# zhibaishouheilab/HealthiVert-GAN

Hardware: AMD Instinct MI355X
Metric: sagittal slices/sec (train step, G+D) at 256x256 bs=16 (higher is better)
Workload: dtype f16; 1 GPU; two-stage coarse+refine generator + 3x PatchGAN D train step, 256x256, per-GPU bs=16, norm=batch, vanilla GAN; global_batch=16, parallelism=dp1, launch=hipGraph replay (1 graphs/step), 4 streams

## Files before the change

healthivert-gan_amd/csrc/conv_igemm.hip:

```cpp
#include <string.h>

#include "hv_common.h"
#include <stdlib.h>

#define HV_MAX_TAPS 25
#define HV_BK 32

thread_local int hv_path_note = 0;
thread_local int hv_wtable_used = 0;
extern "C" int hv_last_weight_tables(void) { return hv_wtable_used; }
thread_local char hv_kname[192] = "";
extern "C" const char* hv_last_kernel_name(void) { return hv_kname; }
extern "C" int hv_last_kernel_path(void) { return hv_path_note; }
thread_local hipEvent_t hv_ev_start = nullptr, hv_ev_stop = nullptr;
extern "C" int hv_set_kernel_timing(void* ev_start, void* ev_stop) {
    hv_ev_start = (hipEvent_t)ev_start; hv_ev_stop = (hipEvent_t)ev_stop;
    return HV_OK;
}

int hv_conv2d_halo(const hv_conv_desc* d, const void* w_f16, hipStream_t s);
int hv_conv2d_g4(const hv_conv_desc* d, hipStream_t s);
int hv_conv2d_thin_dgrad(const hv_conv_desc* d, hipStream_t s);
int hv_conv2d_logits_dgrad(const hv_conv_desc* d, hipStream_t s);
size_t hv_conv2d_g4_stats_floats(const hv_conv_desc* d, int* nparts);
size_t hv_conv2d_g4_bstats_parts(const hv_conv_desc* d);
size_t hv_conv2d_logits_bstats_parts(const hv_conv_desc* d);
size_t hv_wgrad_halo_workspace_bytes(const hv_wgrad_desc* d);
int hv_wgrad_halo(const hv_wgrad_desc* d, int* nslabs, hipStream_t s);
size_t hv_wgrad_tr_workspace_bytes(const hv_wgrad_desc* d);
int hv_wgrad_tr(const hv_wgrad_desc* d, int* nslabs, hipStream_t s);
int hv_wgrad_thin(const hv_wgrad_desc* d, int* nslabs, hipStream_t s);
size_t hv_wgrad_thin_workspace_bytes(const hv_wgrad_desc* d);
int hv_conv2d_narrow(const hv_conv_desc* d, hipStream_t s);
int hv_conv2d_thin_in(const hv_conv_desc* d, hipStream_t s);
int hv_conv2d_stem5(const hv_conv_desc* d, hipStream_t s);
int hv_conv2d_stem5_dgrad(const hv_conv_desc* d, hipStream_t s);
int hv_conv2d_head(const hv_conv_desc* d, hipStream_t s);
int hv_conv2d_px(const hv_conv_desc* d, hipStream_t s);
int hv_conv2d_s2t(const hv_conv_desc* d, hipStream_t s);

struct ConvCls {
    int ph, pw, Hc, Wc, ntaps, Ktot, m0, mcount;
    uint32_t taps[HV_MAX_TAPS];
};
struct ConvK {
    const void* x; const float* w; const float* bias; const float* scale; void* y;
    int x_half, y_half, mul_half;
    long long w_bs, scale_bs;
    int B, Hl, Wl, in_shift, Wp, img_stride, x_ld, x_coff, Cin;
    int Cout, w_row, y_ld, y_coff, Ho, Wo;
    int bstep, boff, ostep;
    float alpha; int act, accumulate, vec_store, ncls;
    int xcd_swizzle;
    const void* mul_src; int mul_ld, mul_coff, mul_act, mul_vec;
    ConvCls cls[4];
};

template <typename T> struct Stage;
template <> struct Stage<float> {
    static constexpr int LD = HV_BK + 4;
    static __device__ __forceinline__ void st4(float* dst, float4 v) { *reinterpret_cast<float4*>(dst) = v; }
};
template <> struct Stage<_Float16> {
    static constexpr int LD = HV_BK + 8;
    static __device__ __forceinline__ void st4(_Float16* dst, float4 v) {
        f16x4 h = {(_Float16)v.x, (_Float16)v.y, (_Float16)v.z, (_Float16)v.w};
        *reinterpret_cast<f16x4*>(dst) = h;
    }
};

template <typename T, int MT, int NT> struct Frags;
template <int MT, int NT> struct Frags<float, MT, NT> {
    float4 w[NT][2], x[MT][2];
    __device__ __forceinline__ void load(const float* Bs, const float* As, int wrow0, int xrow0, int lane) {
        const int off = (lane & 15) * Stage<float>::LD + (lane >> 4) * 8;
#pragma unroll
        for (int n = 0; n < NT; ++n) {
            const float* p = Bs + (wrow0 + n * 16) * Stage<float>::LD + off;
            w[n][0] = *reinterpret_cast<const float4*>(p);
            w[n][1] = *reinterpret_cast<const float4*>(p + 4);
        }
#pragma unroll
        for (int m = 0; m < MT; ++m) {
            const float* p = As + (xrow0 + m * 16) * Stage<float>::LD + off;
            x[m][0] = *reinterpret_cast<const float4*>(p);
            x[m][1] = *reinterpret_cast<const float4*>(p + 4);
        }
    }
    __device__ __forceinline__ void mma(f32x4 (&acc)[NT][MT]) {
#pragma unroll
        for (int n = 0; n < NT; ++n)
#pragma unroll
            for (int m = 0; m < MT; ++m) {
                f32x4 a = acc[n][m];
                a = __builtin_amdgcn_mfma_f32_16x16x4f32(w[n][0].x, x[m][0].x, a, 0, 0, 0);
                a = __builtin_amdgcn_mfma_f32_16x16x4f32(w[n][0].y, x[m][0].y, a, 0, 0, 0);
                a = __builtin_amdgcn_mfma_f32_16x16x4f32(w[n][0].z, x[m][0].z, a, 0, 0, 0);
                a = __builtin_amdgcn_mfma_f32_16x16x4f32(w[n][0].w, x[m][0].w, a, 0, 0, 0);
                a = __builtin_amdgcn_mfma_f32_16x16x4f32(w[n][1].x, x[m][1].x, a, 0, 0, 0);
                a = __builtin_amdgcn_mfma_f32_16x16x4f32(w[n][1].y, x[m][1].y, a, 0, 0, 0);
                a = __builtin_amdgcn_mfma_f32_16x16x4f32(w[n][1].z, x[m][1].z, a, 0, 0, 0);
                a = __builtin_amdgcn_mfma_f32_16x16x4f32(w[n][1].w, x[m][1].w, a, 0, 0, 0);
                acc[n][m] = a;
            }
    }
};
template <int MT, int NT> struct Frags<_Float16, MT, NT> {
    f16x8 w[NT], x[MT];
    __device__ __forceinline__ void load(const _Float16* Bs, const _Float16* As, int wrow0, int xrow0, int lane) {
        const int off = (lane & 15) * Stage<_Float16>::LD + (lane >> 4) * 8;
#pragma unroll
        for (int n = 0; n < NT; ++n) w[n] = *reinterpret_cast<const f16x8*>(Bs + (wrow0 + n * 16) * Stage<_Float16>::LD + off);
#pragma unroll
        for (int m = 0; m < MT; ++m) x[m] = *reinterpret_cast<const f16x8*>(As + (xrow0 + m * 16) * Stage<_Float16>::LD + off);
    }
    __device__ __forceinline__ void mma(f32x4 (&acc)[NT][MT]) {
#pragma unroll
        for (int n = 0; n < NT; ++n)
#pragma unroll
            for (int m = 0; m < MT; ++m) acc[n][m] = __builtin_amdgcn_mfma_f32_16x16x32_f16(w[n], x[m], acc[n][m], 0, 0, 0);
    }
};

template <typename T, int BM, int BN, int WM, int WN, bool ASC, bool XH>
__global__ __launch_bounds__(256) void conv_igemm_kernel(const ConvK p) {
    constexpr int LD = Stage<T>::LD;
    constexpr int APASS = BM / 32;
    constexpr int BPASS = (BN + 31) / 32;
    constexpr int TMW = BM / WM, TNW = BN / WN;
    constexpr int MT = TMW / 16, NT = TNW / 16;
    static_assert(WM * WN == 4 && MT >= 1 && NT >= 1, "bad tile");
    __shared__ __attribute__((aligned(16))) T As[BM * LD];
    __shared__ __attribute__((aligned(16))) T Bs[BN * LD];
    __shared__ uint32_t taps_s[32];

    const int tid = threadIdx.x, lane = tid & 63, wave = tid >> 6;
    int bx = blockIdx.x;
    if (p.xcd_swizzle) {
        const int q = gridDim.x >> 3, r = gridDim.x & 7, xcd = bx & 7, loc = bx >> 3;
        bx = xcd < r ? xcd * (q + 1) + loc : r * (q + 1) + (xcd - r) * q + loc;
    }
    int ci = 0;
#pragma unroll
    for (int i = 1; i < 4; ++i)
        if (i < p.ncls && bx >= p.cls[i].m0) ci = i;
    const ConvCls& C = p.cls[ci];
    const int ntaps = C.ntaps, Ktot = C.Ktot, Hc = C.Hc, Wc = C.Wc, Mc = C.mcount, ph = C.ph, pw = C.pw;
    if (tid < ntaps) taps_s[tid] = C.taps[tid];
    const int m_base = (bx - C.m0) * BM;
    const int n_base = blockIdx.y * BN;
    const int HWc = Hc * Wc;

    const int chunk = tid & 7, prow = tid >> 3;
    int a_nb[APASS], a_hw[APASS];
    const int sample0 = m_base / HWc;
#pragma unroll
    for (int i = 0; i < APASS; ++i) {
        const int m = m_base + prow + i * 32;
        int bh = -20000, bw = -20000, nb = 0;
        if (m < Mc) {
            const int n = m / HWc, rem = m - n * HWc;
            const int ii = rem / Wc, jj = rem - ii * Wc;
            bh = ii * p.bstep + p.boff;
            bw = jj * p.bstep + p.boff;
            nb = n * p.img_stride;
        }
        a_nb[i] = nb;
        a_hw[i] = (int)(((uint32_t)bh << 16) | ((uint32_t)bw & 0xffffu));
    }
    const float* wbase = p.w + (p.w_bs ? (long long)sample0 * p.w_bs : 0ll);
    const int nk = (Ktot + HV_BK - 1) / HV_BK;

    float4 ra[APASS], rb[BPASS];
    auto gload = [&](int kt) {
        const int kg = kt * HV_BK + chunk * 4;
        if (!ASC) {
            const bool kok = kg < Ktot;
            int tapi = 0, c = 0, dh = 0, dw = 0, widx = 0;
            if (kok) {
                tapi = kg / p.Cin;
                c = kg - tapi * p.Cin;
                const uint32_t e = taps_s[tapi];
                dh = (int)(int8_t)(e & 0xff);
// ... 524 lines not shown
#pragma unroll
            for (int it = 0; it < XPT; ++it) store(Xs, LDX, rx[it], x_cg[it], x_run[it]);
        }
        __syncthreads();
        if (pix0 + KT < pix_end) {
            if (has_g) load_g(pix0 + KT);
            if (has_x) load_x(pix0 + KT);
        }
        if constexpr (F16) {
            const _Float16* G16 = reinterpret_cast<const _Float16*>(Gs);
            const _Float16* X16 = reinterpret_cast<const _Float16*>(Xs);
#pragma unroll
            for (int ks = 0; ks < KT / 32; ++ks) {
                f16x8 a[NT], b[CT];
#pragma unroll
                for (int n = 0; n < NT; ++n) {
                    const int row = wn * TNW + n * 16 + (lane & 15);
                    a[n] = *reinterpret_cast<const f16x8*>(G16 + row * LDG + ((ks * 4 + (lane >> 4)) ^ ((row >> 2) & 7)) * 8);
                }
#pragma unroll
                for (int c = 0; c < CT; ++c) {
                    const int row = wc * TCW + c * 16 + (lane & 15);
                    b[c] = *reinterpret_cast<const f16x8*>(X16 + row * LDX + ((ks * 4 + (lane >> 4)) ^ ((row >> 2) & 7)) * 8);
                }
#pragma unroll
                for (int n = 0; n < NT; ++n)
#pragma unroll
                    for (int c = 0; c < CT; ++c) acc[n][c] = __builtin_amdgcn_mfma_f32_16x16x32_f16(a[n], b[c], acc[n][c], 0, 0, 0);
            }
        } else {
            const float* G32 = reinterpret_cast<const float*>(Gs);
            const float* X32 = reinterpret_cast<const float*>(Xs);
#pragma unroll
            for (int k4 = 0; k4 < KT / 4; ++k4) {
                const int pk = k4 * 4 + (lane >> 4);
                float a[NT], b[CT];
#pragma unroll
                for (int n = 0; n < NT; ++n) a[n] = G32[pk * LDG + wn * TNW + n * 16 + (lane & 15)];
#pragma unroll
                for (int c = 0; c < CT; ++c) b[c] = X32[pk * LDX + wc * TCW + c * 16 + (lane & 15)];
#pragma unroll
                for (int n = 0; n < NT; ++n)
#pragma unroll
                    for (int c = 0; c < CT; ++c) acc[n][c] = __builtin_amdgcn_mfma_f32_16x16x4f32(a[n], b[c], acc[n][c], 0, 0, 0);
            }
        }
    }
    if (do_bias) {
        __syncthreads();
        float* bsh = reinterpret_cast<float*>(Xs);
        if (has_g) { bsh[tid * 4 + 0] = bs0; bsh[tid * 4 + 1] = bs1; bsh[tid * 4 + 2] = bs2; bsh[tid * 4 + 3] = bs3; }
        __syncthreads();
        if (tid < BN && n_base + tid < p.Cout) {
            const int cg = tid >> 2, c = tid & 3;
            float t = 0.f;
            for (int run = 0; run < KT / 8; ++run) t += bsh[(run * (BN / 4) + cg) * 4 + c];
            p.bias_out[(long long)blockIdx.x * p.Cout + n_base + tid] = t;
        }
    }
    float* out = p.out + (long long)blockIdx.x * p.slab;
#pragma unroll
    for (int n = 0; n < NT; ++n)
#pragma unroll
        for (int c = 0; c < CT; ++c) {
            const int j = j_base + wc * TCW + c * 16 + (lane & 15);
            if (j >= p.J) continue;
#pragma unroll
            for (int r = 0; r < 4; ++r) {
                const int co = n_base + wn * TNW + n * 16 + (lane >> 4) * 4 + r;
                if (co < p.Cout) out[(long long)co * p.J + j] = acc[n][c][r];
            }
        }
}

template <int G>
__global__ __launch_bounds__(256) void wgrad_reduce_kernel(const float* __restrict__ slabs, float* __restrict__ dw, long long n, int splits, int accumulate,
                                                           const float* __restrict__ bslabs, float* __restrict__ dbias, int nb, int bias_accumulate) {
    constexpr int Q = 256 / G;
    __shared__ float4 sh[G][Q];
    const int e = threadIdx.x % Q, grp = threadIdx.x / Q;
    const long long wblocks = (n / 4 + Q - 1) / Q;
    auto add = [](float4& a, const float4 b) { a.x += b.x; a.y += b.y; a.z += b.z; a.w += b.w; };
    const bool bias_block = (long long)blockIdx.x >= wblocks;
    const long long i = bias_block ? ((long long)blockIdx.x - wblocks) * Q + e : ((long long)blockIdx.x * Q + e) * 4;
    const bool live = i < (bias_block ? (long long)nb : n);
    float4 acc[4];
#pragma unroll
    for (int u = 0; u < 4; ++u) acc[u] = make_float4(0.f, 0.f, 0.f, 0.f);
    if (live) {
        int k = grp;
        if (bias_block) {
            for (; k + 3 * G < splits; k += 4 * G)
#pragma unroll
                for (int u = 0; u < 4; ++u) acc[u].x += bslabs[(long long)(k + u * G) * nb + i];
            for (; k < splits; k += G) acc[0].x += bslabs[(long long)k * nb + i];
        } else {
            for (; k + 3 * G < splits; k += 4 * G)
#pragma unroll
                for (int u = 0; u < 4; ++u) add(acc[u], *reinterpret_cast<const float4*>(slabs + (long long)(k + u * G) * n + i));
            for (; k < splits; k += G) add(acc[0], *reinterpret_cast<const float4*>(slabs + (long long)k * n + i));
        }
    }
    add(acc[0], acc[1]); add(acc[2], acc[3]); add(acc[0], acc[2]);
    sh[grp][e] = acc[0];
    __syncthreads();
#pragma unroll
    for (int h = G / 2; h >= 1; h >>= 1) {
        if (grp < h) add(sh[grp][e], sh[grp + h][e]);
        __syncthreads();
    }
    if (grp == 0 && live) {
        float4 t = sh[0][e];
        if (bias_block) dbias[i] = bias_accumulate ? dbias[i] + t.x : t.x;
        else {
            if (accumulate) add(t, *reinterpret_cast<const float4*>(dw + i));
            *reinterpret_cast<float4*>(dw + i) = t;
        }
    }
}

thread_local HvFold hv_carry = {};
thread_local int hv_carry_taken = 0;
static int launch_wgrad_reduce(const float* slabs, float* dw, long long n, int splits, int accumulate, const float* bslabs, float* dbias, int nb,
                                int bias_accumulate, hipStream_t s);
static int wgrad_fold_or_defer(const hv_wgrad_desc* d, const float* slabs, long long n, int splits, const float* bslabs, hipStream_t s) {
    if (d->pending && !(n & 3) && !(((uintptr_t)slabs | (uintptr_t)d->dw) & 15)) {
        hv_wgrad_fold* f = d->pending;
        f->slabs = slabs; f->dw = d->dw; f->numel = n; f->nslabs = splits; f->accumulate = d->accumulate;
        f->bias_slabs = d->dbias ? bslabs : nullptr; f->dbias = d->dbias; f->Cout = d->Cout; f->dbias_accumulate = d->dbias_accumulate;
        return HV_OK;
    }
    if (d->pending) d->pending->nslabs = 0;
    return launch_wgrad_reduce(slabs, d->dw, n, splits, d->accumulate, bslabs, d->dbias, d->Cout, d->dbias_accumulate, s);
}
extern "C" int hv_wgrad_fold_now(const hv_wgrad_fold* f, void* stream) {
    if (!f) return HV_ERR_ARG;
    if (f->nslabs <= 0) return HV_OK;
    if (!f->slabs || !f->dw || f->numel <= 0 || (f->numel & 3)) return HV_ERR_ARG;
    return launch_wgrad_reduce(f->slabs, f->dw, f->numel, f->nslabs, f->accumulate, f->bias_slabs, f->dbias, f->Cout, f->dbias_accumulate, (hipStream_t)stream);
}
static int launch_wgrad_reduce(const float* slabs, float* dw, long long n, int splits, int accumulate, const float* bslabs, float* dbias, int nb,
                                int bias_accumulate, hipStream_t s) {
#define HV_RED(G_)                                                                                                                          \
    hipLaunchKernelGGL(wgrad_reduce_kernel<G_>, dim3(hv_cdiv(n / 4, 256 / G_) + (dbias ? hv_cdiv(nb, 256 / G_) : 0)), dim3(256), 0, s, slabs, dw, n, splits, \
                       accumulate, bslabs, dbias, nb, bias_accumulate)
    if (splits <= 16) HV_RED(4);
    else if (splits <= 64) HV_RED(16);
    else HV_RED(32);
#undef HV_RED
    HV_LAUNCH_CHECK();
    return HV_OK;
}

struct WgradPlan { int BN, BC, KT, splits, chunk; };
static int wgrad_plan(const hv_wgrad_desc* d, WgradPlan* pl) {
    const int J = d->KH * d->KW * d->Cin;
    const long long M = (long long)d->B * d->Ho * d->Wo;
    constexpr int kBc128MinJ = 4096;
    int BN, BC;
    if (d->Cout <= 16) { BN = 16; BC = 128; }
    else if (d->Cout <= 32) { BN = 32; BC = 128; }
    else if (d->Cout <= 64) { BN = 64; BC = J >= 512 ? 256 : 64; }
    else { BN = 128; BC = J >= kBc128MinJ ? 128 : 64; }
    const long long tiles = (long long)hv_cdiv(d->Cout, BN) * hv_cdiv(J, BC);
    constexpr int kWantWg = 512;
    long long want = (kWantWg + tiles - 1) / tiles;
    if (want > 256) want = 256;
    long long maxs = (M + 255) / 256;
    long long splits = want < 1 ? 1 : want;
    if (splits > maxs) splits = maxs;
    if (splits < 1) splits = 1;
    const int KT = d->precision == HV_F32 ? 32 : ((BN == 64 && BC == 64) ? 128 : 64);
    long long chunk = (M + splits - 1) / splits;
    chunk = (chunk + KT - 1) / KT * KT;
    splits = (M + chunk - 1) / chunk;
    pl->BN = BN; pl->BC = BC; pl->KT = KT; pl->splits = (int)splits; pl->chunk = (int)chunk;
    return HV_OK;
}

static int wgrad_validate(const hv_wgrad_desc* d) {
    if (!d || !d->x || !d->g || !d->dw) return HV_ERR_ARG;
    if (d->B <= 0 || d->H <= 0 || d->W <= 0 || d->Cin <= 0 || d->Cout <= 0 || d->KH <= 0 || d->KW <= 0 || d->stride <= 0 ||
        d->dil <= 0 || d->pad < 0 || d->Ho <= 0 || d->Wo <= 0)
        return HV_ERR_ARG;
    if ((d->Cin & 3) || (d->Cout & 3) || (d->x_ld & 3) || (d->x_coff & 3) || (d->g_ld & 3) || (d->g_coff & 3)) return HV_ERR_UNSUPPORTED;
    if (((uintptr_t)d->x & 15) || ((uintptr_t)d->g & 15)) return HV_ERR_UNSUPPORTED;
    if (d->in_shift < 0 || d->in_shift > 1) return HV_ERR_UNSUPPORTED;
    if (d->precision != HV_F32 && d->precision != HV_F16) return HV_ERR_ARG;
    if ((d->x_f16 != 0) != (d->g_f16 != 0) || (d->x_f16 != 0) != (d->precision == HV_F16)) return HV_ERR_UNSUPPORTED;
    const int Hp = d->H >> d->in_shift, Wp = d->W >> d->in_shift;
    if ((long long)d->B * Hp * Wp * d->x_ld >= (1ll << 29) || (long long)d->B * d->Ho * d->Wo * d->g_ld >= (1ll << 29)) return HV_ERR_UNSUPPORTED;
    return HV_OK;
}

extern "C" size_t hv_conv2d_wgrad_workspace_bytes(const hv_wgrad_desc* d) {
    if (wgrad_validate(d) != HV_OK) return 0;
    const size_t thin = hv_wgrad_thin_workspace_bytes(d);
    if (thin) return thin;
    const size_t halo = hv_wgrad_halo_workspace_bytes(d);
    if (halo) return halo;
    const size_t trb = hv_wgrad_tr_workspace_bytes(d);
    if (trb) return trb;
    WgradPlan pl;
    wgrad_plan(d, &pl);
    if (pl.splits <= 1 && !d->accumulate && !d->dbias) return 0;
    return (size_t)pl.splits * ((size_t)d->Cout * d->KH * d->KW * d->Cin + (d->dbias ? d->Cout : 0)) * sizeof(float);
}

template <typename T, bool FAST>
static int launch_wgrad(const WgradK& k, const WgradPlan& pl, hipStream_t s) {
    constexpr bool F16 = sizeof(T) == 2;
    constexpr int KT = F16 ? 64 : 32, KT64 = F16 ? 128 : 32;
    dim3 grid(pl.splits, hv_cdiv(k.Cout, pl.BN), hv_cdiv(k.J, pl.BC));
    if (pl.KT != ((pl.BN == 64 && pl.BC == 64) ? KT64 : KT)) return HV_ERR_ARG;
    {
        const int bn = pl.BN, bc = pl.BN == 16 || pl.BN == 32 ? 128 : pl.BC, wn = (pl.BN <= 32 || (pl.BN == 64 && pl.BC == 256)) ? 1 : 2;
        HV_KNAME("wgrad_kernel<%s, %d, %d, %d, %d, %d, %s>", F16 ? "_Float16" : "float", bn, bc, wn, 4 / wn, pl.KT, FAST ? "true" : "false");
    }
    constexpr bool SH = F16;
    if (pl.BN == 16) hipLaunchKernelGGL((wgrad_kernel<T, 16, 128, 1, 4, KT, FAST, SH>), grid, dim3(256), 0, s, k);
    else if (pl.BN == 32) hipLaunchKernelGGL((wgrad_kernel<T, 32, 128, 1, 4, KT, FAST, SH>), grid, dim3(256), 0, s, k);
    else if (pl.BN == 64 && pl.BC == 256) hipLaunchKernelGGL((wgrad_kernel<T, 64, 256, 1, 4, KT, FAST, SH>), grid, dim3(256), 0, s, k);
    else if (pl.BN == 64) hipLaunchKernelGGL((wgrad_kernel<T, 64, 64, 2, 2, KT64, FAST, SH>), grid, dim3(256), 0, s, k);
    else if (pl.BC == 128) hipLaunchKernelGGL((wgrad_kernel<T, 128, 128, 2, 2, KT, FAST, SH>), grid, dim3(256), 0, s, k);
    else hipLaunchKernelGGL((wgrad_kernel<T, 128, 64, 2, 2, KT, FAST, SH>), grid, dim3(256), 0, s, k);
    HV_LAUNCH_CHECK();
    return HV_OK;
}

static int wgrad_dispatch(const hv_wgrad_desc* d, void* stream);
extern "C" int hv_conv2d_wgrad(const hv_wgrad_desc* d, void* stream) {
    int rc = wgrad_validate(d);
    if (rc != HV_OK) return rc;
    hv_carry.splits = 0;
    hv_carry_taken = 0;
    const hv_wgrad_fold* c = d->carry;
    if (c && c->nslabs > 0) {
        if (!c->slabs || !c->dw || c->numel <= 0 || (c->numel & 3)) return HV_ERR_ARG;
        const bool overlap = (c->slabs == d->workspace);
        if (!overlap && c->dw != d->dw) {
            hv_carry = HvFold{c->slabs, c->dw, c->numel, c->nslabs, c->accumulate, c->dbias ? c->bias_slabs : nullptr, c->dbias, c->Cout, c->dbias_accumulate};
        } else {
            rc = hv_wgrad_fold_now(c, stream);
            if (rc != HV_OK) return rc;
            c = nullptr;
        }
    } else c = nullptr;
    rc = wgrad_dispatch(d, stream);
    const bool taken = hv_carry_taken != 0;
    hv_carry.splits = 0;
    hv_carry_taken = 0;
    if (rc != HV_OK) return rc;
    if (c && !taken) return hv_wgrad_fold_now(c, stream);
    return HV_OK;
}
static int wgrad_dispatch(const hv_wgrad_desc* d, void* stream) {
    int rc;
    const long long nW = (long long)d->Cout * d->KH * d->KW * d->Cin;
    {
        int nslabs = 0;
        rc = hv_wgrad_thin(d, &nslabs, (hipStream_t)stream);
        if (rc == HV_ERR_UNSUPPORTED) rc = hv_wgrad_halo(d, &nslabs, (hipStream_t)stream);
        if (rc == HV_ERR_UNSUPPORTED) rc = hv_wgrad_tr(d, &nslabs, (hipStream_t)stream);
        if (rc == HV_OK) {
            const float* bsl = d->dbias ? d->workspace + (long long)nslabs * nW : nullptr;
            return wgrad_fold_or_defer(d, d->workspace, nW, nslabs, bsl, (hipStream_t)stream);
        }
        if (rc != HV_ERR_UNSUPPORTED) return rc;
    }
    WgradPlan pl;
    wgrad_plan(d, &pl);
    const bool direct = pl.splits <= 1 && !d->accumulate && !d->dbias;
    if (!direct) {
        if (!d->workspace || d->workspace_bytes < (size_t)pl.splits * (nW + (d->dbias ? d->Cout : 0)) * sizeof(float)) return HV_ERR_WORKSPACE;
    }
    hv_path_note = 10;
    WgradK k;
    k.x = d->x; k.g = d->g; k.out = direct ? d->dw : d->workspace;
    k.B = d->B; k.Hl = d->H; k.Wl = d->W; k.in_shift = d->in_shift; k.Wp = d->W >> d->in_shift;
    k.img_stride = (d->H >> d->in_shift) * k.Wp * d->x_ld; k.x_ld = d->x_ld; k.x_coff = d->x_coff; k.Cin = d->Cin;
    k.Ho = d->Ho; k.Wo = d->Wo; k.g_ld = d->g_ld; k.g_coff = d->g_coff; k.Cout = d->Cout;
    k.KW = d->KW; k.stride = d->stride; k.pad = d->pad; k.dil = d->dil; k.J = d->KH * d->KW * d->Cin;
    k.M = d->B * d->Ho * d->Wo; k.chunk = pl.chunk; k.slab = nW;
    k.bias_out = d->dbias ? d->workspace + (long long)pl.splits * nW : nullptr;
    k.half = d->x_f16 ? 1 : 0;
    const size_t es = k.half ? 2 : 4;
    k.x_bytes = (unsigned)((size_t)d->B * (d->H >> d->in_shift) * k.Wp * d->x_ld * es);
    k.g_bytes = (unsigned)((size_t)k.M * d->g_ld * es);
    auto pow2 = [](int v) { return v > 0 && (v & (v - 1)) == 0; };
    const bool fast = pow2(d->Wo) && pow2(d->Ho) && d->Wo >= 8;
    k.lw = k.lhw = 0;
    k.kt_q = pl.KT / d->Wo; k.kt_r = pl.KT % d->Wo;
    if (fast) { k.lw = __builtin_ctz(d->Wo); k.lhw = k.lw + __builtin_ctz(d->Ho); }
    hipStream_t s = (hipStream_t)stream;
    HV_TIMING_BEGIN(s);
    if (d->precision == HV_F32) rc = fast ? launch_wgrad<float, true>(k, pl, s) : launch_wgrad<float, false>(k, pl, s);
    else rc = fast ? launch_wgrad<_Float16, true>(k, pl, s) : launch_wgrad<_Float16, false>(k, pl, s);
    HV_TIMING_END(s);
    if (rc != HV_OK) return rc;
    if (!direct) return wgrad_fold_or_defer(d, d->workspace, nW, pl.splits, k.bias_out, s);
    if (d->pending) d->pending->nslabs = 0;
    return HV_OK;
}
```

healthivert-gan_amd/csrc/prep.hip:

```cpp
#include <stdlib.h>

#include "hv_common.h"

#define SN_EPS 1e-12f
#define PREP_THREADS 512
#define PREP_MAXK 4608
#define PREP_MAXCO 1024

__device__ __forceinline__ long long wsrc_index(const hv_wprep_layer& L, int co, int ci, int tap) {
    return L.transposed_src ? ((long long)ci * L.Cout + co) * L.taps + tap : ((long long)co * L.Cin + ci) * L.taps + tap;
}

__global__ __launch_bounds__(PREP_THREADS) void weight_prep_kernel(const hv_wprep_layer* __restrict__ layers) {
    const hv_wprep_layer L = layers[blockIdx.x];
    __shared__ float v_s[PREP_MAXK];
    __shared__ float u_s[PREP_MAXCO];
    __shared__ float red[20];
    const int tid = threadIdx.x, lane = tid & 63, wave = tid >> 6, nwave = PREP_THREADS / 64;
    const int K = L.Cin * L.taps;
    float sigma = 1.f;
    if (L.sn) {
        const float* W = L.w_orig;
        for (int i = tid; i < L.Cout; i += PREP_THREADS) u_s[i] = L.u[i];
        for (int i = tid; i < K; i += PREP_THREADS) v_s[i] = L.v[i];
// ... 551 lines not shown
    return HV_OK;
}

__global__ void adam_tick_kernel(float* step) { step[0] += 1.f; }

__global__ __launch_bounds__(256) void adam_kernel(const hv_adam_tensor* __restrict__ ts, const float* __restrict__ lr_p, float beta1,
                                                   float beta2, float eps, const float* __restrict__ step_p) {
    const hv_adam_tensor t = ts[blockIdx.y];
    const long long base = (long long)blockIdx.x * 1024;
    if (base >= t.n) return;
    const float step = step_p[0], lr = lr_p[0];
    const float bc1 = 1.f - powf(beta1, step), bc2 = 1.f - powf(beta2, step);
    const float step_size = lr / bc1, bc2_sqrt = sqrtf(bc2);
#pragma unroll
    for (int k = 0; k < 4; ++k) {
        const long long i = base + k * 256 + threadIdx.x;
        if (i < t.n) {
            const float g = t.g[i];
            const float m = t.m[i] + (g - t.m[i]) * (1.f - beta1);
            const float v = t.v[i] * beta2 + (1.f - beta2) * g * g;
            t.m[i] = m;
            t.v[i] = v;
            const float denom = sqrtf(v) / bc2_sqrt + eps;
            t.p[i] = t.p[i] - step_size * (m / denom);
        }
    }
}

__global__ __launch_bounds__(256) void grad_unscale_check_kernel(float* __restrict__ g, long long n, float mul, float* __restrict__ state) {
    bool bad = false;
    const bool scale = mul != 1.f;
    for (long long i = ((long long)blockIdx.x * 256 + threadIdx.x) * 4; i < n; i += (long long)gridDim.x * 1024) {
        if (i + 3 < n) {
            float4 v = *reinterpret_cast<const float4*>(g + i);
            bad |= !(fabsf(v.x) <= 3.0e38f) | !(fabsf(v.y) <= 3.0e38f) | !(fabsf(v.z) <= 3.0e38f) | !(fabsf(v.w) <= 3.0e38f);
            if (scale) { v.x *= mul; v.y *= mul; v.z *= mul; v.w *= mul; *reinterpret_cast<float4*>(g + i) = v; }
        } else {
            for (long long j = i; j < n; ++j) { bad |= !(fabsf(g[j]) <= 3.0e38f); if (scale) g[j] *= mul; }
        }
    }
    if (__any(bad) && (threadIdx.x & 63) == 0) { hv_publish(state + 1, 1.f); hv_stores_done(); }
    __syncthreads();
    if (threadIdx.x == 0) {
        unsigned* ticket = reinterpret_cast<unsigned*>(state + 4);
        if (hv_take_ticket_is_last(ticket, gridDim.x)) {
            const bool any_bad = hv_collect(state + 1) != 0.f;
            if (any_bad) state[2] += 1.f; else state[0] += 1.f;
            state[3] = any_bad ? 1.f : 0.f;
            hv_publish(state + 1, 0.f);
            hv_ticket_reset(ticket);
        }
    }
}
__global__ __launch_bounds__(256) void adam_guarded_kernel(const hv_adam_tensor* __restrict__ ts, const float* __restrict__ lr_p, float beta1,
                                                           float beta2, float eps, const float* __restrict__ state) {
    if (state[3] != 0.f) return;
    const hv_adam_tensor t = ts[blockIdx.y];
    const long long base = (long long)blockIdx.x * 1024;
    if (base >= t.n) return;
    const float step = state[0], lr = lr_p[0];
    const float bc1 = 1.f - powf(beta1, step), bc2 = 1.f - powf(beta2, step);
    const float step_size = lr / bc1, bc2_sqrt = sqrtf(bc2);
#pragma unroll
    for (int k = 0; k < 4; ++k) {
        const long long i = base + k * 256 + threadIdx.x;
        if (i < t.n) {
            const float g = t.g[i];
            const float m = t.m[i] + (g - t.m[i]) * (1.f - beta1);
            const float v = t.v[i] * beta2 + (1.f - beta2) * g * g;
            t.m[i] = m;
            t.v[i] = v;
            const float denom = sqrtf(v) / bc2_sqrt + eps;
            t.p[i] = t.p[i] - step_size * (m / denom);
        }
    }
}
extern "C" int hv_adam_step_guarded(const hv_adam_tensor* d_tensors, int n_tensors, long long max_numel, const float* d_lr, float beta1,
                                    float beta2, float eps, float* d_state, float* flat_grad, long long n_grad, float grad_mul, void* stream) {
    if (!d_tensors || n_tensors <= 0 || max_numel <= 0 || !d_lr || !d_state || !flat_grad || n_grad <= 0 || ((uintptr_t)flat_grad & 15) || !(grad_mul > 0.f))
        return HV_ERR_ARG;
    const int blocks = (int)(n_grad / 4096 + 1 < 256 ? n_grad / 4096 + 1 : 256);
    hipLaunchKernelGGL(grad_unscale_check_kernel, dim3(blocks), dim3(256), 0, (hipStream_t)stream, flat_grad, n_grad, grad_mul, d_state);
    HV_LAUNCH_CHECK();
    dim3 grid(hv_cdiv(max_numel, 1024), n_tensors);
    hipLaunchKernelGGL(adam_guarded_kernel, grid, dim3(256), 0, (hipStream_t)stream, d_tensors, d_lr, beta1, beta2, eps, d_state);
    HV_LAUNCH_CHECK();
    return HV_OK;
}

extern "C" int hv_adam_step(const hv_adam_tensor* d_tensors, int n_tensors, long long max_numel, const float* d_lr, float beta1,
                            float beta2, float eps, float* d_step, void* stream) {
    if (!d_tensors || n_tensors <= 0 || max_numel <= 0 || !d_lr || !d_step) return HV_ERR_ARG;
    hipLaunchKernelGGL(adam_tick_kernel, dim3(1), dim3(1), 0, (hipStream_t)stream, d_step);
    HV_LAUNCH_CHECK();
    dim3 grid(hv_cdiv(max_numel, 1024), n_tensors);
    hipLaunchKernelGGL(adam_kernel, grid, dim3(256), 0, (hipStream_t)stream, d_tensors, d_lr, beta1, beta2, eps, d_step);
    HV_LAUNCH_CHECK();
    return HV_OK;
}

__global__ void fill_kernel(float* p, long long n, float v) {
    long long i = (long long)blockIdx.x * blockDim.x + threadIdx.x;
    const long long st = (long long)gridDim.x * blockDim.x;
    for (; i < n; i += st) p[i] = v;
}
__global__ void axpy_kernel(float* y, const float* x, long long n, float a, int assign) {
    long long i = (long long)blockIdx.x * blockDim.x + threadIdx.x;
    const long long st = (long long)gridDim.x * blockDim.x;
    for (; i < n; i += st) y[i] = assign ? a * x[i] : y[i] + a * x[i];
}
static int ew_grid(long long n) { long long b = (n + 255) / 256; return (int)(b > 4096 ? 4096 : (b < 1 ? 1 : b)); }
extern "C" int hv_fill(float* p, long long n, float value, void* stream) {
    if (!p || n <= 0) return HV_ERR_ARG;
    hipLaunchKernelGGL(fill_kernel, dim3(ew_grid(n)), dim3(256), 0, (hipStream_t)stream, p, n, value);
    HV_LAUNCH_CHECK();
    return HV_OK;
}
extern "C" int hv_axpy(float* y, const float* x, long long n, float a, void* stream) {
    if (!y || !x || n <= 0) return HV_ERR_ARG;
    hipLaunchKernelGGL(axpy_kernel, dim3(ew_grid(n)), dim3(256), 0, (hipStream_t)stream, y, x, n, a, 0);
    HV_LAUNCH_CHECK();
    return HV_OK;
}
__global__ void affine_kernel(float* y, const float* x, long long n, float a, float b) {
    long long i = (long long)blockIdx.x * blockDim.x + threadIdx.x;
    const long long st = (long long)gridDim.x * blockDim.x;
    for (; i < n; i += st) y[i] = a * x[i] + b;
}
extern "C" int hv_affine(float* y, const float* x, long long n, float a, float b, void* stream) {
    if (!y || !x || n <= 0) return HV_ERR_ARG;
    hipLaunchKernelGGL(affine_kernel, dim3(ew_grid(n)), dim3(256), 0, (hipStream_t)stream, y, x, n, a, b);
    HV_LAUNCH_CHECK();
    return HV_OK;
}

__global__ void mul_kernel(float* y, const float* x, const float* z, long long n) {
    long long i = (long long)blockIdx.x * blockDim.x + threadIdx.x;
    const long long st = (long long)gridDim.x * blockDim.x;
    for (; i < n; i += st) y[i] = z ? (y[i] * x[i]) * z[i] : y[i] * x[i];
}
extern "C" int hv_mul(float* y, const float* x, long long n, void* stream) {
    if (!y || !x || n <= 0) return HV_ERR_ARG;
    hipLaunchKernelGGL(mul_kernel, dim3(ew_grid(n)), dim3(256), 0, (hipStream_t)stream, y, x, (const float*)nullptr, n);
    HV_LAUNCH_CHECK();
    return HV_OK;
}
extern "C" int hv_mul3(float* y, const float* x, const float* z, long long n, void* stream) {
    if (!y || !x || !z || n <= 0) return HV_ERR_ARG;
    hipLaunchKernelGGL(mul_kernel, dim3(ew_grid(n)), dim3(256), 0, (hipStream_t)stream, y, x, z, n);
    HV_LAUNCH_CHECK();
    return HV_OK;
}

extern "C" int hv_version(void) { return 106; }
extern "C" const char* hv_arch(void) { return "gfx950"; }
```

healthivert-gan_amd/csrc/wgrad_tr.hip:

```cpp
#include <stdlib.h>

#include <type_traits>

#include "hv_common.h"

typedef __fp16 hv_fp16x4 __attribute__((__vector_size__(4 * sizeof(__fp16))));
typedef unsigned int u32x4 __attribute__((ext_vector_type(4)));
typedef unsigned int u32x2 __attribute__((ext_vector_type(2)));

struct WTrK {
    const _Float16* x; const _Float16* g; float* slabs;
    int Hl, Wl, in_shift, Wp, img_stride, x_ld, x_coff, Cin;
    int Ho, Wo, g_ld, g_coff, Cout, pad;
    int tiles_x, tiles_per_img, ntiles;
    int dil, tiles_per_sub;
    int Hf, Wf;
    long long slab;
    unsigned x_bytes, g_bytes;
    float* bias_out;
    int dbg;
    int gx;
    HvFold fold;
};

__device__ __forceinline__ f16x4 tr_read(const _Float16* lds_addr) {
    typedef hv_fp16x4 __attribute__((address_space(3)))* lp;
    return __builtin_bit_cast(f16x4, __builtin_amdgcn_ds_read_tr16_b64_v4f16((lp)(lds_addr)));
}

__host__ __device__ constexpr int wtr_stride(int ch, int st) {
    const int row = ch * 2;
    if (st == 1) return (row / 32) % 2 ? row : row + 32;
    return row + 16;
}

template <int KS, int ST, int BN, int BC>
__global__ __launch_bounds__(256, 2) void wgrad_tr_kernel(const WTrK p) {
    constexpr int TH = 8, TW = 16, TAPS = KS * KS, SLOTS = (TAPS + 3) / 4;
    constexpr int PH = (TH - 1) * ST + KS, PW = (TW - 1) * ST + KS;
    constexpr int NT = BN / 16, CT = BC / 16;
    constexpr int SG = wtr_stride(BN, 1), SX = wtr_stride(BC, ST);
    constexpr int GI = TH * TW * (BN / 8), XI = PH * PW * (BC / 8);
    constexpr int GPT = (GI + 255) / 256, XPT = (XI + 255) / 256;
    static_assert(NT * CT * SLOTS <= 32, "accumulator budget");
    extern __shared__ __attribute__((aligned(16))) char smem[];
    char* Gs = smem;
    char* Xs = smem + TH * TW * SG;

    if ((int)blockIdx.x >= p.gx) {
        const int fx = (int)gridDim.x - p.gx;
        hv_fold_blocks(p.fold, ((int)blockIdx.x - p.gx) + fx * ((int)blockIdx.y + (int)gridDim.y * (int)blockIdx.z), fx * (int)gridDim.y * (int)gridDim.z, smem);
        return;
    }
    const int tid = threadIdx.x, lane = tid & 63, wave = __builtin_amdgcn_readfirstlane(tid >> 6);
    const int co0 = blockIdx.y * BN, ci0 = blockIdx.z * BC;
    const int grp = lane >> 4, sub = lane & 15, qr = sub >> 2, pc = sub & 3;

    f32x4 acc[SLOTS][NT][CT];
#pragma unroll
    for (int s = 0; s < SLOTS; ++s)
#pragma unroll
        for (int n = 0; n < NT; ++n)
#pragma unroll
            for (int c = 0; c < CT; ++c) acc[s][n][c] = (f32x4){0.f, 0.f, 0.f, 0.f};
    const bool do_bias = p.bias_out != nullptr && blockIdx.z == 0 && wave == 0;
    f32x4 bacc[NT];
#pragma unroll
    for (int n = 0; n < NT; ++n) bacc[n] = (f32x4){0.f, 0.f, 0.f, 0.f};

    const _Float16* ga = reinterpret_cast<const _Float16*>(Gs + (4 * grp + qr) * SG + pc * 8);
    const _Float16* xa[SLOTS];
#pragma unroll
    for (int s = 0; s < SLOTS; ++s) {
        const int t = wave + 4 * s, r = t / KS, q = t - r * KS;
        xa[s] = reinterpret_cast<const _Float16*>(Xs + ((4 * grp + qr) * ST + (t < TAPS ? r * PW + q : 0)) * SX + pc * 8);
    }

    const __amdgpu_buffer_rsrc_t xsrc = __builtin_amdgcn_make_buffer_rsrc(const_cast<_Float16*>(p.x), 0, p.x_bytes, 0x00020000);
    const __amdgpu_buffer_rsrc_t gsrc = __builtin_amdgcn_make_buffer_rsrc(const_cast<_Float16*>(p.g), 0, p.g_bytes, 0x00020000);
    u32x4 rg[GPT], rx[XPT];
    auto prefetch = [&](int tile) __attribute__((always_inline)) {
        const int n_img = tile / p.tiles_per_img;
        int tr = tile - n_img * p.tiles_per_img;
        const int d = p.dil, sub = tr / p.tiles_per_sub;
        tr -= sub * p.tiles_per_sub;
        const int ry = sub / d, rxo = sub - ry * d;
        const int oy0 = (tr / p.tiles_x) * TH, ox0 = (tr % p.tiles_x) * TW;
#pragma unroll
        for (int i = 0; i < GPT; ++i) {
            const int e = tid + i * 256;
            const int c8 = e % (BN / 8), pix = e / (BN / 8), ty = pix / TW, tx = pix - ty * TW;
            const int oy = oy0 + ty, ox = ox0 + tx, co = co0 + c8 * 8;
            const bool ok = e < GI && oy < p.Ho && ox < p.Wo && co < p.Cout;
            rg[i] = __builtin_amdgcn_raw_buffer_load_b128(gsrc, ok ? (unsigned)(((n_img * p.Hf + ry + d * oy) * p.Wf + rxo + d * ox) * p.g_ld + p.g_coff + co) * 2u : 0x80000000u, 0, 0);
        }
#pragma unroll
        for (int i = 0; i < XPT; ++i) {
            const int e = tid + i * 256;
            const int c8 = e % (BC / 8), pix = e / (BC / 8), py = pix / PW, px = pix - py * PW;
            const int hi = oy0 * ST - p.pad + py, wi = ox0 * ST - p.pad + px, ci = ci0 + c8 * 8;
            const bool ok = e < XI && (unsigned)hi < (unsigned)p.Hl && (unsigned)wi < (unsigned)p.Wl && ci < p.Cin;
            rx[i] = __builtin_amdgcn_raw_buffer_load_b128(
                xsrc, ok ? (unsigned)(n_img * p.img_stride + (((ry + d * hi) >> p.in_shift) * p.Wp + ((rxo + d * wi) >> p.in_shift)) * p.x_ld + p.x_coff + ci) * 2u : 0x80000000u, 0, 0);
        }
    };
    auto flush = [&]() __attribute__((always_inline)) {
#pragma unroll
        for (int i = 0; i < GPT; ++i) {
            const int e = tid + i * 256;
            if (e < GI) *reinterpret_cast<u32x4*>(Gs + (e / (BN / 8)) * SG + (e % (BN / 8)) * 16) = rg[i];
        }
#pragma unroll
        for (int i = 0; i < XPT; ++i) {
            const int e = tid + i * 256;
            if (e < XI) *reinterpret_cast<u32x4*>(Xs + (e / (BC / 8)) * SX + (e % (BC / 8)) * 16) = rx[i];
        }
    };
    const f16x8 ones = {1, 1, 1, 1, 1, 1, 1, 1};

    if ((int)blockIdx.x < p.ntiles) prefetch(blockIdx.x);
    for (int tile = blockIdx.x; tile < p.ntiles; tile += p.gx) {
        __syncthreads();
        flush();
        __syncthreads();
        if (tile + p.gx < p.ntiles) prefetch(tile + p.gx);
        auto lda = [&](int ks, f16x8 (&a)[NT]) __attribute__((always_inline)) {
#pragma unroll
            for (int n = 0; n < NT; ++n) {
                const f16x4 lo = tr_read(ga + ((2 * ks) * TW * SG + n * 32) / 2), hi = tr_read(ga + ((2 * ks + 1) * TW * SG + n * 32) / 2);
                a[n] = (f16x8){lo[0], lo[1], lo[2], lo[3], hi[0], hi[1], hi[2], hi[3]};
            }
        };
        auto ldb = [&](int ks, int sl, f16x8 (&bb)[CT]) __attribute__((always_inline)) {
#pragma unroll
            for (int c = 0; c < CT; ++c) {
                const f16x4 lo = tr_read(xa[sl] + ((2 * ks) * ST * PW * SX + c * 32) / 2), hi = tr_read(xa[sl] + ((2 * ks + 1) * ST * PW * SX + c * 32) / 2);
                bb[c] = (f16x8){lo[0], lo[1], lo[2], lo[3], hi[0], hi[1], hi[2], hi[3]};
            }
        };
        f16x8 aq[2][NT], bq[2][CT];
        lda(0, aq[0]);
        ldb(0, 0, bq[0]);
#pragma unroll
        for (int ks = 0; ks < TH / 2; ++ks) {
            if (do_bias) {
#pragma unroll
                for (int n = 0; n < NT; ++n) bacc[n] = __builtin_amdgcn_mfma_f32_16x16x32_f16(aq[ks & 1][n], ones, bacc[n], 0, 0, 0);
            }
#pragma unroll
            for (int sl = 0; sl < SLOTS; ++sl) {
                const int idx = ks * SLOTS + sl;
                __builtin_amdgcn_sched_barrier(0);
                if (sl + 1 < SLOTS) ldb(ks, sl + 1, bq[(idx + 1) & 1]);
                else if (ks + 1 < TH / 2) { lda(ks + 1, aq[(ks + 1) & 1]); ldb(ks + 1, 0, bq[(idx + 1) & 1]); }
                __builtin_amdgcn_sched_barrier(0);
                if (wave + 4 * sl < TAPS) {
#pragma unroll
                    for (int n = 0; n < NT; ++n)
#pragma unroll
                        for (int c = 0; c < CT; ++c) acc[sl][n][c] = __builtin_amdgcn_mfma_f32_16x16x32_f16(aq[ks & 1][n], bq[idx & 1][c], acc[sl][n][c], 0, 0, 0);
                }
            }
        }
    }
    float* out = p.slabs + (long long)blockIdx.x * p.slab;
#pragma unroll
    for (int s = 0; s < SLOTS; ++s) {
        const int t = wave + 4 * s;
        if (t >= TAPS) continue;
#pragma unroll
        for (int n = 0; n < NT; ++n)
#pragma unroll
            for (int c = 0; c < CT; ++c) {
                const int ci = ci0 + c * 16 + (lane & 15);
#pragma unroll
                for (int r = 0; r < 4; ++r) {
                    const int co = co0 + n * 16 + (lane >> 4) * 4 + r;
                    if (co < p.Cout && ci < p.Cin) out[((long long)co * TAPS + t) * p.Cin + ci] = acc[s][n][c][r];
                }
            }
    }
    if (do_bias && (lane & 15) == 0) {
#pragma unroll
        for (int n = 0; n < NT; ++n)
#pragma unroll
            for (int r = 0; r < 4; ++r) {
                const int co = co0 + n * 16 + (lane >> 4) * 4 + r;
                if (co < p.Cout) p.bias_out[(long long)blockIdx.x * p.Cout + co] = bacc[n][r];
            }
    }
}

typedef int i32x4 __attribute__((ext_vector_type(4)));
__device__ __forceinline__ void wtr_dma16(i32x4 rsrc, unsigned lds_byte, unsigned voff) {
    asm volatile("s_mov_b32 m0, %0\n\tbuffer_load_dwordx4 %1, %2, 0 offen lds" : : "s"(__builtin_amdgcn_readfirstlane(lds_byte)), "v"(voff), "s"(rsrc) : "memory", "m0");
}
__device__ __forceinline__ i32x4 wtr_rsrc(const void* base, unsigned bytes) {
    const unsigned long long a = (unsigned long long)base;
    return (i32x4){(int)__builtin_amdgcn_readfirstlane((unsigned)a), (int)__builtin_amdgcn_readfirstlane((unsigned)(a >> 32) & 0xffffu),
                   (int)__builtin_amdgcn_readfirstlane(bytes), 0x00020000};
}

template <int KS, int ST>
struct WTrdCfg {
    static constexpr int BN = 64, BC = 32, TH = 8, TW = 16, TAPS = KS * KS, SLOTS = (TAPS + 3) / 4;
    static constexpr int PH = (TH - 1) * ST + KS, PW = (TW - 1) * ST + KS, PWP = ST == 1 ? 24 : 48;
    static constexpr int NT = BN / 16, CT = BC / 16, XPR = BC / 8, XROW = BC * 2;
    static constexpr int XI = PH * PWP * XPR, XINS = (XI + 63) / 64, XPT = (XINS + 3) / 4;
    static constexpr int GBUF = TH * TW * 128, XBUF = XINS * 1024, BUFSZ = GBUF + XBUF;
    static constexpr int SPS = CT == 2 ? 2 : 4;
};

template <int KS, int ST>
__global__ __launch_bounds__(512, 1) void wgrad_trd_kernel(const WTrK p) {
    using C = WTrdCfg<KS, ST>;
    constexpr int BN = C::BN, BC = C::BC, TH = C::TH, TW = C::TW, TAPS = C::TAPS, SLOTS = C::SLOTS, PW = C::PW, PWP = C::PWP;
    constexpr int NT = C::NT, CT = C::CT, XPR = C::XPR, XROW = C::XROW, XI = C::XI, XINS = C::XINS, XPT = C::XPT, GBUF = C::GBUF, BUFSZ = C::BUFSZ;
    constexpr int SPS = SLOTS < C::SPS ? SLOTS : C::SPS, NSTG = (SLOTS + SPS - 1) / SPS;
    extern __shared__ __attribute__((aligned(16))) char smem[];
    const int tid = threadIdx.x, lane = tid & 63, wave8 = __builtin_amdgcn_readfirstlane(tid >> 6);
    const bool loader = wave8 >= 4;
    const int wave = wave8 & 3;
    const int co0 = blockIdx.y * BN, ci0 = blockIdx.z * BC;
    const int grp = lane >> 4, sub = lane & 15, qr = sub >> 2, pc = sub & 3, tx_l = 4 * grp + qr;

    f32x4 acc[SLOTS][NT][CT];
#pragma unroll
    for (int s = 0; s < SLOTS; ++s)
#pragma unroll
        for (int n = 0; n < NT; ++n)
#pragma unroll
            for (int c = 0; c < CT; ++c) acc[s][n][c] = (f32x4){0.f, 0.f, 0.f, 0.f};
    const bool do_bias = p.bias_out != nullptr && blockIdx.z == 0 && wave8 == 4;
    f32x4 bacc[NT];
#pragma unroll
    for (int n = 0; n < NT; ++n) bacc[n] = (f32x4){0.f, 0.f, 0.f, 0.f};

    const int ga0 = tx_l * 128 + (((tx_l >> 1) & 3) << 5) + pc * 8;
    int xa0[SLOTS];
#pragma unroll
    for (int s = 0; s < SLOTS; ++s) {
        const int t = wave + 4 * s, tt = t < TAPS ? t : 0, r = tt / KS, q = tt - r * KS;
        const int u = ST == 1 ? tx_l + q : tx_l + (q >> 1), half = ST == 1 ? 0 : (q & 1) * 24;
        xa0[s] = GBUF + (r * PWP + half + u) * XROW + (((u >> 2) & 1) << 5) + pc * 8;
    }

    constexpr int NOPE = -(1 << 30);
    int grel[4], xrel[XPT], xpp[XPT];
#pragma unroll
    for (int i = 0; i < 4; ++i) {
        const int e = (wave * 4 + i) * 64 + lane, pix = e >> 3, j = e & 7, ty = pix >> 4, tx = pix & 15;
        const int co = co0 + ((j ^ (((tx >> 1) & 3) << 1)) << 3);
        grel[i] = co < p.Cout ? (ty * p.Wo + tx) * p.g_ld + p.g_coff + co : NOPE;
    }
#pragma unroll
    for (int i = 0; i < XPT; ++i) {
        const int e = (wave + 4 * i) * 64 + lane, row = e / XPR, j = e % XPR;
        const int py = row / PWP, rem = row - py * PWP;
        const int u = ST == 1 ? rem : rem % 24, px = ST == 1 ? rem : 2 * u + rem / 24;
        const int ci = ci0 + ((j ^ (((u >> 2) & 1) << 1)) << 3);
        const bool ok = e < XI && px < PW && ci < p.Cin;
        xrel[i] = ok ? (py * p.Wl + px) * p.x_ld + p.x_coff + ci : NOPE;
        xpp[i] = (py << 8) | px;
    }
    const i32x4 xsrc = wtr_rsrc(p.x, p.x_bytes), gsrc = wtr_rsrc(p.g, p.g_bytes);
    const unsigned lds0 = (unsigned)(size_t)(__attribute__((address_space(3))) char*)smem;

    struct TileAt { int hmax, wmax, gbase, y0, x0, xbase; };
    auto tile_at = [&](int tile) __attribute__((always_inline)) {
        TileAt t;
        const int n_img = tile / p.tiles_per_img, tr = tile - n_img * p.tiles_per_img;
        const int ty0 = tr / p.tiles_x, oy0 = ty0 * TH, ox0 = (tr - ty0 * p.tiles_x) * TW;
        t.hmax = p.Ho - oy0; t.wmax = p.Wo - ox0;
        t.gbase = ((n_img * p.Ho + oy0) * p.Wo + ox0) * p.g_ld;
        t.y0 = oy0 * ST - p.pad; t.x0 = ox0 * ST - p.pad;
        t.xbase = n_img * p.img_stride + (t.y0 * p.Wl + t.x0) * p.x_ld;
        return t;
    };
    constexpr int NPART = 4 + XPT;
    auto issue_part = [&](const TileAt& t, int buf, int part) __attribute__((always_inline)) {
        const unsigned dstb = lds0 + buf * BUFSZ;
        if (part < 4) {
            const int i = part, k = wave * 4 + i, pix = k * 8 + (lane >> 3), ty = pix >> 4, tx = pix & 15;
            const bool ok = grel[i] >= 0 && ty < t.hmax && tx < t.wmax;
            wtr_dma16(gsrc, dstb + k * 1024, ok ? (unsigned)(t.gbase + grel[i]) * 2u : 0x80000000u);
        } else {
            const int i = part - 4, k = wave + 4 * i;
            if (k < XINS) {
                const int hi = t.y0 + (xpp[i] >> 8), wi = t.x0 + (xpp[i] & 255);
                const bool ok = xrel[i] > NOPE / 2 && (unsigned)hi < (unsigned)p.Hl && (unsigned)wi < (unsigned)p.Wl;
                wtr_dma16(xsrc, dstb + GBUF + k * 1024, ok ? (unsigned)(t.xbase + xrel[i]) * 2u : 0x80000000u);
            }
        }
    };

    const f16x8 ones = {1, 1, 1, 1, 1, 1, 1, 1};
    f16x8 aq[2][NT], bq[2][SPS][CT];
    auto lda = [&](int BUFC, int ks, int n, f16x8 (&a)[NT]) __attribute__((always_inline)) {
        const _Float16* base = reinterpret_cast<const _Float16*>(smem + ((ga0 + BUFC) ^ (n << 5)));
        const f16x4 lo = tr_read(base + ((2 * ks) * TW * 128) / 2), hi = tr_read(base + ((2 * ks + 1) * TW * 128) / 2);
        a[n] = (f16x8){lo[0], lo[1], lo[2], lo[3], hi[0], hi[1], hi[2], hi[3]};
    };
    auto ldb = [&](int BUFC, int ks, int sl, f16x8 (&bb)[CT]) __attribute__((always_inline)) {
#pragma unroll
        for (int c = 0; c < CT; ++c) {
            const _Float16* base = reinterpret_cast<const _Float16*>(smem + ((xa0[sl] + BUFC) ^ (c << 5)));
            const f16x4 lo = tr_read(base + ((2 * ks) * ST * PWP * XROW) / 2), hi = tr_read(base + ((2 * ks + 1) * ST * PWP * XROW) / 2);
            bb[c] = (f16x8){lo[0], lo[1], lo[2], lo[3], hi[0], hi[1], hi[2], hi[3]};
        }
    };
    auto load_stage = [&](int BUFC, int g) __attribute__((always_inline)) {
        const int ks = g / NSTG, j = g - ks * NSTG;
#pragma unroll
        for (int u = 0; u < SPS; ++u)
            if (j * SPS + u < SLOTS) ldb(BUFC, ks, j * SPS + u, bq[g & 1][u]);
    };
    auto load_a_part = [&](int BUFC, int ks, int j) __attribute__((always_inline)) {
        constexpr int PER = (NT + NSTG - 1) / NSTG;
#pragma unroll
        for (int n = j * PER; n < (j + 1) * PER && n < NT; ++n) lda(BUFC, ks, n, aq[ks & 1]);
    };
#define WTD_MIX()                                                                                                                       \
    do {                                                                                                                                \
        __builtin_amdgcn_sched_group_barrier(0x008, 1, 0); __builtin_amdgcn_sched_group_barrier(0x100, 1, 0);                             \
        __builtin_amdgcn_sched_group_barrier(0x008, 1, 0); __builtin_amdgcn_sched_group_barrier(0x100, 1, 0);                             \
        __builtin_amdgcn_sched_group_barrier(0x008, 1, 0); __builtin_amdgcn_sched_group_barrier(0x100, 1, 0);                             \
        __builtin_amdgcn_sched_group_barrier(0x008, 1, 0); __builtin_amdgcn_sched_group_barrier(0x100, 1, 0);                             \
    } while (0)
    auto tile_body = [&](int BUFC) __attribute__((always_inline)) {
        constexpr int NG = (TH / 2) * NSTG;
#pragma unroll
        for (int j = 0; j < NSTG; ++j) load_a_part(BUFC, 0, j);
        load_stage(BUFC, 0);
#pragma unroll
        for (int g = 0; g < NG; ++g) {
            const int ks = g / NSTG, j = g - ks * NSTG;
            __builtin_amdgcn_sched_barrier(0);
#ifdef WT_STAMPS
            if (!(p.dbg & 4))
#endif
            if (g + 1 < NG) {
                load_stage(BUFC, g + 1);
                if (ks + 1 < TH / 2) load_a_part(BUFC, ks + 1, j);
            }
#pragma unroll
            for (int u = 0; u < SPS; ++u) {
                const int sl = j * SPS + u;
#ifdef WT_STAMPS
                if (p.dbg & 2) continue;
#endif
                if (sl < SLOTS && wave + 4 * sl < TAPS) {
#pragma unroll
                    for (int n = 0; n < NT; ++n)
#pragma unroll
                        for (int c = 0; c < CT; ++c) acc[sl][n][c] = __builtin_amdgcn_mfma_f32_16x16x32_f16(aq[ks & 1][n], bq[g & 1][u][c], acc[sl][n][c], 0, 0, 0);
                }
            }
            WTD_MIX(); WTD_MIX(); WTD_MIX(); WTD_MIX();
        }
    };
    auto bias_tile = [&](int BUFC) __attribute__((always_inline)) {
#pragma unroll
        for (int ks = 0; ks < TH / 2; ++ks) {
            f16x8 a[NT];
#pragma unroll
            for (int n = 0; n < NT; ++n) lda(BUFC, ks, n, a);
#pragma unroll
            for (int n = 0; n < NT; ++n) bacc[n] = __builtin_amdgcn_mfma_f32_16x16x32_f16(a[n], ones, bacc[n], 0, 0, 0);
        }
    };

#ifdef WT_STAMPS
    unsigned long long wt_t[4], wt_sum[3] = {0, 0, 0}, wt_begin = __builtin_amdgcn_s_memrealtime();
#define WTD_STAMP(i) wt_t[i] = __builtin_amdgcn_s_memrealtime()
#define WTD_ACC() do { __builtin_amdgcn_sched_barrier(0); WTD_STAMP(3); for (int i_ = 0; i_ < 3; ++i_) wt_sum[i_] += wt_t[i_ + 1] - wt_t[i_]; } while (0)
#else
#define WTD_STAMP(i)
#define WTD_ACC()
#endif
    const int step = gridDim.x;
    auto issue_tile = [&](int t, int buf) __attribute__((always_inline)) {
        const TileAt at = tile_at(t);
#pragma unroll
        for (int q = 0; q < NPART; ++q) issue_part(at, buf, q);
    };
    if (loader) {
        int tile = blockIdx.x, buf = 0;
        if (tile < p.ntiles) issue_tile(tile, 0);
        for (; tile < p.ntiles; tile += step, buf ^= 1) {
            __builtin_amdgcn_s_waitcnt(0x0F70);
            __builtin_amdgcn_s_barrier();
#ifdef WT_STAMPS
            if (p.dbg & 1) continue;
#endif
            if (tile + step < p.ntiles) issue_tile(tile + step, buf ^ 1);
            if (do_bias) bias_tile(buf * BUFSZ);
        }
    } else {
        int bufoff = 0;
        for (int tile = blockIdx.x; tile < p.ntiles; tile += step, bufoff ^= BUFSZ) {
            WTD_STAMP(0);
            __syncthreads();
            WTD_STAMP(1);
            WTD_STAMP(2);
            tile_body(bufoff);
            WTD_ACC();
        }
    }
#ifdef WT_STAMPS
    const unsigned long long wt_loop_end = __builtin_amdgcn_s_memrealtime();
#endif
    float* out = p.slabs + (long long)blockIdx.x * p.slab;
#pragma unroll
    for (int s = 0; s < SLOTS; ++s) {
        const int t = wave + 4 * s;
        if (t >= TAPS || loader) continue;
#pragma unroll
        for (int n = 0; n < NT; ++n)
#pragma unroll
            for (int c = 0; c < CT; ++c) {
                const int ci = ci0 + c * 16 + (lane & 15);
#pragma unroll
                for (int r = 0; r < 4; ++r) {
                    const int co = co0 + n * 16 + (lane >> 4) * 4 + r;
                    if (co < p.Cout && ci < p.Cin) out[((long long)co * TAPS + t) * p.Cin + ci] = acc[s][n][c][r];
                }
            }
    }
    if (do_bias && (lane & 15) == 0) {
#pragma unroll
        for (int n = 0; n < NT; ++n)
#pragma unroll
            for (int r = 0; r < 4; ++r) {
                const int co = co0 + n * 16 + (lane >> 4) * 4 + r;
                if (co < p.Cout) p.bias_out[(long long)blockIdx.x * p.Cout + co] = bacc[n][r];
            }
    }
#ifdef WT_STAMPS
    __builtin_amdgcn_s_waitcnt(0);
    if (tid == 0 && blockIdx.x == gridDim.x / 2 && blockIdx.y == gridDim.y / 2 && blockIdx.z == 0)
        printf("wtrd<%d,%d> grid %d x %d x %d: barrier %.2f  tile scalars %.2f  mfma section (+dma issue) %.2f  | loop %.2f  slab write %.2f us\n", KS, ST,
               (int)gridDim.x, (int)gridDim.y, (int)gridDim.z, wt_sum[0] / 100.0, wt_sum[1] / 100.0, wt_sum[2] / 100.0,
               (wt_loop_end - wt_begin) / 100.0, (__builtin_amdgcn_s_memrealtime() - wt_loop_end) / 100.0);
#endif
}

struct WTrPlan { int BN, BC, gx, dil; size_t lds; bool dma; };

static bool wgrad_tr_plan(const hv_wgrad_desc* d, WTrPlan* pl) {
    if (d->precision != HV_F16 || !d->x_f16 || !d->g_f16 || d->KH != d->KW) return false;
    if (!((d->KH == 3 || d->KH == 4) && (d->stride == 1 || d->stride == 2))) return false;
    pl->dil = 1;
    if (d->dil != 1) {
        if ((d->dil != 2 && d->dil != 4 && d->dil != 8) || d->KH != 3 || d->stride != 1 || d->pad != d->dil || d->in_shift) return false;
        if (d->H % d->dil || d->W % d->dil || d->Ho != d->H || d->Wo != d->W) return false;
        pl->dil = d->dil;
    } else if (d->Ho != (d->H + 2 * d->pad - d->KH) / d->stride + 1 || d->Wo != (d->W + 2 * d->pad - d->KW) / d->stride + 1) return false;
    if ((d->Cin & 7) || (d->Cout & 7) || (d->x_ld & 7) || (d->x_coff & 7) || (d->g_ld & 7) || (d->g_coff & 7)) return false;
    if (d->Cout < (d->stride == 2 ? 16 : 32) || d->Cin < 16) return false;
    pl->BN = d->Cout >= 64 ? 64 : 32;
    pl->BC = d->Cin >= 32 ? 32 : 16;
    {
        if (d->stride == 1 && d->Cout == 64 && d->Cin <= 64 && d->Cin >= 32) pl->BN = 32;
    }
    const bool s2_dma = d->stride == 2 && pl->BN == 64 && !(d->Cin & 31) && d->in_shift == 0;
    if (d->stride == 2 && pl->BN == 64 && !s2_dma) pl->BC = 16;
    const int PH = 7 * d->stride + d->KH, PW = 15 * d->stride + d->KW;
    pl->lds = (size_t)128 * wtr_stride(pl->BN, 1) + (size_t)PH * PW * wtr_stride(pl->BC, d->stride);
    pl->dma = pl->BN == 64 && pl->BC == 32 && d->in_shift == 0 && pl->dil == 1;
    const bool dma_candidate = pl->dma;
    if (pl->dma) {
        const int PWP = d->stride == 1 ? 24 : 48, XI = PH * PWP * (pl->BC / 8);
        pl->lds = (size_t)2 * (8 * 16 * 128 + (XI + 63) / 64 * 1024);
    }
    const long long ntiles = (long long)d->B * pl->dil * pl->dil * hv_cdiv(d->Ho / pl->dil, 8) * hv_cdiv(d->Wo / pl->dil, 16);
    constexpr int kWantBig = 256, kWantSmall = 512;
    auto chunks = [&]() {
        const long long pairs = (long long)hv_cdiv(d->Cout, pl->BN) * hv_cdiv(d->Cin, pl->BC);
        const int want = (pairs <= 4 && (long long)d->Cout * d->KH * d->KW * d->Cin * 4 <= 256 * 1024) ? kWantSmall : kWantBig;
        long long gx = (want + pairs - 1) / pairs;
        if (gx > ntiles) gx = ntiles;
        if (gx < 1) gx = 1;
        pl->gx = (int)gx;
    };
    chunks();
    if (dma_candidate && ntiles < 4 * pl->gx) {
        pl->dma = false;
        if (d->stride == 2) { pl->BC = 16; chunks(); }
        pl->lds = (size_t)128 * wtr_stride(pl->BN, 1) + (size_t)PH * PW * wtr_stride(pl->BC, d->stride);
    }
    return true;
}

size_t hv_wgrad_tr_workspace_bytes(const hv_wgrad_desc* d) {
    WTrPlan pl;
    if (!wgrad_tr_plan(d, &pl)) return 0;
    return (size_t)pl.gx * ((size_t)d->Cout * d->KH * d->KW * d->Cin + (d->dbias ? d->Cout : 0)) * sizeof(float);
}

template <int KS, int ST, int BN, int BC>
static int launch_wtr(const WTrK& k, const WTrPlan& pl, const hv_wgrad_desc* d, hipStream_t s) {
    auto kern = wgrad_tr_kernel<KS, ST, BN, BC>;
    static int lds_limit = 48 * 1024;
    if ((int)pl.lds > lds_limit) {
        hipError_t e = hipFuncSetAttribute(reinterpret_cast<const void*>(kern), hipFuncAttributeMaxDynamicSharedMemorySize, 150 * 1024);
        if (e != hipSuccess) return -1000 - (int)e;
        lds_limit = 150 * 1024;
    }
    dim3 grid(pl.gx, hv_cdiv(d->Cout, BN), hv_cdiv(d->Cin, BC));
    WTrK kk = k;
    kk.fold.splits = 0;
    const int fx = hv_carry_blocks((int)(grid.y * grid.z));
    if (fx > 0) { kk.fold = hv_carry; hv_carry_taken = 1; grid.x += fx; }
    hv_path_note = 12;
    HV_KNAME("wgrad_tr_kernel<%d, %d, %d, %d>", KS, ST, BN, BC);
    HV_TIMING_BEGIN(s);
    hipLaunchKernelGGL(kern, grid, dim3(256), pl.lds, s, kk);
    HV_TIMING_END(s);
    HV_LAUNCH_CHECK();
    return HV_OK;
}

template <int KS, int ST>
static int launch_wtrd(const WTrK& k, const WTrPlan& pl, const hv_wgrad_desc* d, hipStream_t s) {
    auto kern = wgrad_trd_kernel<KS, ST>;
    static bool raised = false;
    if (!raised) {
        hipError_t e = hipFuncSetAttribute(reinterpret_cast<const void*>(kern), hipFuncAttributeMaxDynamicSharedMemorySize, 150 * 1024);
        if (e != hipSuccess) return -1000 - (int)e;
        raised = true;
    }
    dim3 grid(pl.gx, hv_cdiv(d->Cout, 64), hv_cdiv(d->Cin, WTrdCfg<KS, ST>::BC));
    hv_path_note = 13;
    HV_KNAME("wgrad_trd_kernel<%d, %d>", KS, ST);
    HV_TIMING_BEGIN(s);
    hipLaunchKernelGGL(kern, grid, dim3(512), pl.lds, s, k);
    HV_TIMING_END(s);
    HV_LAUNCH_CHECK();
    return HV_OK;
}

template <int KS, int ST, int BN>
__global__ __launch_bounds__(256, 2) void wgrad_thinx_kernel(const WTrK p) {
    constexpr int TH = 8, TW = 16, TAPS = KS * KS, NTN = (TAPS + 3) / 4, NT = BN / 16;
    constexpr int PH = (TH - 1) * ST + KS, PW = (TW - 1) * ST + KS;
    constexpr int SG = wtr_stride(BN, 1);
    constexpr int GI = TH * TW * (BN / 8), XI = PH * PW;
    constexpr int GPT = (GI + 255) / 256, XPT = (XI + 255) / 256;
    constexpr int XBYTES = (XI * 8 + 15) / 16 * 16;
    static_assert(NT * NTN <= 16, "accumulator budget");
    extern __shared__ __attribute__((aligned(16))) char smem[];
    char* Gs = smem;
    char* Xs = smem + TH * TW * SG;
    float* red = reinterpret_cast<float*>(smem);

    if ((int)blockIdx.x >= p.gx) {
        const int fx = (int)gridDim.x - p.gx;
        hv_fold_blocks(p.fold, ((int)blockIdx.x - p.gx) + fx * ((int)blockIdx.y + (int)gridDim.y * (int)blockIdx.z), fx * (int)gridDim.y * (int)gridDim.z, smem);
        return;
    }
    const int tid = threadIdx.x, lane = tid & 63, wave = __builtin_amdgcn_readfirstlane(tid >> 6);
    const int co0 = blockIdx.y * BN;
    const int grp = lane >> 4, sub = lane & 15, qr = sub >> 2, pc = sub & 3;
    f32x4 acc[NT][NTN];
#pragma unroll
    for (int n = 0; n < NT; ++n)
#pragma unroll
        for (int j = 0; j < NTN; ++j) acc[n][j] = (f32x4){0.f, 0.f, 0.f, 0.f};
    const bool do_bias = p.bias_out != nullptr;
    f32x4 bacc[NT];
#pragma unroll
    for (int n = 0; n < NT; ++n) bacc[n] = (f32x4){0.f, 0.f, 0.f, 0.f};
    const _Float16* ga = reinterpret_cast<const _Float16*>(Gs + ((2 * wave) * TW + 4 * grp + qr) * SG + pc * 8);
    const _Float16* xb[NTN];
#pragma unroll
    for (int j = 0; j < NTN; ++j) {
        const int t = 4 * j + pc, tt = t < TAPS ? t : 0, r = tt / KS, q = tt - r * KS;
        xb[j] = reinterpret_cast<const _Float16*>(Xs + ((((2 * wave) * ST + r) * PW) + (4 * grp + qr) * ST + q) * 8);
    }
    const __amdgpu_buffer_rsrc_t xsrc = __builtin_amdgcn_make_buffer_rsrc(const_cast<_Float16*>(p.x), 0, p.x_bytes, 0x00020000);
    const __amdgpu_buffer_rsrc_t gsrc = __builtin_amdgcn_make_buffer_rsrc(const_cast<_Float16*>(p.g), 0, p.g_bytes, 0x00020000);
    constexpr int DEPTH = BN > 16 ? 2 : 3;
    u32x4 rgs[DEPTH][GPT];
    u32x2 rxs[DEPTH][XPT];
    auto prefetch = [&](int tile, auto SI) __attribute__((always_inline)) {
        u32x4 (&rg)[GPT] = rgs[decltype(SI)::value];
        u32x2 (&rx)[XPT] = rxs[decltype(SI)::value];
        const int n_img = tile / p.tiles_per_img, tr = tile - n_img * p.tiles_per_img;
        const int oy0 = (tr / p.tiles_x) * TH, ox0 = (tr % p.tiles_x) * TW;
#pragma unroll
        for (int i = 0; i < GPT; ++i) {
            const int e = tid + i * 256;
            const int c8 = e % (BN / 8), pix = e / (BN / 8), ty = pix / TW, tx = pix - ty * TW;
            const int oy = oy0 + ty, ox = ox0 + tx, co = co0 + c8 * 8;
            const bool ok = e < GI && oy < p.Ho && ox < p.Wo && co < p.Cout;
            rg[i] = __builtin_amdgcn_raw_buffer_load_b128(gsrc, ok ? (unsigned)(((n_img * p.Ho + oy) * p.Wo + ox) * p.g_ld + p.g_coff + co) * 2u : 0x80000000u, 0, 0);
        }
#pragma unroll
        for (int i = 0; i < XPT; ++i) {
            const int e = tid + i * 256;
            const int py = e / PW, px = e - py * PW;
            const int hi = oy0 * ST - p.pad + py, wi = ox0 * ST - p.pad + px;
            const bool ok = e < XI && (unsigned)hi < (unsigned)p.Hl && (unsigned)wi < (unsigned)p.Wl;
            rx[i] = __builtin_bit_cast(u32x2, __builtin_amdgcn_raw_buffer_load_b64(xsrc, ok ? (unsigned)(n_img * p.img_stride + (hi * p.Wp + wi) * p.x_ld + p.x_coff) * 2u : 0x80000000u, 0, 0));
        }
    };
    auto flush = [&](auto SI) __attribute__((always_inline)) {
        u32x4 (&rg)[GPT] = rgs[decltype(SI)::value];
        u32x2 (&rx)[XPT] = rxs[decltype(SI)::value];
#pragma unroll
        for (int i = 0; i < GPT; ++i) {
            const int e = tid + i * 256;
            if (e < GI) *reinterpret_cast<u32x4*>(Gs + (e / (BN / 8)) * SG + (e % (BN / 8)) * 16) = rg[i];
        }
#pragma unroll
        for (int i = 0; i < XPT; ++i) {
            const int e = tid + i * 256;
            if (e < XI) *reinterpret_cast<u32x2*>(Xs + e * 8) = rx[i];
        }
    };
    const f16x8 ones = {1, 1, 1, 1, 1, 1, 1, 1};
    auto mfma_tile = [&]() __attribute__((always_inline)) {
        f16x8 a[NT], b[NTN];
#pragma unroll
        for (int n = 0; n < NT; ++n) {
            const f16x4 lo = tr_read(ga + (n * 32) / 2), hi = tr_read(ga + (TW * SG + n * 32) / 2);
            a[n] = (f16x8){lo[0], lo[1], lo[2], lo[3], hi[0], hi[1], hi[2], hi[3]};
        }
#pragma unroll
        for (int j = 0; j < NTN; ++j) {
            const f16x4 lo = tr_read(xb[j]), hi = tr_read(xb[j] + (ST * PW * 8) / 2);
            b[j] = (f16x8){lo[0], lo[1], lo[2], lo[3], hi[0], hi[1], hi[2], hi[3]};
        }
// ... 150 lines not shown
        f16x8 a[NT], b[NTN];
#pragma unroll
        for (int n = 0; n < NT; ++n) {
            const f16x4 lo = tr_read(xa + (n * 32) / 2), hi = tr_read(xa + (TW * SX + n * 32) / 2);
            a[n] = (f16x8){lo[0], lo[1], lo[2], lo[3], hi[0], hi[1], hi[2], hi[3]};
        }
#pragma unroll
        for (int j = 0; j < NTN; ++j) {
            const f16x4 lo = tr_read(tb[j]), hi = tr_read(tb[j] + (PW * 8) / 2);
            b[j] = (f16x8){lo[0], lo[1], lo[2], lo[3], hi[0], hi[1], hi[2], hi[3]};
        }
#pragma unroll
        for (int n = 0; n < NT; ++n)
#pragma unroll
            for (int j = 0; j < NTN; ++j) acc[n][j] = __builtin_amdgcn_mfma_f32_16x16x32_f16(a[n], b[j], acc[n][j], 0, 0, 0);
    };
    typedef std::integral_constant<int, 0> S0;
    typedef std::integral_constant<int, 1> S1;
    typedef std::integral_constant<int, (DEPTH > 2 ? 2 : 0)> S2;
    int tile = blockIdx.x;
    if (tile < p.ntiles) prefetch(tile, S0());
    if (DEPTH > 2 && tile + p.gx < p.ntiles) prefetch(tile + p.gx, S1());
    auto one = [&](auto SA, auto SC) __attribute__((always_inline)) {
        __syncthreads();
        flush(SA);
        __syncthreads();
        if (tile + (DEPTH - 1) * p.gx < p.ntiles) prefetch(tile + (DEPTH - 1) * p.gx, SC);
        mfma_tile();
        tile += p.gx;
    };
    while (tile < p.ntiles) {
        if constexpr (DEPTH > 2) {
            one(S0(), S2());
            if (tile >= p.ntiles) break;
            one(S1(), S0());
            if (tile >= p.ntiles) break;
            one(S2(), S1());
        } else {
            one(S0(), S1());
            if (tile >= p.ntiles) break;
            one(S1(), S0());
        }
    }
    __syncthreads();
    for (int wv = 0; wv < 4; ++wv) {
        if (wave == wv) {
#pragma unroll
            for (int n = 0; n < NT; ++n)
#pragma unroll
                for (int j = 0; j < NTN; ++j)
#pragma unroll
                    for (int r = 0; r < 4; ++r) {
                        float* d = red + ((n * NTN + j) * 16 + 4 * (lane >> 4) + r) * 16 + (lane & 15);
                        *d = wv == 0 ? acc[n][j][r] : *d + acc[n][j][r];
                    }
        }
        __syncthreads();
    }
    float* out = p.slabs + (long long)blockIdx.x * p.slab;
    for (int e = tid; e < NT * NTN * 256; e += 256) {
        const int row = e & 15, n = (e >> 4) % NT, cj = e / (16 * NT), col = cj & 15, j = cj >> 4;
        const int t = 4 * j + (col >> 2), co = col & 3, ci = ci0 + n * 16 + row;
        if (t < TAPS && co < p.Cout && ci < p.Cin) out[((long long)co * TAPS + t) * p.Cin + ci] = red[((n * NTN + j) * 16 + row) * 16 + col];
    }
}

struct WThinPlan { int kind, gx; size_t lds; };
static bool wgrad_thin_plan(const hv_wgrad_desc* d, WThinPlan* pl) {
    if (d->precision != HV_F16 || !d->x_f16 || !d->g_f16 || d->KH != d->KW || d->dil != 1 || d->in_shift != 0) return false;
    if (d->Ho != (d->H + 2 * d->pad - d->KH) / d->stride + 1 || d->Wo != (d->W + 2 * d->pad - d->KW) / d->stride + 1) return false;
    pl->kind = 0;
    const bool thin_x = d->Cin <= 4 && !(d->x_ld & 3) && !(d->x_coff & 3) && !(d->Cout & 7) && !(d->g_ld & 7) && !(d->g_coff & 7);
    const bool thin_g = d->Cout <= 4 && !(d->g_ld & 3) && !(d->g_coff & 3) && d->stride == 1 && !d->dbias && !(d->x_ld & 3) && !(d->x_coff & 3);
    if (thin_x && d->KH == 5 && d->stride == 1 && d->Cout <= 16) pl->kind = 1;
    else if (thin_g && d->KH == 4 && !(d->Cin & 63) && !(d->x_ld & 7) && !(d->x_coff & 7)) pl->kind = 2;
    else if (thin_g && d->KH == 3 && d->Cin <= 16 && d->Cin > 4) pl->kind = 3;
    if (!pl->kind) return false;
    const int BN = pl->kind == 2 ? 64 : 16, TAPS = d->KH * d->KW, NTN = (TAPS + 3) / 4;
    const int PH = 7 * d->stride + d->KH, PW = 15 * d->stride + d->KW;
    const size_t stage = (size_t)128 * wtr_stride(BN, 1) + (size_t)(PH * PW * 8 + 15) / 16 * 16, red = (size_t)(BN / 16) * (NTN * 256 + 16) * 4;
    pl->lds = stage > red ? stage : red;
    if (pl->lds < 4096) pl->lds = 4096;
    const long long ntiles = pl->kind == 1 ? (long long)d->B * hv_cdiv(d->Ho, 8) * hv_cdiv(d->Wo, 16) : (long long)d->B * hv_cdiv(d->H, 8) * hv_cdiv(d->W, 16);
    constexpr int kWant = 512;
    const long long blocks = pl->kind == 2 ? d->Cin / 64 : 1;
    long long gx = kWant / blocks;
    if (gx < 32) gx = 32;
    pl->gx = (int)(gx < ntiles ? gx : ntiles);
    return true;
}
size_t hv_wgrad_thin_workspace_bytes(const hv_wgrad_desc* d) {
    WThinPlan pl;
    if (!wgrad_thin_plan(d, &pl)) return 0;
    return (size_t)pl.gx * ((size_t)d->Cout * d->KH * d->KW * d->Cin + (d->dbias ? d->Cout : 0)) * sizeof(float);
}
template <int KS, int ST, int BN>
static int launch_wthinx(const WTrK& k, const WThinPlan& pl, const hv_wgrad_desc* d, hipStream_t s) {
    auto kern = wgrad_thinx_kernel<KS, ST, BN>;
    dim3 grid(pl.gx, hv_cdiv(d->Cout, BN), 1);
    WTrK kk = k;
    kk.fold.splits = 0;
    const int fx = hv_carry_blocks((int)grid.y);
    if (fx > 0) { kk.fold = hv_carry; hv_carry_taken = 1; grid.x += fx; }
    hv_path_note = 12;
    HV_KNAME("wgrad_thinx_kernel<%d, %d, %d>", KS, ST, BN);
    HV_TIMING_BEGIN(s);
    hipLaunchKernelGGL(kern, grid, dim3(256), pl.lds, s, kk);
    HV_TIMING_END(s);
    HV_LAUNCH_CHECK();
    return HV_OK;
}
template <int KS, int BN, int IB>
static int launch_wthing(const WTrK& k, const WThinPlan& pl, const hv_wgrad_desc* d, hipStream_t s) {
    auto kern = wgrad_thing_kernel<KS, BN, IB>;
    dim3 grid(pl.gx, hv_cdiv(d->Cin, BN), 1);
    WTrK kk = k;
    kk.fold.splits = 0;
    const int fx = hv_carry_blocks((int)grid.y);
    if (fx > 0) { kk.fold = hv_carry; hv_carry_taken = 1; grid.x += fx; }
    hv_path_note = 12;
    HV_KNAME("wgrad_thing_kernel<%d, %d, %d>", KS, BN, IB);
    HV_TIMING_BEGIN(s);
    hipLaunchKernelGGL(kern, grid, dim3(256), pl.lds, s, kk);
    HV_TIMING_END(s);
    HV_LAUNCH_CHECK();
    return HV_OK;
}
int hv_wgrad_thin(const hv_wgrad_desc* d, int* nslabs, hipStream_t s) {
    WThinPlan pl;
    if (!wgrad_thin_plan(d, &pl)) return HV_ERR_UNSUPPORTED;
    if (!d->workspace || d->workspace_bytes < hv_wgrad_thin_workspace_bytes(d)) return HV_ERR_WORKSPACE;
    WTrK k;
    k.x = reinterpret_cast<const _Float16*>(d->x); k.g = reinterpret_cast<const _Float16*>(d->g); k.slabs = d->workspace;
    k.Hl = d->H; k.Wl = d->W; k.in_shift = 0; k.Wp = d->W;
    k.img_stride = d->H * d->W * d->x_ld; k.x_ld = d->x_ld; k.x_coff = d->x_coff; k.Cin = d->Cin;
    k.Ho = d->Ho; k.Wo = d->Wo; k.Hf = d->Ho; k.Wf = d->Wo; k.g_ld = d->g_ld; k.g_coff = d->g_coff; k.Cout = d->Cout; k.pad = d->pad;
    k.dil = 1;
    if (pl.kind == 1) { k.tiles_x = hv_cdiv(k.Wo, 16); k.tiles_per_sub = k.tiles_x * hv_cdiv(k.Ho, 8); }
    else { k.tiles_x = hv_cdiv(k.Wl, 16); k.tiles_per_sub = k.tiles_x * hv_cdiv(k.Hl, 8); }
    k.tiles_per_img = k.tiles_per_sub; k.ntiles = k.tiles_per_img * d->B;
    k.slab = (long long)d->Cout * d->KH * d->KW * d->Cin;
    k.bias_out = d->dbias ? d->workspace + (long long)pl.gx * k.slab : nullptr;
    k.dbg = 0;
    k.gx = pl.gx;
    k.fold.splits = 0;
    k.x_bytes = (unsigned)((size_t)d->B * k.img_stride * sizeof(_Float16));
    k.g_bytes = (unsigned)((size_t)d->B * d->Ho * d->Wo * d->g_ld * sizeof(_Float16));
    *nslabs = pl.gx;
    if (pl.kind == 1) return launch_wthinx<5, 1, 16>(k, pl, d, s);
    if (pl.kind == 2) return launch_wthing<4, 64, 16>(k, pl, d, s);
    return launch_wthing<3, 16, 8>(k, pl, d, s);
}

int hv_wgrad_tr(const hv_wgrad_desc* d, int* nslabs, hipStream_t s) {
    WTrPlan pl;
    if (!wgrad_tr_plan(d, &pl)) return HV_ERR_UNSUPPORTED;
    const size_t need = hv_wgrad_tr_workspace_bytes(d);
    if (!d->workspace || d->workspace_bytes < need) return HV_ERR_WORKSPACE;
    WTrK k;
    k.x = reinterpret_cast<const _Float16*>(d->x); k.g = reinterpret_cast<const _Float16*>(d->g); k.slabs = d->workspace;
    const int dl = pl.dil;
    k.Hl = d->H / dl; k.Wl = d->W / dl; k.in_shift = d->in_shift; k.Wp = d->W >> d->in_shift;
    k.img_stride = (d->H >> d->in_shift) * k.Wp * d->x_ld; k.x_ld = d->x_ld; k.x_coff = d->x_coff; k.Cin = d->Cin;
    k.Ho = d->Ho / dl; k.Wo = d->Wo / dl; k.Hf = d->Ho; k.Wf = d->Wo; k.g_ld = d->g_ld; k.g_coff = d->g_coff; k.Cout = d->Cout; k.pad = dl > 1 ? 1 : d->pad;
    k.dil = dl;
    k.tiles_x = hv_cdiv(k.Wo, 16); k.tiles_per_sub = k.tiles_x * hv_cdiv(k.Ho, 8); k.tiles_per_img = k.tiles_per_sub * dl * dl; k.ntiles = k.tiles_per_img * d->B;
    k.slab = (long long)d->Cout * d->KH * d->KW * d->Cin;
    k.bias_out = d->dbias ? d->workspace + (long long)pl.gx * k.slab : nullptr;
    k.dbg = 0;
    k.gx = pl.gx;
    k.fold.splits = 0;
#ifdef WT_STAMPS
    if (getenv("HV_WTR_DBG")) k.dbg = atoi(getenv("HV_WTR_DBG"));
#endif
    k.x_bytes = (unsigned)((size_t)d->B * k.img_stride * sizeof(_Float16));
    k.g_bytes = (unsigned)((size_t)d->B * d->Ho * d->Wo * d->g_ld * sizeof(_Float16));
    *nslabs = pl.gx;
#define WTR(KS_, ST_)                                                                                     \
    do {                                                                                                  \
        if (pl.dma) return launch_wtrd<KS_, ST_>(k, pl, d, s);                                            \
        if (pl.BN == 64 && pl.BC == 32) return launch_wtr<KS_, ST_, 64, 32>(k, pl, d, s);                 \
        if (pl.BN == 64 && pl.BC == 16) return launch_wtr<KS_, ST_, 64, 16>(k, pl, d, s);                 \
        if (pl.BN == 32 && pl.BC == 32) return launch_wtr<KS_, ST_, 32, 32>(k, pl, d, s);                 \
        return launch_wtr<KS_, ST_, 32, 16>(k, pl, d, s);                                                 \
    } while (0)
    if (d->KH == 3 && d->stride == 1) WTR(3, 1);
    if (d->KH == 3) WTR(3, 2);
    if (d->stride == 1) WTR(4, 1);
    WTR(4, 2);
#undef WTR
}
```

healthivert-gan_amd/engine.py:

```python
import contextlib
import ctypes
import os
import types

import torch

from . import lib as _lib
from . import ops
from .lib import ptr, stream
from .ops import Act, rup


def precision_note(precision):
    if precision in ('fp16', 'f16'):
        return 'fp16 MFMA operands / fp32 accumulate; activations and gradients stored as fp16 (image tensors, attention scores, weights, statistics fp32)'
    return 'fp32 MFMA (v_mfma_f32_16x16x4_f32), fp32 storage'


SN_MAX_K, SN_MAX_COUT = 4608, 1024


class ConvParams:

    def __init__(self, name, weight, bias, cin, cout, k, cin_fwd=None, cin_wg=None, u=None, v=None, transposed_src=False):
# ... 123 lines not shown
            mf = mb = 7
            if lean and not c.transposed_src:
                mf = (c.use_fwd or 7) | (1 if c.sn else 0)
                mb = c.use_bwd or 7
            rows.append(dict(w_orig=c.weight.data, u=c.u if c.sn else None, v=c.v if c.sn else None, sigma=c.sigma,
                             w_fwd=c.w_fwd if mf & 1 else None, w_bwd=c.w_bwd if mb & 1 else None, w_fwd_h=c.w_fwd_h if mf & 2 else None,
                             w_bwd_h=c.w_bwd_h if mb & 2 else None, w_fwd_t=c.w_fwd_t if mf & 4 else None, w_bwd_t=c.w_bwd_t if mb & 4 else None,
                             Cout=c.cout, Cin=c.cin, taps=c.taps, CinP=c.cin_fwd, CoutF=c.cout, CoutP=c.coutP, CinB=c.cin_fwd, sn=int(c.sn),
                             power_iter=int(pi and c.sn), transposed_src=int(c.transposed_src), w_fwd_t2=c.w_fwd_t2, K2=int(c.split_k or 0)))
        return rows

    def weights_changed(self):
        self.version += 1

    def prep(self, device, power_iter, only_if_stale=False):
        self._ensure(device)
        pi = bool(power_iter)
        table = self.t_prep[pi]
        tset = 'full'
        if LEAN and ops.precision_id(None) == ops.F16:
            tset = tuple((c.use_fwd, c.use_bwd) for c in self.convs)
        if only_if_stale and not pi and PREP_SKIP and self.prepared is not None and self.prepared[0] == self.version and self.prepared[1] in ('full', tset):
            return
        self.prepared = (self.version, tset)
        if LEAN and ops.precision_id(None) == ops.F16:
            key = (self._key, pi, tuple((c.use_fwd, c.use_bwd) for c in self.convs))
            table = self.t_lean.get(key)
            if table is None:
                table = self.t_lean[key] = ops.LayerTable('hv_wprep_layer')
                table.update(self._prep_rows(pi, True), key, device)
        ops.weight_prep(table, max(c.sizes()[0] + c.sizes()[1] for c in self.convs), any_sn=any(c.sn for c in self.convs),
                        any_legacy=any(c.transposed_src for c in self.convs))

    def fold_chain(self):
        h = torch.cuda.current_stream().cuda_stream
        c = self.fold_chains.get(h)
        if c is None:
            c = self.fold_chains[h] = ops.FoldChain(h)
        return c

    def flush_folds(self):
        h = torch.cuda.current_stream().cuda_stream
        for k, c in self.fold_chains.items():
            if k == h:
                c.flush()
            else:
                assert c.pending is None, 'a weight-gradient fold chain of another stream was not flushed before finish_backward()'

    def finish_backward(self, accumulate=False):
        self.flush_folds()
        ops.weight_prep_backward(self.t_bwd[bool(accumulate)], max(c.cout * c.cin * c.taps for c in self.convs), any(c.sn for c in self.convs))


class ConvNode:
    __slots__ = ('p', 'x', 'y', 'k', 's', 'pad', 'd', 'act', 'shift', 'need_dx', 'transposed', 'use_bias', 'dx_c', 'pool_to', 'split', 'full')

    def __init__(self, p, x, y, s=1, pad=0, d=1, act='none', shift=0, need_dx=True, transposed=False, use_bias=True, dx_c=None):
        self.p, self.x, self.y, self.k, self.s, self.pad, self.d = p, x, y, p.k, s, pad, d
        self.act, self.shift, self.need_dx, self.transposed, self.use_bias = act, shift, need_dx, transposed, use_bias
        self.dx_c = dx_c
        self.pool_to = None
        self.split = None
        self.full = None

    def forward_call(self, prec, xn=None, x_raw=None):
        p = self.p
        kw = dict(bias=p.bias if self.use_bias else None, act=self.act, w_h=p.w_fwd_h, precision=prec, cout=p.cout, wuse=(p, 'use_fwd'))
        if self.split is not None and p.w_fwd_t2 is not None and ops.precision_id(prec) == ops.F16:
            low, x1 = self.split
            if low.f16 and self.y.f16 and low.C == p.split_k:
                call = ops.ConvCall(low, p.w_fwd, self.y, self.k, self.s, self.pad, self.d, w_t=p.w_fwd_t2, in_shift=1, cin=p.split_k,
                                    x1=(x1, p.w_fwd, p.split_k, p.taps * p.cin_fwd, p.cin_fwd), **kw)
                if call.supported():
                    return call
        src = self.x if x_raw is None else x_raw
        return ops.ConvCall(Act(src.t, p.cin_fwd, src.coff), p.w_fwd, self.y, self.k, self.s, self.pad, self.d, w_t=p.w_fwd_t, in_shift=self.shift,
                            transposed=self.transposed, xn=xn, **kw)

    def split_forward(self, prec):
        return bool(self.forward_call(prec).d.x1)

    def forward(self, prec, stats=None, xn=None, x_raw=None):
        self.forward_call(prec, xn, x_raw).launch(stats)

    def stats_parts(self, prec):
        return self.forward_call(prec).stats_parts()

    def dx_view(self, book, form):
        a = self.pool_to[0] if form == 'pool_to' else self.x
        g = book.twin(a)
        C = a.C if form == 'pool_to' else self.p.cin_fwd
        return Act(g.t, C if form == 'src' else self.dx_c or C, g.coff)

    def dx_call(self, book, prec, form, dst, accumulate, mul_x=None, bn=None):
        p = self.p
        gy = book.twin(self.y)
        mul = None
        if form == 'pool_to' and self.pool_to[1] != 'none':
            mul = (Act(self.pool_to[0].t, dst.C, self.pool_to[0].coff), self.pool_to[1])
        elif form in ('pool', 'plain') and mul_x:
            mul = (Act(self.x.t, p.cin_fwd, self.x.coff), mul_x)
        return ops.ConvCall(Act(gy.t, p.coutP, gy.coff), p.w_bwd, dst, self.k, self.s, self.pad, self.d, transposed=form != 'src', pool2=form in ('pool', 'pool_to'),
                            accumulate=int(accumulate), precision=prec, w_h=p.w_bwd_h, w_t=p.w_bwd_t, mul=mul, bn=bn, wuse=(p, 'use_bwd'))

    def full_scratch(self):
        if self.full is None:
            x = self.x
            self.full = Act(torch.zeros(x.B, x.H * 2, x.W * 2, x.ld, dtype=x.t.dtype, device=x.t.device), self.p.cin_fwd, 0)
        return self.full

    def pooled(self, book, prec, form='pool', mul_x=None):
        dst = self.dx_view(book, form)
        return self.dx_call(book, prec, form, dst, book.accumulates(dst), mul_x=mul_x).supported()


NO_FORK_STREAMS = set()
_named_streams = {}


def named_stream(name, device, priority=0):
    dev = torch.device(device)
    key = (name, dev.index if dev.index is not None else torch.cuda.current_device(), priority)
    st = _named_streams.get(key)
    if st is None:
        st = _named_streams[key] = torch.cuda.Stream(device=dev, priority=priority)
    return st


PREP_SKIP = os.environ.get('HV_PREP_SKIP', '1') != '0'
LEAN = False


@contextlib.contextmanager
def lean_tables(on=True):
    global LEAN
    prev, LEAN = LEAN, bool(on)
    try:
        yield
    finally:
        LEAN = prev


SERIAL = False


class GradBook:

    def __init__(self):
        self.twins = {}
        self.written = set()
        self.side = None
        self._side_of = None
        self.wgrad_block = WgradBlock()

    def fork(self):
        cur = torch.cuda.current_stream()
        if self.side is None or self._side_of != cur.cuda_stream:
            self.side, self._side_of = named_stream('wgrad-side-of-%x' % cur.cuda_stream, cur.device), cur.cuda_stream
        self.side.wait_stream(cur)
        return self.side

    def join(self):
        if self.side is not None:
            torch.cuda.current_stream().wait_stream(self.side)

    def twin(self, a):
        t = self.twins.get(id(a.t))
        if t is None:
            t = torch.zeros_like(a.t)
            self.twins[id(a.t)] = t
        return Act(t, a.C, a.coff)

    def reset(self):
        self.written.clear()

    def accumulates(self, a):
        return (id(a.t), a.coff, a.C) in self.written

    def mark(self, a):
        acc = self.accumulates(a)
        self.written.add((id(a.t), a.coff, a.C))
        return acc


class WgradBlock:
    __slots__ = ('side', 'collecting', 'queue', 'later', 'pset')

    def __init__(self):
        self.side, self.collecting, self.queue, self.later, self.pset = None, False, [], [], None

    def open(self, pset, device):
        fork = not SERIAL and torch.cuda.current_stream().cuda_stream not in NO_FORK_STREAMS
        self.side = named_stream('generator-wgrad-block', device) if fork else None
        self.collecting, self.queue, self.later, self.pset = fork, [], [], pset

    def add(self, run):
        self.queue.append(run)

    def before_next_block(self, run):
        if self.collecting:
            self.later.append(run)
        else:
            run()

    def launch(self, keep_collecting=False):
        if self.side is None:
            return
        self.side.wait_stream(torch.cuda.current_stream())
        with torch.cuda.stream(self.side):
            for run in self.queue:
                run()
            self.pset.fold_chain().flush()
        self.queue, self.later, self.collecting = self.later, [], keep_collecting

    def join(self):
        assert not self.queue and not self.later, 'WgradBlock.join(): queued weight gradients were never launched'
        if self.side is not None:
            torch.cuda.current_stream().wait_stream(self.side)
        self.side, self.collecting = None, False


def _wgrad(node, p, xin, gfull, accumulate, prec, dbias=None, dbias_accumulate=False):
    chain = p.owner.fold_chain() if p.owner is not None else None
    if node.transposed:
        ops.conv2d_wgrad(gfull, xin, p.dw, node.k, node.s, node.pad, node.d, accumulate=accumulate, precision=prec, chain=chain)
    else:
        ops.conv2d_wgrad(xin, gfull, p.dw, node.k, node.s, node.pad, node.d, in_shift=node.shift, accumulate=accumulate, precision=prec,
                         dbias=dbias, dbias_accumulate=dbias_accumulate, chain=chain)


def conv_backward(node, book, prec, dbias_accumulate=False, wgrad_accumulate=False, wgrad=True, x_wg=None, premultiplied=False,
                  mul_x=None, dbias_done=False, bn=None):
    p = node.p
    assert bn is None or (node.need_dx and not node.transposed and node.pool_to is None and not node.shift), 'conv_backward: bn= needs the plain data-gradient branch'
    gy = book.twin(node.y)
    want_dbias = p.bias is not None and node.use_bias and wgrad and not dbias_done
    fuse_dbias = want_dbias and not node.transposed and p.coutP == p.cout
    if (node.act != 'none' and not premultiplied) or (want_dbias and not fuse_dbias):
        ops.act_backward(gy, node.y, 'none' if premultiplied else node.act, dbias=p.bias.grad if (want_dbias and not fuse_dbias) else None, dbias_accumulate=dbias_accumulate)
    gfull = Act(gy.t, p.coutP, gy.coff)
    if wgrad:
        xs = node.x if x_wg is None else x_wg
        xin = Act(xs.t, p.cin_wg, xs.coff)
        if book.wgrad_block.collecting:
            book.wgrad_block.add(lambda node=node, p=p, xin=xin, gfull=gfull, acc=wgrad_accumulate, db=p.bias.grad if fuse_dbias else None, dba=dbias_accumulate:
                                 _wgrad(node, p, xin, gfull, acc, prec, dbias=db, dbias_accumulate=dba))
        else:
            _wgrad(node, p, xin, gfull, wgrad_accumulate, prec, dbias=p.bias.grad if fuse_dbias else None, dbias_accumulate=dbias_accumulate)
    if not node.need_dx:
        return
    if node.transposed:
        form = 'src'
    elif node.pool_to is not None and node.pooled(book, prec, 'pool_to'):
        form = 'pool_to'
    elif node.shift:
        form = 'pool' if node.pooled(book, prec, 'pool', mul_x) else 'full'
    else:
        form = 'plain'
    if form == 'full':
        assert not mul_x
        full = node.full_scratch()
        node.dx_call(book, prec, 'full', full, False).launch()
        gx = node.dx_view(book, 'plain')
        ops.copy_channels(full, gx, mode=3, accumulate=book.mark(gx))
    else:
        dst = node.dx_view(book, form)
        node.dx_call(book, prec, form, dst, book.mark(dst), mul_x=mul_x, bn=bn).launch()


_branch_streams = {}


def branch_stream():
    if SERIAL:
        return None
    cur = torch.cuda.current_stream()
    if cur.cuda_stream in NO_FORK_STREAMS:
        return None
    key = cur.device.index
    st = _branch_streams.get(key)
    if st is None:
        st = _branch_streams[key] = named_stream('generator-branch', cur.device)
        NO_FORK_STREAMS.add(st.cuda_stream)
    return st


def chain_link(n, nxt, book, prec):
    if not (nxt is not None and n.need_dx and not n.transposed and nxt.act != 'none'
            and n.x.t is nxt.y.t and n.x.coff == nxt.y.coff and n.p.cin_fwd <= nxt.y.t.shape[-1] - nxt.y.coff):
        return False
    return not n.shift or n.pooled(book, prec, 'pool', nxt.act)


def conv_backward_chain(nodes, book, prec, premultiplied_first=False, stop_before=None):
    pre = premultiplied_first
    for i, n in enumerate(nodes):
        nxt = nodes[i + 1] if i + 1 < len(nodes) else stop_before
        link = chain_link(n, nxt, book, prec)
        conv_backward(n, book, prec, premultiplied=pre, mul_x=nxt.act if link else None)
        pre = link


CA_GRAM = True
CA_GEMM = True


def _bgemm(A, B, C, M, N, K, batch, alpha=1.0, colscale=None, b_split=0):
    _lib.get().call('hv_bgemm_nt_h' if C.dtype == torch.float16 else 'hv_bgemm_nt', ptr(A), int(A.dtype == torch.float16), K, ctypes.c_longlong(M * K), ptr(B), int(B.dtype == torch.float16), K,
                    ctypes.c_longlong(N * K), ptr(C), N, ctypes.c_longlong(M * N), M, N, K, batch, ctypes.c_float(alpha), ptr(colscale),
                    ctypes.c_longlong(N if colscale is not None else 0), int(b_split), stream())


def attention_route(prec, f, C, h, w):
    if not (CA_GEMM and ops.precision_id(prec) == ops.F16 and (9 * C) % 32 == 0 and (h * w) % 32 == 0 and C % 4 == 0):
        return 'conv'
    return 'gram' if CA_GRAM and f.f16 and C == 64 and w in (32, 64) and f.ld % 8 == 0 and f.coff == 0 else 'gemm'


CA_TABLES = dict(conv=dict(forward='fd wp wpT raw rawT A f32 out32', backward='AT dOrawT dwp dout32 df32'),
                 gemm=dict(forward='fd wp wp_h raw_h rawT_h A_h O', backward='wpT_h dwp dOraw_h dOrawT_h AT_h df32'),
                 gram=dict(forward='fd_h fdT_h q raw_h rawT_h A_h O', backward='dOraw_h dOrawT_h AT_h df32'),
                 shared=dict(forward='S0 S1 norm rnorm mm argmax', per_sample='mm_b', backward='dA dS1 dS0 Gs coef'))


class AttentionPlan:

    def __init__(self, B, H, W, C, device, img_hw, scale=10.0, fuse=True):
        self.B, self.H, self.W, self.C, self.dims, self.device = B, H, W, C, (B, H, W, C), device
        self.h, self.w, self.L = h, w, L = H // 2, W // 2, (H // 2) * (W // 2)
        assert h == w and H % 2 == 0, "contextual attention expects a square, even-sized feature map"
        self.img_hw, self.scale, self.fuse = img_hw, scale, fuse
        self.fused_adjoint = fuse and h == 32 and w == 32
        self.unused = set() if fuse and not self.fused_adjoint else {'dS0'} if fuse else {'S1', 'dS0'}
        f32, f16 = torch.float32, torch.float16
        LL, fmap, vec, tab, tabT = (f32, (B, h, w, L)), (f32, (B, H, W, C)), (f32, (B, L)), (f16, (B, L, 16 * C)), (f16, (B, 16 * C, L))
        self.spec = dict(S0=LL, S1=LL, dS0=LL, A=LL, AT=LL, dA=LL, dS1=LL, Gs=LL, f32=fmap, out32=fmap, dout32=fmap, df32=fmap, norm=vec, rnorm=vec, q=vec, mm_b=vec, mm=(f32, (L,)),
                         argmax=(torch.int32, (B * L,)), coef=(f32, (33 * B, L)), fd=(f32, (B, h, w, C)), dwp=(f32, (B, h, w, 9 * C)), wp=(f32, (B, L, 9 * C)), wpT=(f32, (B, 9 * C, L)),
                         raw=(f32, (B, L, 16 * C)), rawT=(f32, (B, C, 16 * L)), dOrawT=(f32, (B, C, 16 * L)), wp_h=(f16, (B, L, 9 * C)), wpT_h=(f16, (B, 9 * C, L)), raw_h=tab, rawT_h=tabT,
                         O=tab, dOraw_h=tab, dOrawT_h=tabT, A_h=(f16, (B, L, L)), AT_h=(f16, (B, L, L)), fd_h=(f16, (B, L, C)), fdT_h=(f16, (B, C, L)))
        self.owned, self.sets, self.route, self.last = {}, {}, None, None
        self.buffers('shared', 'forward')

    gemm = property(lambda self: self.route in ('gemm', 'gram'))
    gram = property(lambda self: self.route == 'gram')
    nbytes = lambda self: sum(t.numel() * t.element_size() for t in self.owned.values())

    def buffers(self, route, stage, skip=()):
        r = self if route == 'shared' else self.sets.setdefault(route, types.SimpleNamespace())
        for n in CA_TABLES[route][stage].split():
            if (route, n) in self.owned or n in self.unused or n in skip:
                continue
            if torch.cuda.is_current_stream_capturing():
                raise RuntimeError('AttentionPlan%s: %s route, %s would allocate %s inside a stream capture -- run it eagerly once first' % (self.dims, route, stage, n))
            t = self.owned[route, n] = torch.zeros(*self.spec[n][1], dtype=self.spec[n][0], device=self.device)
            setattr(r, n, Act(t) if t.dim() == 4 else t)
        return r

    def forward(self, f, mask_img, out, prec, want_argmax=False, per_sample_mask=False):
        route, self.route, self.last = attention_route(prec, f, self.C, self.h, self.w), None, None
        L_, B, L, (patches, scores, paste) = _lib.get(), self.B, self.L, self.steps[route][:3]
        r = self.buffers(route, 'forward', skip=[n for n, a in (('f32', f), ('out32', out)) if not a.f16])
        mm, mm_stride = (self.buffers('shared', 'per_sample').mm_b, L) if per_sample_mask else (self.mm, 0)
        patches(self, r, f)
        mask = ('hv_ca_mask_batched', ptr(mask_img), B, ctypes.c_longlong(self.img_hw[0] * self.img_hw[1])) if per_sample_mask else ('hv_ca_mask', ptr(mask_img))
        L_.call(*mask, *self.img_hw, self.h, self.w, ptr(mm), stream())
        scores(self, r, prec)
        if self.fuse:
            L_.call('hv_ca_fuse', ptr(self.S0.t), ptr(self.S1.t), B, self.h, self.w, 0, stream())
        s = self.S1 if self.fuse else self.S0
        if route != 'conv':
            L_.call('hv_ca_softmax_f16', ptr(s.t), ptr(mm), ctypes.c_longlong(mm_stride), ptr(r.A_h), B, L, ctypes.c_float(self.scale), ptr(self.argmax) if want_argmax else None, stream())
        elif per_sample_mask:
            L_.call('hv_ca_softmax_batched', ptr(s.t), ptr(mm), ctypes.c_longlong(mm_stride), ptr(r.A.t), B, L, ctypes.c_float(self.scale), ptr(self.argmax) if want_argmax else None, stream())
        else:
            L_.call('hv_ca_softmax', ptr(s.t), ptr(mm), ptr(r.A.t), B, L, ctypes.c_float(self.scale), ptr(self.argmax) if want_argmax else None, stream())
        paste(self, r, out, prec)
        self.route, self.last = route, (ops.precision_id(prec), per_sample_mask)

    def backward(self, dout, df, accumulate, prec):
        if self.route is None or self.last != (ops.precision_id(prec), False):
            raise RuntimeError('AttentionPlan%s: backward(prec=%s) does not follow the last forward: route %s, (precision, per-sample mask) %s' % (self.dims, prec, self.route, self.last))
        L_, B, L, (paste_grad, score_grad) = _lib.get(), self.B, self.L, self.steps[self.route][3:]
        r = self.buffers(self.route, 'backward', skip=[n for n, a in (('dout32', dout), ('df32', df)) if not a.f16])
        self.buffers('shared', 'backward')
        df_user, df = df, r.df32 if df.f16 else df
        paste_grad(self, r, dout, df, accumulate and df is df_user, prec)
        name, A = ('hv_ca_softmax_backward', r.A.t) if self.route == 'conv' else ('hv_ca_softmax_backward_f16', r.A_h)
        L_.call(name, ptr(self.dA.t), ptr(A), ptr(self.mm), ptr(self.dS1.t), B, L, ctypes.c_float(self.scale), stream())
        if self.fused_adjoint:
            L_.call('hv_ca_fuse_backward_prep', ptr(self.dS1.t), ptr(self.S0.t), ptr(self.norm), ptr(self.rnorm), ptr(self.Gs.t), ptr(self.coef), B, self.h, self.w, stream())
        else:
            if self.fuse:
                L_.call('hv_ca_fuse', ptr(self.dS1.t), ptr(self.dS0.t), B, self.h, self.w, 1, stream())
            L_.call('hv_ca_score_backward_prep', ptr((self.dS0 if self.fuse else self.dS1).t), ptr(self.S0.t), ptr(self.norm), ptr(self.rnorm), ptr(self.Gs.t), ptr(self.coef), B, L, stream())
        score_grad(self, r, df, prec)
        if df is not df_user:
            ops.copy_channels(df, df_user, mode=0, accumulate=bool(accumulate))

    def _conv_patches(self, r, f):
        if f.f16:
            ops.copy_channels(f, r.f32, mode=0)
# ... 61 lines not shown
```

healthivert-gan_amd/models/inpaint_networks.py:

```python
import contextlib
import os

import torch
import torch.nn as nn
from torch.nn.utils import spectral_norm as _sn_register

from ._backend import engine as E
from ._backend import lib as _lib
from ._backend import ops
ptr, stream = _lib.ptr, _lib.stream
Act = ops.Act

_ACTS = ('relu', 'elu', 'lrelu', 'prelu', 'selu', 'tanh', 'sigmoid', 'none')


class Conv2dBlock(nn.Module):

    def __init__(self, input_dim, output_dim, kernel_size, stride, padding=0, conv_padding=0, dilation=1, weight_norm='sn',
                 norm='none', activation='relu', pad_type='zero', transpose=False):
        super().__init__()
        assert pad_type in ('reflect', 'replicate', 'zero', 'none'), "Unsupported padding type: {}".format(pad_type)
        assert norm in ('bn', 'in', 'none'), "Unsupported normalization: {}".format(norm)
        assert weight_norm in ('sn', 'wn', 'none'), "Unsupported normalization: {}".format(weight_norm)
        assert activation in _ACTS, "Unsupported activation: {}".format(activation)
# ... 257 lines not shown
        c = gen.cnum
        self.B, self.H, self.W, self.dev = B, H, W, device
        dt = ops.storage_dtype(gen.precision)
        self.book = E.GradBook()
        levels, views = _buffers(c)
        a = self.a = {n: Act(torch.zeros(B, H >> lv, W >> lv, ops.cpad(C), dtype=dt, device=device), C, 0) for lv, bufs in enumerate(levels) for n, C in bufs.items()}
        a.update({n: a[src].slice(coff, C) for n, (src, coff, C) in views.items()})
        for n in _IMAGES:
            setattr(self, n, torch.zeros(B, 1, H, W, dtype=torch.float32, device=device))
            a[n] = Act(getattr(self, n).view(B, H, W, 1))
        self.node, self.chain = {}, {}
        for gname, chains in _layers(c).items():
            for chain, rows in chains.items():
                for layer, src, dst, s, pad, d, act, *flags in rows:
                    self.node['%s.%s' % (gname, layer)] = E.ConvNode(gen._pset_convs['%s.%s' % (gname, layer)], a[src], a[dst], s, pad, d, act, **(flags[0] if flags else {}))
                self.chain[gname, chain] = tuple(self.node['%s.%s' % (gname, row[0])] for row in rows)
        self.up = {n: _UpConcat(self.node[n], self.node[producer], cam_mode) for n, (_, producer, cam_mode) in _UP_CONCAT.items()}
        self.head = {n: _Head(node, self.book) for n, node in self.node.items() if node.p.cout == 1}
        self.c_pool, self.f_pool = torch.zeros(B, 4 * c, device=device), torch.zeros(B, 4 * c, device=device)
        self.pred1, self.pred2 = torch.zeros(B, 1, device=device), torch.zeros(B, 1, device=device)
        self.attn = gen.fine_generator.contextul_attention.plan(B, H // 4, W // 4, 4 * c, device, (H, W))
        self.d_xs1_total, self.d_cs_total = torch.zeros_like(self.x_stage1), torch.zeros_like(self.coarse_seg)
        self.mask_img = None
        self.generation = 0

    def forward(self, prec, gname, *chains):
        for chain in chains:
            for n in self.chain[gname, chain]:
                n.forward(prec)


class Generator(nn.Module):
    def __init__(self, config, use_cuda):
        super().__init__()
        self.input_dim = config['input_dim']
        self.cnum = config['ngf']
        self.use_cuda = use_cuda
        if self.input_dim != 1:
            raise NotImplementedError("Generator HIP path: input_dim == 1 (single-channel CT slices)")
        self.coarse_generator = CoarseGenerator(self.input_dim, self.cnum, self.use_cuda)
        self.fine_generator = FineGenerator(self.input_dim, self.cnum, self.use_cuda)
        self.precision = None
        self._plans = {}
        self._pset = None
        self._eval_graphs = {}
        self.use_graph = os.environ.get('HV_GRAPH', '1') != '0'
        self._pset_convs = None
        self.time_fine = None
        self._fine_graph_keep = None

    def paramset(self):
        if self._pset is None:
            convs = {}
            for gname in ('coarse_generator', 'fine_generator'):
                g = getattr(self, gname)
                for n, m in g.named_children():
                    if isinstance(m, Conv2dBlock):
                        convs['%s.%s' % (gname, n)] = m.params('%s.%s' % (gname, n), cin_fwd=ops.cpad(m.cin))
            chains = _layers(self.cnum)['coarse_generator']
            for n, (chain, _, _) in _UP_CONCAT.items():
                k2 = chains[chain][0][-1]['dx_c']
                if k2 % 32 == 0 and convs[n].cin == k2 + 1:
                    convs[n].split_k = k2
            self._pset_convs = convs
            cg, fg = self.coarse_generator, self.fine_generator
            self._pset = E.ParamSet(convs.values(), [cg.fc_height.weight, cg.fc_height.bias, fg.fc_height.weight, fg.fc_height.bias])
        return self._pset

    def _plan(self, B, H, W, device):
        key = (B, H, W, str(device), ops.precision_id(self.precision))
        if key not in self._plans:
            if H % 8 or W % 8 or H != W:
                raise NotImplementedError("Generator HIP path expects square inputs with a side divisible by 8")
            self.paramset()
            self._plans[key] = _GenPlan(self, B, H, W, device)
        return self._plans[key]

    def run_forward(self, x, mask, CAM, slice_ratio, training=None, per_sample_mask=False):
        _lib.require_gpu(x, mask, CAM)
        training = self.training if training is None else training
        prec = ops.precision_id(self.precision)
        B, _, H, W = x.shape
        dev = x.device
        P = self._plan(B, H, W, dev)
        self.paramset().prep(dev, power_iter=training)
        x = x.contiguous().float(); mask = mask.contiguous().float(); CAM = CAM.contiguous().float()
        ratio = slice_ratio.to(device=dev, dtype=torch.float64).contiguous()
        P.mask_img = mask
        cg, cgn, a = self.coarse_generator, 'coarse_generator', P.a
        cam = Act(CAM.view(B, H, W, 1))
        ops.gen_input(x, None, mask, ratio, a['c_in'], 0)
        P.forward(prec, cgn, 'enc')
        ops.gap_fc_sigmoid(a['c10'], cg.fc_height.weight, cg.fc_height.bias, P.c_pool, P.pred1)
        P.forward(prec, cgn, 'mid')
        P.up['coarse_generator.conv20'].forward(cam, prec)
        P.forward(prec, cgn, 'dec20')
        P.up['coarse_generator.conv19'].forward(cam, prec)
        P.forward(prec, cgn, 'dec19', 'heads')
        tf = self.time_fine
        if tf is not None and not torch.cuda.is_current_stream_capturing():
            tf.append((torch.cuda.Event(enable_timing=True), torch.cuda.Event(enable_timing=True)))
            tf[-1][0].record()
        else:
            tf = None
        self._fine_forward(P, x, mask, ratio, prec, per_sample_mask)
        if tf is not None:
            tf[-1][1].record()
        return P

    def _fine_forward(self, P, x, mask, ratio, prec, per_sample_mask=False):
        fg, fgn, a = self.fine_generator, 'fine_generator', P.a
        ops.gen_input(x, P.coarse_seg, mask, ratio, a['f_in'], 1)
        side = E.branch_stream()
        main = torch.cuda.current_stream()
        if side is not None:
            side.wait_stream(main)
        with (torch.cuda.stream(side) if side is not None else contextlib.nullcontext()):
            P.forward(prec, fgn, 'pm_in', 'pm')
            P.attn.forward(a['p6'], mask, a['ca'], prec, want_argmax=True, per_sample_mask=per_sample_mask)
            P.forward(prec, fgn, 'pm_out')
        P.forward(prec, fgn, 'dilated')
        if side is not None:
            main.wait_stream(side)
        P.forward(prec, fgn, 'merge')
        ops.gap_fc_sigmoid(a['a11'], fg.fc_height.weight, fg.fc_height.bias, P.f_pool, P.pred2)
        P.forward(prec, fgn, 'trunk')
        ops.copy_channels(a['x_stage1'], a['cat17'].slice(a['a16'].C, 1), mode=0)
        P.forward(prec, fgn, 'heads')

    def fine_forward_graph(self, P, x, mask, slice_ratio):
        prec = ops.precision_id(self.precision)
        ratio = slice_ratio.to(device=x.device, dtype=torch.float64).contiguous()
        x = x.contiguous().float(); mask = mask.contiguous().float()
        g = torch.cuda.CUDAGraph()
        with torch.cuda.graph(g, stream=E.named_stream('capture', x.device), capture_error_mode='thread_local'):
            self._fine_forward(P, x, mask, ratio, prec)
        self._fine_graph_keep = (x, mask, ratio)
        return g

    def run_backward(self, P, d_coarse_seg, d_fine_seg, d_x_stage1, d_x_stage2, d_pred1, d_pred2):
        prec = ops.precision_id(self.precision)
        B, H, W = P.B, P.H, P.W
        book, a, N, head = P.book, P.a, P.node, P.head
        book.reset()
        cg, fg = self.coarse_generator, self.fine_generator
        coarse, fine = (lambda chain: reversed(P.chain['coarse_generator', chain])), (lambda chain: reversed(P.chain['fine_generator', chain]))
        up19, up20 = P.up['coarse_generator.conv19'], P.up['coarse_generator.conv20']
        zero = lambda t, ref: torch.zeros_like(ref) if t is None else t.contiguous().float()
        d_fine_seg, d_x_stage2 = zero(d_fine_seg, P.fine_seg), zero(d_x_stage2, P.x_stage2)
        d_coarse_seg, d_x_stage1 = zero(d_coarse_seg, P.coarse_seg), zero(d_x_stage1, P.x_stage1)
        d_pred1, d_pred2 = zero(d_pred1, P.pred1), zero(d_pred2, P.pred2)
        wg = book.wgrad_block
        wg.open(self.paramset(), d_x_stage2.device)
        wg.before_next_block(lambda: up19.materialise(prec))
        wg.before_next_block(lambda: up20.materialise(prec))
        head['fine_generator.allconv17'].backward(d_x_stage2, book, prec)
        head['fine_generator.allconv18'].backward(d_fine_seg, book, prec)
        ops.add_channels(Act(d_x_stage1.view(B, H, W, 1)), book.twin(a['cat17']).slice(a['a16'].C, 1), Act(P.d_xs1_total.view(B, H, W, 1)))
        allconv11, allconv12 = N['fine_generator.allconv11'], N['fine_generator.allconv12']
        E.conv_backward_chain(list(fine('trunk')), book, prec, stop_before=allconv11)
        pre11 = E.chain_link(allconv12, allconv11, book, prec)
        ops.gap_fc_sigmoid_backward(d_pred2, P.pred2, P.f_pool, fg.fc_height.weight, book.twin(a['a11']),
                                    fg.fc_height.weight.grad, fg.fc_height.bias.grad, mul=(a['a11'], allconv11.act) if pre11 else None)
        E.conv_backward(allconv11, book, prec, premultiplied=pre11, mul_x='elu')
        side = E.branch_stream()
        main = torch.cuda.current_stream()
        pmconv1, pmconv2 = N['fine_generator.pmconv1'], N['fine_generator.pmconv2_downsample']
        if side is not None:
            side.wait_stream(main)
        with (torch.cuda.stream(side) if side is not None else contextlib.nullcontext()):
            E.conv_backward_chain(list(fine('pm_out')), book, prec, premultiplied_first=True)
            gp6 = book.twin(a['p6'])
            P.attn.backward(book.twin(a['ca']), gp6, book.mark(gp6), prec)
            E.conv_backward_chain([*fine('pm'), *(fine('pm_in') if side is None else ())], book, prec, stop_before=None if side is None else pmconv1)
            if side is not None:
                self.paramset().fold_chain().flush()
        E.conv_backward_chain(list(fine('dilated')), book, prec, premultiplied_first=True)
        if side is not None:
            main.wait_stream(side)
            E.conv_backward(pmconv1, book, prec, premultiplied=E.chain_link(pmconv2, pmconv1, book, prec))
        ops.add_channels(Act(d_coarse_seg.view(B, H, W, 1)), book.twin(a['f_in']).slice(1, 1), Act(P.d_cs_total.view(B, H, W, 1)))
        wg.launch(keep_collecting=True)
        head['coarse_generator.conv17'].backward(P.d_xs1_total, book, prec, mul_x='elu')
        head['coarse_generator.conv18'].backward(P.d_cs_total, book, prec, mul_x='elu')
        p19 = up19.backward(coarse('dec19'), book, prec, True)
        p20 = up20.backward(coarse('dec20'), book, prec, p19)
        wg.launch()
        conv10, conv11 = N['coarse_generator.conv10_atrous'], N['coarse_generator.conv11']
        E.conv_backward_chain(list(coarse('mid')), book, prec, premultiplied_first=p20, stop_before=conv10)
        pre10 = E.chain_link(conv11, conv10, book, prec)
        ops.gap_fc_sigmoid_backward(d_pred1, P.pred1, P.c_pool, cg.fc_height.weight, book.twin(a['c10']),
                                    cg.fc_height.weight.grad, cg.fc_height.bias.grad, mul=(a['c10'], conv10.act) if pre10 else None)
        E.conv_backward_chain(list(coarse('enc')), book, prec, premultiplied_first=pre10)
        wg.join()
        self.paramset().finish_backward(accumulate=False)
        self.paramset().attach_grads()

    def forward(self, x, mask, CAM, slice_ratio):
        if not torch.is_tensor(slice_ratio):
            slice_ratio = torch.as_tensor(slice_ratio, dtype=torch.float64).reshape(-1)
        if self.use_graph and not self.training and not torch.is_grad_enabled() and ops.timer() is None and x.is_cuda:
            P = self._eval_replay(x, mask, CAM, slice_ratio)
        else:
            P = self.run_forward(x, mask, CAM, slice_ratio)
        outs = (P.coarse_seg, P.fine_seg, P.x_stage1, P.x_stage2, P.pred1, P.pred2)
        flow = offsets_to_flow(P.attn.argmax, P.B, P.attn.h, P.attn.w, 2)
        if torch.is_grad_enabled() and any(p.requires_grad for p in self.parameters()):
            anchor = next(p for p in self.parameters() if p.requires_grad)
            o = _GeneratorFn.apply(anchor, self, P, *outs)
        else:
            o = tuple(t.clone() for t in outs)
        return o[0], o[1], o[2], o[3], flow, o[4], o[5]

    def _eval_replay(self, x, mask, CAM, slice_ratio):
        key = (tuple(x.shape), x.device.index, next(self.parameters()).data_ptr())
        ent = self._eval_graphs.get(key)
        if ent is None:
            dev = x.device
            static = [x.detach().to(dev, torch.float32).contiguous().clone(), mask.detach().to(dev, torch.float32).contiguous().clone(),
                      CAM.detach().to(dev, torch.float32).contiguous().clone(), slice_ratio.detach().to(dev, torch.float64).contiguous().clone()]
            self.run_forward(*static)
            torch.cuda.synchronize(dev)
            g = torch.cuda.CUDAGraph()
            try:
                with torch.cuda.graph(g, stream=E.named_stream('capture', dev), capture_error_mode='thread_local'):
                    P = self.run_forward(*static)
            except RuntimeError:
                self.use_graph = False
                torch.cuda.synchronize(dev)
                return self.run_forward(x, mask, CAM, slice_ratio)
            if len(self._eval_graphs) >= 8:
                self._eval_graphs.clear()
            ent = self._eval_graphs[key] = (g, static, P)
        g, static, P = ent
        for dst, src in zip(static, (x, mask, CAM, slice_ratio)):
            dst.copy_(src, non_blocking=True)
        g.replay()
        return P


class _GeneratorFn(torch.autograd.Function):

    @staticmethod
    def forward(ctx, anchor, gen, plan, *outs):
        ctx.gen, ctx.plan = gen, plan
        plan.generation = ctx.generation = plan.generation + 1
        return tuple(t.clone() for t in outs)

    @staticmethod
    def backward(ctx, g_cs, g_fs, g_x1, g_x2, g_p1, g_p2):
        if ctx.plan.generation != ctx.generation:
            raise RuntimeError("Generator: a later forward pass of the same shape overwrote this pass's activations before its backward ran "
                               "(one activation plan per input shape); run backward before the next forward")
        S = ops.grad_scale(ctx.gen.precision)
        sc = (lambda t: None if t is None else t * S) if S != 1.0 else (lambda t: t)
        ctx.gen.run_backward(ctx.plan, sc(g_cs), sc(g_fs), sc(g_x1), sc(g_x2), sc(g_p1), sc(g_p2))
        ops.scale_inplace(ctx.gen.paramset().flat_grad, 1.0 / S)
        return (None,) * 9
```

healthivert-gan_amd/ops.py:

```python
import ctypes
import os

import torch

from . import lib as _lib
from .lib import ACT, NORM, F16, F32, ptr, stream

_PRECISION = {'fp32': F32, 'f32': F32, 'fp16': F16, 'f16': F16}


_TIMER = None


def timer():
    return _TIMER


def set_timer(t):
    global _TIMER
    _TIMER = t


def default_precision():
    return _PRECISION[os.environ.get('HV_PRECISION', 'fp32').lower()]
# ... 78 lines not shown
        return Act(x.view(B, H, W, 1))
    ld = C if CP is None else CP
    a = Act.empty(B, H, W, C, x.device, ld=ld, zero=ld != C, dtype=dtype)
    _lib.get().call('hv_nchw_to_nhwc', ptr(x), ptr(a.t), a.f16, B, C, H, W, ld, 0, stream())
    return a


class _Workspace:
    def __init__(self):
        self.buf = {}
        self.retired = []

    def get(self, nbytes, device, slot=0):
        key = (device, slot)
        b = self.buf.get(key)
        if b is None or b.numel() < nbytes:
            if b is not None:
                self.retired.append(b)
            b = torch.empty(max(int(nbytes), 1 << 20), dtype=torch.uint8, device=device)
            self.buf[key] = b
        return b


WS = _Workspace()


def _ws(nbytes, device, slot=0):
    b = WS.get(nbytes + 64, device, (slot, torch.cuda.current_stream(device).cuda_stream))
    return b, ctypes.c_size_t(b.numel())


def conv_out_size(n, k, stride, pad, dil):
    return (n + 2 * pad - dil * (k - 1) - 1) // stride + 1


_PROBES = {}


class ConvCall:
    __slots__ = ('d', 'x', 'y', 'wuse')

    def __init__(self, x, w, y, k, stride=1, pad=0, dil=1, bias=None, act='none', transposed=False, in_shift=0, alpha=1.0, accumulate=0, ch_scale=None,
                 w_bstride=0, ch_scale_bstride=0, precision=None, cin=None, cout=None, w_h=None, mul=None, w_t=None, pool2=False, x1=None, wuse=None, bn=None,
                 xn=None):
        L = _lib.get()
        self.d = d = L.hv_conv_desc()
        self.x, self.y, self.wuse = x, y, wuse
        kh, kw = (k, k) if isinstance(k, int) else k
        d.x = ptr(x.t).value
        d.B, d.H, d.W = x.B, x.H << in_shift, x.W << in_shift
        d.in_shift, d.x_ld, d.x_coff, d.Cin = in_shift, x.ld, x.coff, (x.C if cin is None else cin)
        d.w = ptr(w).value
        d.w_bstride = w_bstride
        d.Cout, d.KH, d.KW, d.stride, d.pad, d.dil, d.transposed = (y.C if cout is None else cout), kh, kw, stride, pad, dil, int(transposed)
        d.bias = None if bias is None else ptr(bias).value
        d.ch_scale = None if ch_scale is None else ptr(ch_scale).value
        d.ch_scale_bstride = ch_scale_bstride
        d.alpha, d.act, d.accumulate = alpha, ACT[act], int(accumulate)
        d.y = ptr(y.t).value
        d.Ho, d.Wo, d.y_ld, d.y_coff = (y.H << 1 if pool2 else y.H), (y.W << 1 if pool2 else y.W), y.ld, y.coff
        d.pool2 = int(bool(pool2))
        if x1 is not None:
            xa, wfull, ch, w1_row, w1_tap = x1
            assert xa.C == 1 and xa.H == d.H and xa.W == d.W
            d.x1, d.x1_f16, d.x1_ld, d.x1_coff = ptr(xa.t).value, xa.f16, xa.ld, xa.coff
            d.w1, d.w1_row, d.w1_tap = ptr(wfull).value + 4 * ch, w1_row, w1_tap
        d.precision = precision_id(precision)
        d.w_f16 = None if w_h is None else ptr(w_h).value
        d.w_f16_tiled = None if (w_t is None or w_h is None) else ptr(w_t).value
        d.x_f16, d.y_f16 = x.f16, y.f16
        if mul is not None:
            m, mact = mul
            d.mul_src, d.mul_ld, d.mul_coff, d.mul_act, d.mul_f16 = ptr(m.t).value, m.ld, m.coff, ACT[mact], m.f16
        if bn is not None:
            bx, bstat, bgroups, bpart = bn
            assert bx.f16 == y.f16 and bx.H == y.H and bx.W == y.W and bx.B == y.B
            d.bn_x, d.bn_x_ld, d.bn_x_coff = ptr(bx.t).value, bx.ld, bx.coff
            d.bn_stats, d.bn_groups = ptr(bstat).value, int(bgroups)
            if bpart is not None:
                d.bstats = ptr(bpart).value
        if xn is not None:
            nstat, ngam, nbet, ngroups, nact, nout = xn
            d.xn_stats, d.xn_groups, d.xn_act = ptr(nstat).value, int(ngroups), ACT[nact]
            if ngam is not None:
                d.xn_gamma, d.xn_beta = ptr(ngam).value, ptr(nbet).value
            if nout is not None:
                assert nout.f16 and nout.B == x.B and nout.H == x.H and nout.W == x.W
                d.xn_out, d.xn_out_ld, d.xn_out_coff = ptr(nout.t).value, nout.ld, nout.coff
        if d.Cout == 1:
            need = L.size('hv_conv2d_workspace_bytes', ctypes.byref(d))
            if need:
                b, _ = _ws(need, x.t.device, slot=1)
                d.workspace, d.workspace_bytes = ptr(b).value, b.numel()

    def _probe(self, fn):
        key = (fn, bytes(self.d))
        if key not in _PROBES:
            _PROBES[key] = _lib.get().size(fn, ctypes.byref(self.d))
        return _PROBES[key]

    def supported(self):
        return bool(self._probe('hv_conv2d_supported'))

    def stats_parts(self):
        return self._probe('hv_conv2d_stats_parts')

    def bstats_parts(self):
        return self._probe('hv_conv2d_bstats_parts')

    def launch(self, stats=None):
        L, d, x, y = _lib.get(), self.d, self.x, self.y
        if stats is not None:
            d.stats = ptr(stats).value
        if _TIMER is not None:
            taps = d.KH * d.KW if not d.transposed else max(1, (d.KH * d.KW) // (d.stride * d.stride))
            flops = 2.0 * y.B * y.H * y.W * d.Cout * taps * d.Cin
            wbytes = (2 if (d.w_f16 and d.precision == F16 and not d.w_bstride) else 4) * d.Cout * d.KH * d.KW * d.Cin * (x.B if d.w_bstride else 1)
            xb, yb = (2 if x.f16 else 4), (2 if y.f16 else 4)
            nbytes = xb * x.B * x.H * x.W * d.Cin + yb * y.B * y.H * y.W * d.Cout * (2 if d.accumulate else 1) + wbytes + \
                ((2 if d.mul_f16 else 4) * y.B * y.H * y.W * d.Cout if d.mul_src else 0)
            _TIMER.wrap(('conv', x.B, d.H, d.W, d.Cin, d.Cout, d.KH, d.stride, d.dil, d.transposed), flops,
                        lambda: L.call('hv_conv2d', ctypes.byref(d), stream()), nbytes)
        else:
            L.call('hv_conv2d', ctypes.byref(d), stream())
        if self.wuse is not None:
            setattr(self.wuse[0], self.wuse[1], getattr(*self.wuse) | int(L.cdll.hv_last_weight_tables()))
        return y


def conv2d(*args, stats=None, **kw):
    return ConvCall(*args, **kw).launch(stats)


def conv2d_supported(*args, **kw):
    return ConvCall(*args, **kw).supported()


def conv2d_stats_parts(*args, **kw):
    return ConvCall(*args, **kw).stats_parts()


def conv2d_bstats_parts(*args, **kw):
    return ConvCall(*args, **kw).bstats_parts()


def pool2_ok(g, y_low, k, stride, pad, dil, precision, w_h, w_t, cout=None, w=None):
    if w_h is None or w_t is None or precision_id(precision) != F16 or g.H != 2 * y_low.H or g.W != 2 * y_low.W:
        return False
    return conv2d_supported(g, w_h if w is None else w, Act(y_low.t, y_low.C if cout is None else cout, y_low.coff), k, stride, pad, dil, transposed=True,
                            pool2=True, precision=precision, w_h=w_h, w_t=w_t)


class FoldChain:
    __slots__ = ('pending', 'slot', 'stream')

    def __init__(self, stream_handle):
        self.pending, self.slot, self.stream = None, 0, stream_handle

    def flush(self):
        if self.pending is not None:
            assert torch.cuda.current_stream().cuda_stream == self.stream, 'FoldChain.flush() on another stream than its weight gradients'
            f, self.pending = self.pending, None
            _lib.get().call('hv_wgrad_fold_now', ctypes.byref(f), stream())


FOLD_CHAIN = True


def conv2d_wgrad(x, g, dw, k, stride=1, pad=0, dil=1, in_shift=0, accumulate=False, precision=None, cin=None, cout=None, dbias=None,
                 dbias_accumulate=False, chain=None):
    L = _lib.get()
    d = L.hv_wgrad_desc()
    kh, kw = (k, k) if isinstance(k, int) else k
    d.x = ptr(x.t).value
    d.B, d.H, d.W, d.in_shift = x.B, x.H << in_shift, x.W << in_shift, in_shift
    d.x_ld, d.x_coff, d.Cin = x.ld, x.coff, (x.C if cin is None else cin)
    d.g = ptr(g.t).value
    d.Ho, d.Wo, d.g_ld, d.g_coff, d.Cout = g.H, g.W, g.ld, g.coff, (g.C if cout is None else cout)
    d.KH, d.KW, d.stride, d.pad, d.dil = kh, kw, stride, pad, dil
    d.dw = ptr(dw).value
    d.accumulate = int(accumulate)
    d.precision = precision_id(precision)
    d.dbias = None if dbias is None else ptr(dbias).value
    d.dbias_accumulate = int(dbias_accumulate)
    d.x_f16, d.g_f16 = x.f16, g.f16
    d.workspace, d.workspace_bytes = None, 0
    if chain is not None and not FOLD_CHAIN:
        chain = None
    need = L.size('hv_conv2d_wgrad_workspace_bytes', ctypes.byref(d))
    fold = None
    if chain is not None:
        assert torch.cuda.current_stream(x.t.device).cuda_stream == chain.stream, 'a FoldChain belongs to one stream'
        if chain.pending is not None:
            d.carry = ctypes.pointer(chain.pending)
        if need:
            b, _ = _ws(need, x.t.device, slot=('fold-chain', chain.slot))
            chain.slot ^= 1
            d.workspace, d.workspace_bytes = ptr(b).value, b.numel()
            fold = L.hv_wgrad_fold()
            d.pending = ctypes.pointer(fold)
    elif need:
        b, _ = _ws(need, x.t.device)
        d.workspace, d.workspace_bytes = ptr(b).value, b.numel()
    if _TIMER is not None:
        flops = 2.0 * g.B * g.H * g.W * d.Cout * kh * kw * d.Cin
        nbytes = (2 if x.f16 else 4) * x.B * x.H * x.W * d.Cin + (2 if g.f16 else 4) * g.B * g.H * g.W * d.Cout + 4 * d.Cout * kh * kw * d.Cin
        _TIMER.wrap(('wgrad', x.B, d.H, d.W, d.Cin, d.Cout, kh, stride, dil, 0), flops,
                    lambda: L.call('hv_conv2d_wgrad', ctypes.byref(d), stream()), nbytes)
    else:
        L.call('hv_conv2d_wgrad', ctypes.byref(d), stream())
    if chain is not None:
        chain.pending = fold if (fold is not None and fold.nslabs > 0) else None
    return dw


class LayerTable:

    def __init__(self, struct_name):
        self.struct_name = struct_name
        self.key = None
        self.dev = None
        self.n = 0

    def update(self, rows, key, device):
        if key == self.key:
            return
        L = _lib.get()
        S = getattr(L, self.struct_name)
        arr = (S * len(rows))()
        for i, r in enumerate(rows):
            for f, v in r.items():
                if torch.is_tensor(v):
                    v = ptr(v).value
                setattr(arr[i], f, v)
        raw = bytes(arr)
        host = torch.frombuffer(bytearray(raw), dtype=torch.uint8)
        self.dev = host.to(device)
        self.key, self.n = key, len(rows)

    def ptr(self):
        return ptr(self.dev)


def tiled_elems(rows, taps, K):
    return _lib.get().size('hv_weight_tiled_elems', int(rows), int(taps), int(K))


def tile_weights(w_h, rows, taps, K):
    n = tiled_elems(rows, taps, K)
    if not n:
        return None
    out = torch.empty(n, dtype=torch.float16, device=w_h.device)
    _lib.get().call('hv_weight_tile_f16', ptr(w_h), ptr(out), int(rows), int(taps), int(K), stream())
    return out


def weight_prep(table, max_numel, any_sn=True, any_legacy=True):
    _lib.get().call('hv_weight_prep2', ctypes.cast(table.ptr(), ctypes.POINTER(_lib.get().hv_wprep_layer)), table.n,
                    ctypes.c_longlong(max_numel), int(any_sn), int(any_legacy), stream())


def weight_prep_backward(table, max_numel, any_sn):
    _lib.get().call('hv_weight_prep_backward', ctypes.cast(table.ptr(), ctypes.POINTER(_lib.get().hv_wprep_bwd_layer)), table.n,
                    ctypes.c_longlong(max_numel), int(any_sn), stream())




def act_backward(dy, y, act, dbias=None, dbias_accumulate=False):
    L = _lib.get()
    need = L.size('hv_act_backward_workspace_bytes', ctypes.c_longlong(dy.npix), dy.C) if dbias is not None else 0
    b, nb = _ws(need, dy.t.device)
    L.call('hv_act_backward', ptr(dy.t), dy.f16, ptr(y.t), y.f16, ctypes.c_longlong(dy.npix), dy.C, dy.ld, dy.coff, y.ld, y.coff, ACT[act],
           ptr(dbias), int(dbias_accumulate), ptr(b), nb, stream())


def head_seed_backward(seed, y, carrier, act, dbias=None, dbias_accumulate=False):
    L = _lib.get()
    npix = carrier.npix
    need = L.size('hv_head_seed_workspace_bytes', ctypes.c_longlong(npix)) if dbias is not None else 0
    b, nb = _ws(need, carrier.t.device)
    L.call('hv_head_seed_backward', ptr(seed), ptr(y.t), y.f16, y.ld, y.coff, ptr(carrier.t), ctypes.c_longlong(npix), ACT[act], ptr(dbias),
           int(dbias_accumulate), ptr(b), nb, stream())


def copy_channels(src, dst, mode=0, accumulate=False):
    assert src.C == dst.C
    _lib.get().call('hv_copy_channels', ptr(src.t), src.f16, ptr(dst.t), dst.f16, dst.B, dst.H, dst.W, dst.C, src.ld, src.coff, dst.ld, dst.coff,
                    mode, int(accumulate), stream())


def add_channels(a, b, dst):
    assert a.C == b.C == dst.C and a.npix == b.npix == dst.npix
    _lib.get().call('hv_add_channels', ptr(a.t), a.f16, a.ld, a.coff, ptr(b.t), b.f16, b.ld, b.coff, ptr(dst.t), dst.f16, dst.ld, dst.coff,
                    ctypes.c_longlong(dst.npix), dst.C, stream())


def fill(t, value=0.0):
    _lib.get().call('hv_fill', ptr(t), ctypes.c_longlong(t.numel()), ctypes.c_float(value), stream())


def axpy(y, x, a=1.0):
    assert y.numel() == x.numel()
    _lib.get().call('hv_axpy', ptr(y), ptr(x), ctypes.c_longlong(y.numel()), ctypes.c_float(a), stream())


def gen_input(x, seg, mask, ratio, dst, order):
    _lib.get().call('hv_gen_input', ptr(x), ptr(seg), ptr(mask), ptr(ratio), ptr(dst.t), dst.f16, dst.B, dst.H, dst.W, dst.ld, order, stream())


def gap_fc_sigmoid(x, fc_w, fc_b, pooled, pred):
    L = _lib.get()
    need = L.size('hv_gap_fc_workspace_bytes', x.B, x.C)
    b, nb = _ws(need, x.t.device)
    L.call('hv_gap_fc_sigmoid', ptr(x.t), x.f16, x.B, x.H * x.W, x.C, x.ld, ptr(fc_w), ptr(fc_b), ptr(pooled), ptr(pred), ptr(b), nb, stream())


def gap_fc_sigmoid_backward(dpred, pred, pooled, fc_w, dx, dw, db, accumulate=False, mul=None):
    m, mact = mul if mul is not None else (None, 'none')
    _lib.get().call('hv_gap_fc_sigmoid_backward', ptr(dpred), ptr(pred), ptr(pooled), ptr(fc_w), ptr(dx.t), dx.f16, dx.B, dx.H * dx.W, dx.C,
                    dx.ld, ptr(dw), ptr(db), int(accumulate), None if m is None else ptr(m.t), 0 if m is None else m.f16, 0 if m is None else m.ld,
                    ACT[mact], stream())


def sobel(img, out=None):
    out = torch.empty_like(img) if out is None else out
    B, _, H, W = img.shape
    _lib.get().call('hv_sobel', ptr(img), ptr(out), B, H, W, stream())
    return out


def gan_loss(z, target_is_real, mode='vanilla', loss=None, loss_weight=1.0, loss_accumulate=False, dz=None, grad_weight=1.0):
    m = {'vanilla': 0, 'lsgan': 1}[mode]
    L = _lib.get()
    n = z.numel()
    if n >= 4096:
        b, nb = _ws(L.size('hv_gan_loss_workspace_bytes', ctypes.c_longlong(n)), z.device, slot=2)
        L.call('hv_gan_loss_ws', ptr(z), ctypes.c_longlong(n), int(bool(target_is_real)), m, ctypes.c_float(loss_weight), ptr(loss),
               int(loss_accumulate), ctypes.c_float(grad_weight), ptr(dz), ptr(b), nb, stream())
        return
    L.call('hv_gan_loss', ptr(z), ctypes.c_longlong(n), int(bool(target_is_real)), m, ctypes.c_float(loss_weight),
           ptr(loss), int(loss_accumulate), ctypes.c_float(grad_weight), ptr(dz), stream())


_TICKETS = {}


def _ticket(device):
    key = (str(device), torch.cuda.current_stream(device).cuda_stream)
    t = _TICKETS.get(key)
    if t is None:
        t = _TICKETS[key] = torch.zeros(16, dtype=torch.int32, device=device)
    return t


def gan_loss_pair(z0, real0, loss0, carrier0, z1=None, real1=True, loss1=None, carrier1=None, mode='vanilla', loss_weight=1.0, loss_accumulate=False,
                  grad_weight=1.0, dbias=None, dbias_accumulate=False):
    n0, n1 = z0.numel(), (0 if z1 is None else z1.numel())
    for c, n in ((carrier0, n0), (carrier1, n1)):
        assert c is None or (c.f16 and c.ld == 4 and c.coff == 0 and c.npix == n)
    L = _lib.get()
    b, nb = _ws(L.size('hv_gan_loss_head_pair_workspace_bytes', ctypes.c_longlong(n0), ctypes.c_longlong(n1)), z0.device, slot=2)
    L.call('hv_gan_loss_head_pair', ptr(z0), ctypes.c_longlong(n0), int(bool(real0)), ptr(loss0), ptr(carrier0.t), ptr(z1), ctypes.c_longlong(n1),
           int(bool(real1)), ptr(loss1), None if carrier1 is None else ptr(carrier1.t), {'vanilla': 0, 'lsgan': 1}[mode], ctypes.c_float(loss_weight),
           int(loss_accumulate), ctypes.c_float(grad_weight), ptr(dbias), int(dbias_accumulate), ptr(b), nb,
           ptr(_ticket(z0.device)), stream())
# ... 62 lines not shown
```

healthivert-gan_amd/profiler.py:

```python
import ctypes

import torch

from . import lib as _lib
from . import ops


class KernelTimer:
    def __init__(self):
        self.records = []
        self.paths = {}
        self.bytes = {}
        self.names = {}
        self.only = None
        self.active = False
        self.pair_us = 0.0

    def calibrate(self, n=200):
        torch.cuda.synchronize()
        pairs = []
        for _ in range(n):
            s, e = torch.cuda.Event(enable_timing=True), torch.cuda.Event(enable_timing=True)
            s.record(); e.record()
            pairs.append((s, e))
        torch.cuda.synchronize()
        v = sorted(s.elapsed_time(e) * 1e3 for s, e in pairs)
        self.pair_us = v[len(v) // 20]
        return self.pair_us

    def wrap(self, key, flops, launch, nbytes=0):
        self.bytes[key] = nbytes
        if not self.active or (self.only is not None and key not in self.only):
            return launch()
        s, e = torch.cuda.Event(enable_timing=True), torch.cuda.Event(enable_timing=True)
        L = _lib.get().cdll
        s.record(); e.record()
        L.hv_set_kernel_timing(ctypes.c_void_p(s.cuda_event), ctypes.c_void_p(e.cuda_event))
        r = launch()
        self.paths[key] = L.hv_last_kernel_path()
        self.names[key] = (L.hv_last_kernel_name() or b'').decode()
        self.records.append((key, flops, s, e))
        return r

    def enable(self, only=None):
        self.records, self.only, self.active = [], (set(only) if only else None), True
        ops.set_timer(self)

    def disable(self):
        self.active = False
        ops.set_timer(None)

    def summary(self):
        torch.cuda.synchronize()
        agg = {}
        for key, flops, s, e in self.records:
            a = agg.setdefault(key, [0.0, 0, flops])
            a[0] += max(s.elapsed_time(e) - self.pair_us * 1e-3, 1e-4)
            a[1] += 1
        return agg

    def by_kernel(self):
        out = {}
        for key, (ms, n, flops) in self.summary().items():
            a = out.setdefault(self.names.get(key) or describe(key, self.paths.get(key)), [0.0, 0, 0.0, []])
            a[0] += ms; a[1] += n; a[2] += flops * n; a[3].append(key)
        return out

    def dominant(self):
        bk = self.by_kernel()
        if not bk:
            return None
        name, a = max(bk.items(), key=lambda kv: kv[1][0])
        return name, a[3]

    def dominant_mfma(self, peak_tflops):
        ridge = peak_tflops * 1e12 / (HBM_PEAK_GBS * 1e9)
        best = None
        for name, (ms, n, flops, keys) in self.by_kernel().items():
            nbytes = sum(self.bytes.get(k, 0) * self.summary()[k][1] for k in keys)
            if nbytes and flops / nbytes >= ridge and (best is None or ms > best[0]):
                best = (ms, name, keys)
        return (best[1], best[2]) if best else None

    def roofline(self, precision, peak_tflops, total_ms=None, name=None):
        bk = self.by_kernel()
        if not bk or (name is not None and name not in bk):
            return None
        if name is None:
            name = max(bk.items(), key=lambda kv: kv[1][0])[0]
        ms, n, flops, keys = bk[name]
        agg = self.summary()
        achieved = flops / (ms * 1e-3) / 1e12
        ridge = peak_tflops * 1e12 / (HBM_PEAK_GBS * 1e9)

        def shape_row(k):
            avg_s = agg[k][0] / agg[k][1] * 1e-3
            tf, gbs = agg[k][2] / avg_s / 1e12, self.bytes.get(k, 0) / avg_s / 1e9
            hbm = bool(self.bytes.get(k)) and agg[k][2] / self.bytes[k] < ridge
            return {'shape': describe(k, self.paths.get(k), self.names.get(k)), 'launches': agg[k][1], 'avg_us': round(avg_s * 1e6, 2), 'tflops': round(tf, 1),
                    'algorithmic_gbs': round(gbs, 1), 'bound': 'hbm' if hbm else 'mfma',
                    'frac': round(gbs / HBM_PEAK_GBS if hbm else tf / peak_tflops, 4)}
        shapes = [shape_row(k) for k in sorted(keys, key=lambda k: -agg[k][0])]
        nbytes = sum(self.bytes.get(k, 0) * agg[k][1] for k in keys)
        out = {'kernel': name, 'launches': n, 'avg_us': round(ms / n * 1e3, 2), 'avg_us_events': round(ms / n * 1e3 + self.pair_us, 2),
               'event_pair_overhead_us': round(self.pair_us, 2), 'gflop_per_launch': round(flops / n / 1e9, 3),
               'algorithmic_mb_per_launch': round(nbytes / n / 1e6, 2), 'shapes': shapes, 'traffic': None}
        if nbytes and flops / nbytes < ridge:
            gbs = nbytes / (ms * 1e-3) / 1e9
            out.update(bound='hbm', achieved=round(gbs, 1), peak=HBM_PEAK_GBS, unit='GB/s', frac=round(gbs / HBM_PEAK_GBS, 4),
                       achieved_tflops=round(achieved, 2), flop_per_byte=round(flops / nbytes, 1), ridge_flop_per_byte=round(ridge, 1))
        else:
            out.update(bound='mfma', achieved=round(achieved, 2), peak=peak_tflops, unit='TFLOP/s', frac=round(achieved / peak_tflops, 4),
                       flop_per_byte=round(flops / nbytes, 1) if nbytes else None, ridge_flop_per_byte=round(ridge, 1))
        return out


HBM_PEAK_GBS = 8000.0

KERNEL_NAMES = {0: 'conv_igemm_kernel', 1: 'narrow_fwd_kernel', 2: 'conv_halo_kernel', 3: 'conv_halo2_kernel', 4: 'thin1_fwd_kernel', 5: 'head_gemm_kernel', 6: 'conv_s2t_kernel',
                7: 'conv_lf_kernel', 8: 'conv_g4_kernel', 9: 'thin_dgrad_kernel', 10: 'wgrad_kernel', 11: 'wgrad_halo_kernel', 12: 'wgrad_tr_kernel', 13: 'wgrad_trd_kernel', 14: 'conv_px_kernel'}


def describe(key, path=None, kname=None):
    kind, B, H, W, cin, cout, k, s, d, tr = key
    name = kname or KERNEL_NAMES.get(path, {'conv': 'conv_igemm_kernel', 'wgrad': 'wgrad_kernel'}[kind])
    if name.startswith('void '):
        name = name[5:]
    name = name.split('(')[0]
    return '%s %s B%d %dx%d Cin%d->Cout%d k%d s%d d%d' % (name, 'transposed' if tr else 'forward', B, H, W, cin, cout, k, s, d)
```

include/hvgan.h:

```cpp
#ifndef HVGAN_H
#define HVGAN_H
#include <stddef.h>
#include <stdint.h>

#ifdef __cplusplus
extern "C" {
#endif

#define HV_OK 0
#define HV_ERR_ARG (-1)
#define HV_ERR_UNSUPPORTED (-2)
#define HV_ERR_WORKSPACE (-3)

enum { HV_F32 = 0, HV_F16 = 1 };
enum { HV_ACT_NONE = 0, HV_ACT_ELU = 1, HV_ACT_RELU = 2, HV_ACT_LRELU = 3, HV_ACT_SIGMOID = 4, HV_ACT_CLAMP = 5 };
enum { HV_NORM_NONE = 0, HV_NORM_BATCH = 1, HV_NORM_INSTANCE = 2 };

int hv_version(void);
const char* hv_arch(void);
int hv_last_kernel_path(void);
const char* hv_last_kernel_name(void);
int hv_set_kernel_timing(void* ev_start, void* ev_stop);
int hv_set_s2t_mode(int mode);

typedef struct {
    const float* x; int B, H, W;
    int in_shift; int x_ld, x_coff, Cin;
    const float* w; long long w_bstride;
    int Cout, KH, KW, stride, pad, dil, transposed;
    const float* bias;
    const float* ch_scale;
    long long ch_scale_bstride;
    float alpha; int act; int accumulate;
    float* y; int Ho, Wo, y_ld, y_coff;
    int precision;
    const void* w_f16;
    const void* w_f16_tiled;
    const float* mul_src; int mul_ld, mul_coff, mul_act;
    int x_f16, y_f16, mul_f16;
    void* workspace; size_t workspace_bytes;
    float* stats;
    const void* x1;
    int x1_f16, x1_ld, x1_coff;
    const float* w1; int w1_row, w1_tap;
    int pool2;
    const void* bn_x; int bn_x_ld, bn_x_coff;
    const float* bn_stats; int bn_groups;
    float* bstats;
    const float* xn_stats; const float* xn_gamma; const float* xn_beta; int xn_groups, xn_act;
    void* xn_out; int xn_out_ld, xn_out_coff;
} hv_conv_desc;
int hv_conv2d(const hv_conv_desc* d, void* stream);
size_t hv_conv2d_bstats_parts(const hv_conv_desc* d);
size_t hv_conv2d_workspace_bytes(const hv_conv_desc* d);
size_t hv_conv2d_stats_parts(const hv_conv_desc* d);
int hv_last_weight_tables(void);
int hv_conv2d_supported(const hv_conv_desc* d);

typedef struct {
    const float* slabs; float* dw; long long numel; int nslabs; int accumulate;
    const float* bias_slabs; float* dbias; int Cout; int dbias_accumulate;
} hv_wgrad_fold;

typedef struct {
    const float* x; int B, H, W; int in_shift; int x_ld, x_coff, Cin;
    const float* g; int Ho, Wo, g_ld, g_coff, Cout;
    int KH, KW, stride, pad, dil;
    float* dw; int accumulate;
    float* workspace; size_t workspace_bytes;
    int precision;
    int x_f16, g_f16;
    float* dbias; int dbias_accumulate;
    hv_wgrad_fold* pending;
    const hv_wgrad_fold* carry;
} hv_wgrad_desc;
int hv_wgrad_fold_now(const hv_wgrad_fold* fold , void* stream);
size_t hv_conv2d_wgrad_workspace_bytes(const hv_wgrad_desc* d);
int hv_conv2d_wgrad(const hv_wgrad_desc* d, void* stream);

typedef struct {
    const float* w_orig;
    float* u; float* v;
    float* sigma;
    float* w_fwd;
    float* w_bwd;
    void* w_fwd_h; void* w_bwd_h;
    void* w_fwd_t; void* w_bwd_t;
    int Cout, Cin, taps, CinP, CoutF, CoutP, CinB;
    int sn, power_iter, transposed_src;
    void* w_fwd_t2; int K2;
} hv_wprep_layer;
int hv_weight_prep(const hv_wprep_layer* d_layers, int n_layers, long long max_numel, void* stream);
int hv_weight_prep2(const hv_wprep_layer* d_layers, int n_layers, long long max_numel, int any_sn, int any_legacy, void* stream);

size_t hv_weight_tiled_elems(int rows, int taps, int K);
int hv_weight_tile_f16(const void* w_f16, void* w_tiled, int rows, int taps, int K, void* stream);

typedef struct {
    const float* dw_ohwi; const float* w_fwd; const float* u; const float* v; const float* sigma;
    float* dw_orig; int Cout, Cin, taps, CinP, sn, transposed_src, accumulate;
} hv_wprep_bwd_layer;
int hv_weight_prep_backward(const hv_wprep_bwd_layer* d_layers, int n_layers, long long max_numel, int any_sn, void* stream);

size_t hv_head_seed_workspace_bytes(long long npix);
int hv_head_seed_backward(const float* seed, const void* y, int y_f16, int y_ld, int y_coff, void* carrier_f16, long long npix, int act, float* dbias,
                          int dbias_accumulate, float* workspace, size_t workspace_bytes, void* stream);

int hv_act_backward(void* dy, int dy_f16, const void* y, int y_f16 , long long npix, int C, int dy_ld, int dy_coff,
                    int y_ld, int y_coff, int act, float* dbias, int dbias_accumulate, float* workspace, size_t workspace_bytes, void* stream);
size_t hv_act_backward_workspace_bytes(long long npix, int C);

typedef struct {
    const void* x; void* y; int B, HW, C; int x_ld, x_coff, y_ld, y_coff;
    int norm; int training; float eps, momentum;
    const float* gamma; const float* beta; float* running_mean; float* running_var; long long* num_batches_tracked;
    float* stats; int act; int post_sigmoid;
    float* workspace; size_t workspace_bytes;
    int groups;
    int f16;
    const float* partials; int n_partials;
} hv_norm_desc;
size_t hv_norm_workspace_bytes(int B, int HW, int C);
int hv_norm_act_forward(const hv_norm_desc* d, void* stream);
typedef struct {
    const void* dy; const void* y; const void* x; void* dx; int B, HW, C;
    int dy_ld, dy_coff, y_ld, y_coff, x_ld, x_coff, dx_ld, dx_coff;
    int norm; int training; const float* gamma; const float* stats;
    int act; int post_sigmoid;
    float* dgamma; float* dbeta; int param_accumulate;
    float* workspace; size_t workspace_bytes;
    int groups;
    int f16;
    const float* partials; int n_partials;
} hv_norm_bwd_desc;
int hv_norm_act_backward(const hv_norm_bwd_desc* d, void* stream);

int hv_nchw_to_nhwc(const float* src, void* dst, int dst_f16, int B, int C, int H, int W, int dst_ld, int dst_coff, void* stream);
int hv_nhwc_to_nchw(const void* src, int src_f16, float* dst, int B, int C, int H, int W, int src_ld, int src_coff, int accumulate, void* stream);
int hv_copy_channels(const void* src, int src_f16, void* dst, int dst_f16, int B, int H, int W, int C, int src_ld, int src_coff, int dst_ld,
                     int dst_coff, int mode, int accumulate, void* stream);
int hv_add_channels(const void* a, int a_f16, int a_ld, int a_coff, const void* b, int b_f16, int b_ld, int b_coff, void* dst, int dst_f16, int dst_ld,
                    int dst_coff, long long npix, int C, void* stream);

int hv_gen_input(const float* x, const float* seg, const float* mask, const double* slice_ratio, void* dst, int dst_f16,
                 int B, int H, int W, int CP, int order, void* stream);
size_t hv_gap_fc_workspace_bytes(int B, int C);
int hv_gap_fc_sigmoid(const void* x, int x_f16, int B, int HW, int C, int x_ld, const float* fc_w, const float* fc_b,
                      float* pooled , float* pred , float* workspace, size_t workspace_bytes, void* stream);
int hv_gap_fc_sigmoid_backward(const float* dpred, const float* pred, const float* pooled, const float* fc_w,
                               void* dx, int dx_f16, int B, int HW, int C, int dx_ld, float* dw, float* db, int accumulate,
                               const void* mul_src, int mul_f16, int mul_ld, int mul_act, void* stream);

int hv_ca_patches(const void* f, int f_f16 , int B, int H, int W, int C, int f_ld, float* fd, float* wp, float* wpT, float* norm,
                  float* rnorm, void* stream);
int hv_ca_raw_patches(const float* f, int B, int H, int W, int C, int f_ld, float* raw, float* rawT, void* stream);
int hv_ca_mask(const float* mask, int Himg, int Wimg, int h, int w, float* mm, void* stream);
int hv_ca_mask_batched(const float* mask, int B, long long mask_bstride, int Himg, int Wimg, int h, int w, float* mm, void* stream);
int hv_ca_fuse(const float* S, float* out, int B, int h, int w, int adjoint, void* stream);
int hv_ca_softmax(const float* S, const float* mm, float* A, int B, int L, float scale, int* argmax, void* stream);
int hv_ca_softmax_batched(const float* S, const float* mm, long long mm_bstride, float* A, int B, int L, float scale, int* argmax,
                          void* stream);
int hv_ca_flow(const int* argmax, int B, int h, int w, int up, float* flow, void* stream);
int hv_ca_softmax_backward(const float* dA, const float* A, const float* mm, float* dS, int B, int L, float scale, void* stream);
int hv_transpose_batched(const float* src, float* dst, int B, int R, int C, void* stream);
int hv_bgemm_nt(const void* A, int a_f16, int lda, long long strideA, const void* B, int b_f16, int ldb, long long strideB, float* C, int ldc,
                long long strideC, int M, int N, int K, int batch, float alpha, const float* colscale, long long strideS, int b_split, void* stream);
int hv_ca_fold(const float* src, void* dst, int dst_f16 , int B, int H, int W, int C, int dst_ld, float alpha, int accumulate, void* stream);
int hv_bgemm_nt_h(const void* A, int a_f16, int lda, long long strideA, const void* B, int b_f16, int ldb, long long strideB, void* C_h, int ldc,
                  long long strideC, int M, int N, int K, int batch, float alpha, const float* colscale, long long strideS, int b_split, void* stream);
int hv_ca_fold_h(const void* src_h, void* dst, int dst_f16, int B, int H, int W, int C, int dst_ld, float alpha, int accumulate, void* stream);
int hv_ca_raw_patches_f16(const void* f, int f_f16 , int B, int H, int W, int C, int f_ld, void* raw_h, void* rawT_h, void* stream);
int hv_transpose_batched_f16(const float* src, void* dst_h, int B, int R, int C, void* stream);
int hv_ca_patches_h(const void* f, int f_f16, int B, int H, int W, int C, int f_ld, float* fd, float* wp, void* wp_h, float* norm, float* rnorm,
                    void* stream);
int hv_ca_softmax_f16(const float* S, const float* mm, long long mm_bstride , void* A_h, int B, int L, float scale,
                      int* argmax, void* stream);
int hv_ca_softmax_backward_f16(const float* dA, const void* A_h, const float* mm, float* dS, int B, int L, float scale, void* stream);
int hv_transpose_batched_h2h(const void* src_h, void* dst_h, int B, int R, int C, void* stream);
int hv_ca_score_backward_prep(const float* dS, const float* S0, const float* norm, const float* rnorm, float* Gs, float* coef,
                              int B, int L, void* stream);
int hv_ca_fuse_backward_prep(const float* dS1, const float* S0, const float* norm, const float* rnorm, float* Gs, float* coef, int B, int h, int w,
                             void* stream);
int hv_ca_patches_backward(const float* dwp, const float* wp, const float* coef, float* df, int B, int H, int W, int C,
                           int df_ld, int accumulate, void* stream);

int hv_ca_gram_down(const void* f, int f_f16, int B, int H, int W, int C, int f_ld, void* fd_h, void* fdT_h, float* q, void* stream);
int hv_ca_gram_scores(const void* fd_h, const float* q, int B, int h, int w, int C, float* S0, float* norm, float* rnorm, void* stream);
int hv_ca_gram_backward(const float* Gs, const void* fd_h, const void* fdT_h, const float* coef, int B, int h, int w, int C, float* df, int df_ld,
                        void* stream);

int hv_sobel(const float* img, float* out, int B, int H, int W, void* stream);
typedef struct {
    const float* real_B; const float* mask; const float* x_stage1; const float* x_stage2;
    const float* fine_seg; const float* coarse_seg; const float* pred1; const float* pred2;
    const long long* height; const long long* x1; const long long* x2; const long long* maxheight;
    float* fake_B; float* fake_B_coarse; float* fake_B_local; float* real_B_local;
    float* fine_bin; float* coarse_bin; float* pred1_h; float* pred2_h; int* rows;
    int B, H, W, half_band;
} hv_postg_desc;
int hv_post_generator(const hv_postg_desc* d, void* stream);
int hv_shrm_composite(const float* gen, const float* real, const float* pred_scaled, const long long* height,
                      const long long* x1, const long long* x2, float* out, int* rows, int B, int H, int W, void* stream);

int hv_gan_loss(const float* z, long long n, int target_is_real, int mode, float loss_weight, float* loss, int loss_accumulate,
                float grad_weight, float* dz, void* stream);
size_t hv_gan_loss_workspace_bytes(long long n);
int hv_gan_loss_ws(const float* z, long long n, int target_is_real, int mode, float loss_weight, float* loss, int loss_accumulate,
                   float grad_weight, float* dz, void* workspace, size_t workspace_bytes, void* stream);

size_t hv_gan_loss_head_workspace_bytes(long long n);
int hv_gan_loss_head(const float* z, long long n, int target_is_real, int mode, float loss_weight, float* loss, int loss_accumulate, float grad_weight,
                     float* dz, void* carrier_f16, float* dbias, int dbias_accumulate, void* workspace, size_t workspace_bytes, void* stream);

size_t hv_gan_loss_head_pair_workspace_bytes(long long n0, long long n1);
int hv_gan_loss_head_pair(const float* z0, long long n0, int real0, float* loss0, void* carrier0_f16, const float* z1, long long n1, int real1, float* loss1,
                          void* carrier1_f16, int mode, float loss_weight, int loss_accumulate, float grad_weight, float* dbias, int dbias_accumulate,
                          void* workspace, size_t workspace_bytes, unsigned* ticket, void* stream);

typedef struct {
    const float* fake_B; const float* fake_B_coarse; const float* real_B; const float* mask;
    const float* fine_seg; const float* coarse_seg; const float* real_B_mask; const float* normal_vert;
    const float* fake_edges; const float* real_edges; const float* pred1_h; const float* pred2_h;
    const long long* height; const long long* maxheight;
    float lambda_L1;
    float* losses; float* d_fake_B; float* d_fake_B_coarse; float* d_fine_seg; float* d_coarse_seg;
    float* d_pred1; float* d_pred2;
    int B, H, W;
    float* workspace; size_t workspace_bytes;
    float grad_scale;
    const float* gan_terms; int n_gan_terms; float* loss_G_GAN; float* loss_G;
    const float* add_d_fake_B;
// ... 259 lines not shown
```

Measured before the change: 2573 slices/s.

## Batch same-shape 3x3 weight-gradient layers into one grouped wgrad_tr launch

Adds a grouped weight-gradient kernel that runs up to 8 same-shape 3x3 stride-1 Cout=64 layers (for example the atrous mid-block convs) in a single launch, with a fixed chunk count per layer. Pending split-K folds from earlier layers ride along in spare blocks, and a grouped fold kernel reduces several folds in one launch. The Python engine collects eligible layers on the side stream and flushes them as groups. The aim is fewer small launches and better GPU fill for narrow wgrad layers. In exchange the chunk count is fixed, grid.y is padded across layers, and the fold ordering logic becomes more complex.

```diff
diff --git a/healthivert-gan_amd/csrc/conv_igemm.hip b/healthivert-gan_amd/csrc/conv_igemm.hip
--- a/healthivert-gan_amd/csrc/conv_igemm.hip
+++ b/healthivert-gan_amd/csrc/conv_igemm.hip
@@ -29,6 +29,9 @@
 int hv_wgrad_halo(const hv_wgrad_desc* d, int* nslabs, hipStream_t s);
 size_t hv_wgrad_tr_workspace_bytes(const hv_wgrad_desc* d);
 int hv_wgrad_tr(const hv_wgrad_desc* d, int* nslabs, hipStream_t s);
+size_t hv_wgrad_trg_workspace_bytes(const hv_wgrad_desc* d, int chunks);
+bool hv_wgrad_trg_ok(const hv_wgrad_desc* descs, int n, int chunks);
+int hv_wgrad_trg(const hv_wgrad_desc* descs, int n, int chunks, int* nslabs, const HvFold* folds, int nfold, hipStream_t s);
 int hv_wgrad_thin(const hv_wgrad_desc* d, int* nslabs, hipStream_t s);
 size_t hv_wgrad_thin_workspace_bytes(const hv_wgrad_desc* d);
 int hv_conv2d_narrow(const hv_conv_desc* d, hipStream_t s);
@@ -859,6 +862,34 @@
     return HV_OK;
 }
 
+struct HvFoldSet { HvFold f[8]; };
+__global__ __launch_bounds__(256) void wgrad_fold_group_kernel(const HvFoldSet a) {
+    __shared__ float4 sh[256];
+    hv_fold_blocks(a.f[blockIdx.y], (int)blockIdx.x, (int)gridDim.x, sh);
+}
+extern "C" int hv_wgrad_fold_group(const hv_wgrad_fold* folds, int n, void* stream) {
+    if (!folds || n < 0) return HV_ERR_ARG;
+    for (int i0 = 0; i0 < n; i0 += 8) {
+        HvFoldSet a = {};
+        int m = 0, gx = 0;
+        for (int i = i0; i < n && i < i0 + 8; ++i) {
+            const hv_wgrad_fold& f = folds[i];
+            if (f.nslabs <= 0) continue;
+            if (!f.slabs || !f.dw || f.numel <= 0 || (f.numel & 3)) return HV_ERR_ARG;
+            for (int j = 0; j < m; ++j)
+                if (a.f[j].dw == f.dw) return HV_ERR_ARG;
+            a.f[m++] = HvFold{f.slabs, f.dw, f.numel, f.nslabs, f.accumulate, f.dbias ? f.bias_slabs : nullptr, f.dbias, f.Cout, f.dbias_accumulate};
+            const int Q = 256 / (f.nslabs <= 16 ? 4 : f.nslabs <= 64 ? 16 : 32);
+            const int blocks = hv_cdiv(f.numel / 4, Q) + (f.dbias ? hv_cdiv(f.Cout, Q) : 0);
+            if (blocks > gx) gx = blocks;
+        }
+        if (!m) continue;
+        hipLaunchKernelGGL(wgrad_fold_group_kernel, dim3(gx, m), dim3(256), 0, (hipStream_t)stream, a);
+        HV_LAUNCH_CHECK();
+    }
+    return HV_OK;
+}
+
 struct WgradPlan { int BN, BC, KT, splits, chunk; };
 static int wgrad_plan(const hv_wgrad_desc* d, WgradPlan* pl) {
     const int J = d->KH * d->KW * d->Cin;
@@ -961,6 +992,59 @@
     if (c && !taken) return hv_wgrad_fold_now(c, stream);
     return HV_OK;
 }
+extern "C" size_t hv_wgrad_tr_group_workspace_bytes(const hv_wgrad_desc* d, int chunks_per_layer) {
+    if (wgrad_validate(d) != HV_OK) return 0;
+    return hv_wgrad_trg_workspace_bytes(d, chunks_per_layer);
+}
+extern "C" int hv_wgrad_tr_group(const hv_wgrad_desc* descs, int n, int chunks_per_layer, int* nslabs, void* stream) {
+    constexpr int kMax = 8;
+    if (!descs || !nslabs || n < 1 || chunks_per_layer < 1) return HV_ERR_ARG;
+    if (n > kMax) return HV_ERR_UNSUPPORTED;
+    for (int i = 0; i < n; ++i) {
+        const int rc = wgrad_validate(&descs[i]);
+        if (rc != HV_OK) return rc;
+    }
+    if (!hv_wgrad_trg_ok(descs, n, chunks_per_layer)) return HV_ERR_UNSUPPORTED;
+    for (int i = 0; i < n; ++i) {
+        const hv_wgrad_desc& d = descs[i];
+        if (!d.workspace || ((uintptr_t)d.workspace & 15) || d.workspace_bytes < hv_wgrad_trg_workspace_bytes(&d, chunks_per_layer)) return HV_ERR_WORKSPACE;
+        for (int j = 0; j < i; ++j)
+            if (descs[j].workspace == d.workspace || descs[j].dw == d.dw) return HV_ERR_ARG;
+        const hv_wgrad_fold* c = d.carry;
+        if (c && c->nslabs > 0 && (!c->slabs || !c->dw || c->numel <= 0 || (c->numel & 3))) return HV_ERR_ARG;
+    }
+    HvFold folds[kMax];
+    const hv_wgrad_fold* after[kMax];
+    int nfold = 0, nafter = 0;
+    for (int i = 0; i < n; ++i) {
+        const hv_wgrad_fold* c = descs[i].carry;
+        if (!c || c->nslabs <= 0) continue;
+        bool clash = false;
+        for (int j = 0; j < n; ++j) clash = clash || c->slabs == descs[j].workspace || c->dw == descs[j].dw;
+        bool twice = false;
+        for (int j = 0; j < nfold; ++j) twice = twice || c->dw == folds[j].dw;
+        if (twice && !clash) { after[nafter++] = c; continue; }
+        if (clash) {
+            const int rc = hv_wgrad_fold_now(c, stream);
+            if (rc != HV_OK) return rc;
+        } else
+            folds[nfold++] = HvFold{c->slabs, c->dw, c->numel, c->nslabs, c->accumulate, c->dbias ? c->bias_slabs : nullptr, c->dbias, c->Cout, c->dbias_accumulate};
+    }
+    int rc = hv_wgrad_trg(descs, n, chunks_per_layer, nslabs, folds, nfold, (hipStream_t)stream);
+    if (rc != HV_OK) return rc;
+    for (int i = 0; i < nafter; ++i) {
+        rc = hv_wgrad_fold_now(after[i], stream);
+        if (rc != HV_OK) return rc;
+    }
+    for (int i = 0; i < n; ++i) {
+        const hv_wgrad_desc& d = descs[i];
+        const long long nW = (long long)d.Cout * d.KH * d.KW * d.Cin;
+        rc = wgrad_fold_or_defer(&d, d.workspace, nW, nslabs[i], d.dbias ? d.workspace + (long long)nslabs[i] * nW : nullptr, (hipStream_t)stream);
+        if (rc != HV_OK) return rc;
+    }
+    return HV_OK;
+}
+
 static int wgrad_dispatch(const hv_wgrad_desc* d, void* stream) {
     int rc;
     const long long nW = (long long)d->Cout * d->KH * d->KW * d->Cin;
diff --git a/healthivert-gan_amd/csrc/prep.hip b/healthivert-gan_amd/csrc/prep.hip
--- a/healthivert-gan_amd/csrc/prep.hip
+++ b/healthivert-gan_amd/csrc/prep.hip
@@ -727,5 +727,5 @@
     return HV_OK;
 }
 
-extern "C" int hv_version(void) { return 106; }
+extern "C" int hv_version(void) { return 107; }
 extern "C" const char* hv_arch(void) { return "gfx950"; }
diff --git a/healthivert-gan_amd/csrc/wgrad_tr.hip b/healthivert-gan_amd/csrc/wgrad_tr.hip
--- a/healthivert-gan_amd/csrc/wgrad_tr.hip
+++ b/healthivert-gan_amd/csrc/wgrad_tr.hip
@@ -7,6 +7,8 @@
 typedef __fp16 hv_fp16x4 __attribute__((__vector_size__(4 * sizeof(__fp16))));
 typedef unsigned int u32x4 __attribute__((ext_vector_type(4)));
 typedef unsigned int u32x2 __attribute__((ext_vector_type(2)));
+
+size_t hv_wgrad_halo_workspace_bytes(const hv_wgrad_desc* d);
 
 struct WTrK {
     const _Float16* x; const _Float16* g; float* slabs;
@@ -35,7 +37,7 @@
 }
 
 template <int KS, int ST, int BN, int BC>
-__global__ __launch_bounds__(256, 2) void wgrad_tr_kernel(const WTrK p) {
+__device__ __forceinline__ void wgrad_tr_body(const WTrK& p, const int by, const int bz, char* smem) {
     constexpr int TH = 8, TW = 16, TAPS = KS * KS, SLOTS = (TAPS + 3) / 4;
     constexpr int PH = (TH - 1) * ST + KS, PW = (TW - 1) * ST + KS;
     constexpr int NT = BN / 16, CT = BC / 16;
@@ -43,17 +45,11 @@
     constexpr int GI = TH * TW * (BN / 8), XI = PH * PW * (BC / 8);
     constexpr int GPT = (GI + 255) / 256, XPT = (XI + 255) / 256;
     static_assert(NT * CT * SLOTS <= 32, "accumulator budget");
-    extern __shared__ __attribute__((aligned(16))) char smem[];
     char* Gs = smem;
     char* Xs = smem + TH * TW * SG;
 
-    if ((int)blockIdx.x >= p.gx) {
-        const int fx = (int)gridDim.x - p.gx;
-        hv_fold_blocks(p.fold, ((int)blockIdx.x - p.gx) + fx * ((int)blockIdx.y + (int)gridDim.y * (int)blockIdx.z), fx * (int)gridDim.y * (int)gridDim.z, smem);
-        return;
-    }
     const int tid = threadIdx.x, lane = tid & 63, wave = __builtin_amdgcn_readfirstlane(tid >> 6);
-    const int co0 = blockIdx.y * BN, ci0 = blockIdx.z * BC;
+    const int co0 = by * BN, ci0 = bz * BC;
     const int grp = lane >> 4, sub = lane & 15, qr = sub >> 2, pc = sub & 3;
 
     f32x4 acc[SLOTS][NT][CT];
@@ -63,7 +59,7 @@
         for (int n = 0; n < NT; ++n)
 #pragma unroll
             for (int c = 0; c < CT; ++c) acc[s][n][c] = (f32x4){0.f, 0.f, 0.f, 0.f};
-    const bool do_bias = p.bias_out != nullptr && blockIdx.z == 0 && wave == 0;
+    const bool do_bias = p.bias_out != nullptr && bz == 0 && wave == 0;
     f32x4 bacc[NT];
 #pragma unroll
     for (int n = 0; n < NT; ++n) bacc[n] = (f32x4){0.f, 0.f, 0.f, 0.f};
@@ -189,6 +185,50 @@
                 if (co < p.Cout) p.bias_out[(long long)blockIdx.x * p.Cout + co] = bacc[n][r];
             }
     }
+}
+
+template <int KS, int ST, int BN, int BC>
+__global__ __launch_bounds__(256, 2) void wgrad_tr_kernel(const WTrK p) {
+    extern __shared__ __attribute__((aligned(16))) char smem[];
+    if ((int)blockIdx.x >= p.gx) {
+        const int fx = (int)gridDim.x - p.gx;
+        hv_fold_blocks(p.fold, ((int)blockIdx.x - p.gx) + fx * ((int)blockIdx.y + (int)gridDim.y * (int)blockIdx.z), fx * (int)gridDim.y * (int)gridDim.z, smem);
+        return;
+    }
+    wgrad_tr_body<KS, ST, BN, BC>(p, blockIdx.y, blockIdx.z, smem);
+}
+
+constexpr int kWTrGroupMax = 8;
+struct WTrGLayer {
+    const _Float16* x; const _Float16* g; float* slabs; float* bias_out;
+    int Hl, Wl, Ho, Wo, img_stride, x_ld, x_coff, g_ld, g_coff;
+    int tiles_x, tiles_per_img, tiles_per_sub, ntiles, dil, gx;
+    unsigned x_bytes, g_bytes;
+};
+struct WTrG {
+    WTrK common;
+    int nfold;
+    WTrGLayer L[kWTrGroupMax];
+    HvFold folds[kWTrGroupMax];
+};
+
+__global__ __launch_bounds__(256, 2) void wgrad_trg_kernel(const WTrG a) {
+    extern __shared__ __attribute__((aligned(16))) char smem[];
+    if ((int)blockIdx.x >= a.common.gx) {
+        const int fx = (int)gridDim.x - a.common.gx, T = fx * (int)gridDim.y * (int)gridDim.z;
+        const int l = ((int)blockIdx.x - a.common.gx) + fx * ((int)blockIdx.y + (int)gridDim.y * (int)blockIdx.z);
+        const int f = l % a.nfold;
+        hv_fold_blocks(a.folds[f], l / a.nfold, (T - f + a.nfold - 1) / a.nfold, smem);
+        return;
+    }
+    const WTrGLayer& L = a.L[blockIdx.y >> 1];
+    if ((int)blockIdx.x >= L.gx) return;
+    WTrK p = a.common;
+    p.x = L.x; p.g = L.g; p.slabs = L.slabs; p.bias_out = L.bias_out;
+    p.Hl = L.Hl; p.Wl = L.Wl; p.Ho = L.Ho; p.Wo = L.Wo; p.img_stride = L.img_stride; p.x_ld = L.x_ld; p.x_coff = L.x_coff; p.g_ld = L.g_ld; p.g_coff = L.g_coff;
+    p.tiles_x = L.tiles_x; p.tiles_per_img = L.tiles_per_img; p.tiles_per_sub = L.tiles_per_sub; p.ntiles = L.ntiles; p.dil = L.dil; p.gx = L.gx;
+    p.x_bytes = L.x_bytes; p.g_bytes = L.g_bytes;
+    wgrad_tr_body<3, 1, 32, 32>(p, blockIdx.y & 1, blockIdx.z, smem);
 }
 
 typedef int i32x4 __attribute__((ext_vector_type(4)));
@@ -479,6 +519,7 @@
         const long long pairs = (long long)hv_cdiv(d->Cout, pl->BN) * hv_cdiv(d->Cin, pl->BC);
         const int want = (pairs <= 4 && (long long)d->Cout * d->KH * d->KW * d->Cin * 4 <= 256 * 1024) ? kWantSmall : kWantBig;
         long long gx = (want + pairs - 1) / pairs;
+        if (d->chunks > 0) gx = d->chunks;
         if (gx > ntiles) gx = ntiles;
         if (gx < 1) gx = 1;
         pl->gx = (int)gx;
@@ -935,12 +976,8 @@
     return launch_wthing<3, 16, 8>(k, pl, d, s);
 }
 
-int hv_wgrad_tr(const hv_wgrad_desc* d, int* nslabs, hipStream_t s) {
-    WTrPlan pl;
-    if (!wgrad_tr_plan(d, &pl)) return HV_ERR_UNSUPPORTED;
-    const size_t need = hv_wgrad_tr_workspace_bytes(d);
-    if (!d->workspace || d->workspace_bytes < need) return HV_ERR_WORKSPACE;
-    WTrK k;
+static void wtr_fill(const hv_wgrad_desc* d, const WTrPlan& pl, WTrK* kp) {
+    WTrK& k = *kp;
     k.x = reinterpret_cast<const _Float16*>(d->x); k.g = reinterpret_cast<const _Float16*>(d->g); k.slabs = d->workspace;
     const int dl = pl.dil;
     k.Hl = d->H / dl; k.Wl = d->W / dl; k.in_shift = d->in_shift; k.Wp = d->W >> d->in_shift;
@@ -953,11 +990,89 @@
     k.dbg = 0;
     k.gx = pl.gx;
     k.fold.splits = 0;
+    k.x_bytes = (unsigned)((size_t)d->B * k.img_stride * sizeof(_Float16));
+    k.g_bytes = (unsigned)((size_t)d->B * d->Ho * d->Wo * d->g_ld * sizeof(_Float16));
+}
+
+static bool wtrg_plan(const hv_wgrad_desc* d, int chunks, WTrPlan* pl) {
+    if (chunks < 1) return false;
+    if (hv_wgrad_thin_workspace_bytes(d) || hv_wgrad_halo_workspace_bytes(d)) return false;
+    hv_wgrad_desc dd = *d;
+    dd.chunks = chunks;
+    if (!wgrad_tr_plan(&dd, pl)) return false;
+    return d->KH == 3 && d->stride == 1 && pl->BN == 32 && pl->BC == 32 && !pl->dma && d->Cout == 64 && d->in_shift == 0 && d->pad == d->dil && d->Ho == d->H &&
+           d->Wo == d->W;
+}
+size_t hv_wgrad_trg_workspace_bytes(const hv_wgrad_desc* d, int chunks) {
+    WTrPlan pl;
+    if (!wtrg_plan(d, chunks, &pl)) return 0;
+    return (size_t)pl.gx * ((size_t)d->Cout * d->KH * d->KW * d->Cin + (d->dbias ? d->Cout : 0)) * sizeof(float);
+}
+bool hv_wgrad_trg_ok(const hv_wgrad_desc* descs, int n, int chunks) {
+    if (n < 1 || n > kWTrGroupMax) return false;
+    for (int i = 0; i < n; ++i) {
+        WTrPlan pl;
+        const hv_wgrad_desc &d = descs[i], &r = descs[0];
+        if (!wtrg_plan(&d, chunks, &pl)) return false;
+        if (d.B != r.B || d.H != r.H || d.W != r.W || d.Cin != r.Cin) return false;
+    }
+    return true;
+}
+int hv_wgrad_trg(const hv_wgrad_desc* descs, int n, int chunks, int* nslabs, const HvFold* folds, int nfold, hipStream_t s) {
+    if (!hv_wgrad_trg_ok(descs, n, chunks) || nfold < 0 || nfold > kWTrGroupMax) return HV_ERR_UNSUPPORTED;
+    WTrG a = {};
+    WTrPlan pl;
+    int gx_max = 0;
+    for (int i = 0; i < n; ++i) {
+        wtrg_plan(&descs[i], chunks, &pl);
+        WTrK k;
+        wtr_fill(&descs[i], pl, &k);
+        if (i == 0) a.common = k;
+        WTrGLayer& L = a.L[i];
+        L.x = k.x; L.g = k.g; L.slabs = k.slabs; L.bias_out = k.bias_out;
+        L.Hl = k.Hl; L.Wl = k.Wl; L.Ho = k.Ho; L.Wo = k.Wo; L.img_stride = k.img_stride; L.x_ld = k.x_ld; L.x_coff = k.x_coff; L.g_ld = k.g_ld; L.g_coff = k.g_coff;
+        L.tiles_x = k.tiles_x; L.tiles_per_img = k.tiles_per_img; L.tiles_per_sub = k.tiles_per_sub; L.ntiles = k.ntiles; L.dil = k.dil; L.gx = k.gx;
+        L.x_bytes = k.x_bytes; L.g_bytes = k.g_bytes;
+        nslabs[i] = pl.gx;
+        if (pl.gx > gx_max) gx_max = pl.gx;
+    }
+    for (int i = n; i < kWTrGroupMax; ++i) a.L[i] = a.L[0];
+    a.common.gx = gx_max;
+    a.nfold = nfold;
+    for (int i = 0; i < kWTrGroupMax; ++i) a.folds[i] = folds && i < nfold ? folds[i] : HvFold{};
+    auto kern = wgrad_trg_kernel;
+    dim3 grid(gx_max, 2 * n, hv_cdiv(descs[0].Cin, 32));
+    if (nfold > 0) {
+        long long total = 0;
+        for (int i = 0; i < nfold; ++i) {
+            const int Q = 256 / (folds[i].splits <= 16 ? 4 : folds[i].splits <= 64 ? 16 : 32);
+            long long t = (folds[i].n / 4 + Q - 1) / Q + (folds[i].dbias ? (folds[i].nb + Q - 1) / Q : 0);
+            if (t > total) total = t;
+        }
+        if (total > 192) total = 192;
+        total *= nfold;
+        const int planes = (int)(grid.y * grid.z);
+        grid.x += (unsigned)((total + planes - 1) / planes);
+    }
+    hv_path_note = 12;
+    HV_KNAME("wgrad_trg_kernel(WTrG)");
+    HV_TIMING_BEGIN(s);
+    hipLaunchKernelGGL(kern, grid, dim3(256), pl.lds, s, a);
+    HV_TIMING_END(s);
+    HV_LAUNCH_CHECK();
+    return HV_OK;
+}
+
+int hv_wgrad_tr(const hv_wgrad_desc* d, int* nslabs, hipStream_t s) {
+    WTrPlan pl;
+    if (!wgrad_tr_plan(d, &pl)) return HV_ERR_UNSUPPORTED;
+    const size_t need = hv_wgrad_tr_workspace_bytes(d);
+    if (!d->workspace || d->workspace_bytes < need) return HV_ERR_WORKSPACE;
+    WTrK k;
+    wtr_fill(d, pl, &k);
 #ifdef WT_STAMPS
     if (getenv("HV_WTR_DBG")) k.dbg = atoi(getenv("HV_WTR_DBG"));
 #endif
-    k.x_bytes = (unsigned)((size_t)d->B * k.img_stride * sizeof(_Float16));
-    k.g_bytes = (unsigned)((size_t)d->B * d->Ho * d->Wo * d->g_ld * sizeof(_Float16));
     *nslabs = pl.gx;
 #define WTR(KS_, ST_)                                                                                     \
     do {                                                                                                  \
diff --git a/healthivert-gan_amd/engine.py b/healthivert-gan_amd/engine.py
--- a/healthivert-gan_amd/engine.py
+++ b/healthivert-gan_amd/engine.py
@@ -299,6 +299,7 @@
         self.side = None
         self._side_of = None
         self.wgrad_block = WgradBlock()
+        self.wgrad_groups = None
 
     def fork(self):
         cur = torch.cuda.current_stream()
@@ -350,13 +351,17 @@
         else:
             run()
 
-    def launch(self, keep_collecting=False):
+    def launch(self, keep_collecting=False, groups=None):
         if self.side is None:
             return
         self.side.wait_stream(torch.cuda.current_stream())
         with torch.cuda.stream(self.side):
+            if groups is not None:
+                groups.hold = True
             for run in self.queue:
                 run()
+            if groups is not None:
+                groups.flush()
             self.pset.fold_chain().flush()
         self.queue, self.later, self.collecting = self.later, [], keep_collecting
 
@@ -367,7 +372,46 @@
         self.side, self.collecting = None, False
 
 
-def _wgrad(node, p, xin, gfull, accumulate, prec, dbias=None, dbias_accumulate=False):
+WGRAD_GROUP_LAYERS = 4
+WGRAD_GROUP_CHUNKS = 32
+
+
+class WgradGroups:
+    __slots__ = ('items', 'hold')
+
+    def __init__(self):
+        self.items, self.hold = {}, False
+
+    def offer(self, p, member):
+        if not ops.wgrad_group_ok(WGRAD_GROUP_CHUNKS, **member):
+            return False
+        x = member['x']
+        key = (x.B, x.H, x.W, x.C)
+        items = self.items.setdefault(key, [])
+        items.append((p, dict(member, name=getattr(p, 'name', None) or 'conv')))
+        if not self.hold and len(items) >= WGRAD_GROUP_LAYERS:
+            self._issue(self.items.pop(key))
+        return True
+
+    def flush(self):
+        pending, self.items, self.hold = self.items, {}, False
+        for items in pending.values():
+            self._issue(items)
+
+    @staticmethod
+    def _issue(items):
+        ngroups = -(-len(items) // WGRAD_GROUP_LAYERS)
+        for i in range(ngroups):
+            part = items[i * len(items) // ngroups:(i + 1) * len(items) // ngroups]
+            owner = part[0][0].owner
+            ops.conv2d_wgrad_group([m for _, m in part], WGRAD_GROUP_CHUNKS, chain=owner.fold_chain() if owner is not None else None)
+
+
+def _wgrad(node, p, xin, gfull, accumulate, prec, dbias=None, dbias_accumulate=False, groups=None):
+    if groups is not None and not node.transposed and groups.offer(p, dict(
+            x=xin, g=gfull, dw=p.dw, k=node.k, stride=node.s, pad=node.pad, dil=node.d, in_shift=node.shift, accumulate=accumulate, precision=prec,
+            dbias=dbias, dbias_accumulate=dbias_accumulate)):
+        return
     chain = p.owner.fold_chain() if p.owner is not None else None
     if node.transposed:
         ops.conv2d_wgrad(gfull, xin, p.dw, node.k, node.s, node.pad, node.d, accumulate=accumulate, precision=prec, chain=chain)
@@ -391,9 +435,9 @@
         xin = Act(xs.t, p.cin_wg, xs.coff)
         if book.wgrad_block.collecting:
             book.wgrad_block.add(lambda node=node, p=p, xin=xin, gfull=gfull, acc=wgrad_accumulate, db=p.bias.grad if fuse_dbias else None, dba=dbias_accumulate:
-                                 _wgrad(node, p, xin, gfull, acc, prec, dbias=db, dbias_accumulate=dba))
+                                 _wgrad(node, p, xin, gfull, acc, prec, dbias=db, dbias_accumulate=dba, groups=book.wgrad_groups))
         else:
-            _wgrad(node, p, xin, gfull, wgrad_accumulate, prec, dbias=p.bias.grad if fuse_dbias else None, dbias_accumulate=dbias_accumulate)
+            _wgrad(node, p, xin, gfull, wgrad_accumulate, prec, dbias=p.bias.grad if fuse_dbias else None, dbias_accumulate=dbias_accumulate, groups=book.wgrad_groups)
     if not node.need_dx:
         return
     if node.transposed:
diff --git a/healthivert-gan_amd/models/inpaint_networks.py b/healthivert-gan_amd/models/inpaint_networks.py
--- a/healthivert-gan_amd/models/inpaint_networks.py
+++ b/healthivert-gan_amd/models/inpaint_networks.py
@@ -433,6 +433,9 @@
         d_pred1, d_pred2 = zero(d_pred1, P.pred1), zero(d_pred2, P.pred2)
         wg = book.wgrad_block
         wg.open(self.paramset(), d_x_stage2.device)
+        if book.wgrad_groups is None:
+            book.wgrad_groups = E.WgradGroups()
+        groups = book.wgrad_groups
         wg.before_next_block(lambda: up19.materialise(prec))
         wg.before_next_block(lambda: up20.materialise(prec))
         head['fine_generator.allconv17'].backward(d_x_stage2, book, prec)
@@ -461,18 +464,19 @@
             main.wait_stream(side)
             E.conv_backward(pmconv1, book, prec, premultiplied=E.chain_link(pmconv2, pmconv1, book, prec))
         ops.add_channels(Act(d_coarse_seg.view(B, H, W, 1)), book.twin(a['f_in']).slice(1, 1), Act(P.d_cs_total.view(B, H, W, 1)))
-        wg.launch(keep_collecting=True)
+        wg.launch(keep_collecting=True, groups=groups)
         head['coarse_generator.conv17'].backward(P.d_xs1_total, book, prec, mul_x='elu')
         head['coarse_generator.conv18'].backward(P.d_cs_total, book, prec, mul_x='elu')
         p19 = up19.backward(coarse('dec19'), book, prec, True)
         p20 = up20.backward(coarse('dec20'), book, prec, p19)
-        wg.launch()
+        wg.launch(groups=groups)
         conv10, conv11 = N['coarse_generator.conv10_atrous'], N['coarse_generator.conv11']
         E.conv_backward_chain(list(coarse('mid')), book, prec, premultiplied_first=p20, stop_before=conv10)
         pre10 = E.chain_link(conv11, conv10, book, prec)
         ops.gap_fc_sigmoid_backward(d_pred1, P.pred1, P.c_pool, cg.fc_height.weight, book.twin(a['c10']),
                                     cg.fc_height.weight.grad, cg.fc_height.bias.grad, mul=(a['c10'], conv10.act) if pre10 else None)
         E.conv_backward_chain(list(coarse('enc')), book, prec, premultiplied_first=pre10)
+        groups.flush()
         wg.join()
         self.paramset().finish_backward(accumulate=False)
         self.paramset().attach_grads()
diff --git a/healthivert-gan_amd/ops.py b/healthivert-gan_amd/ops.py
--- a/healthivert-gan_amd/ops.py
+++ b/healthivert-gan_amd/ops.py
@@ -254,25 +254,39 @@
 
 
 class FoldChain:
-    __slots__ = ('pending', 'slot', 'stream')
+    __slots__ = ('pending', 'group', 'slot', 'gslot', 'stream')
 
     def __init__(self, stream_handle):
-        self.pending, self.slot, self.stream = None, 0, stream_handle
+        self.pending, self.group, self.slot, self.gslot, self.stream = None, [], 0, 0, stream_handle
+
+    def take(self, n):
+        folds = ([self.pending] if self.pending is not None else []) + self.group
+        self.pending = None
+        if n is None:
+            n = len(folds)
+        self.group = folds[n:]
+        return folds[:n]
 
     def flush(self):
-        if self.pending is not None:
+        if self.pending is not None or self.group:
             assert torch.cuda.current_stream().cuda_stream == self.stream, 'FoldChain.flush() on another stream than its weight gradients'
-            f, self.pending = self.pending, None
-            _lib.get().call('hv_wgrad_fold_now', ctypes.byref(f), stream())
+            fold_now(self.take(None))
+
+
+def fold_now(folds):
+    L = _lib.get()
+    if len(folds) == 1:
+        L.call('hv_wgrad_fold_now', ctypes.byref(folds[0]), stream())
+    elif folds:
+        arr = (L.hv_wgrad_fold * len(folds))(*folds)
+        L.call('hv_wgrad_fold_group', arr, len(folds), stream())
 
 
 FOLD_CHAIN = True
 
 
-def conv2d_wgrad(x, g, dw, k, stride=1, pad=0, dil=1, in_shift=0, accumulate=False, precision=None, cin=None, cout=None, dbias=None,
-                 dbias_accumulate=False, chain=None):
-    L = _lib.get()
-    d = L.hv_wgrad_desc()
+def _wgrad_desc(x, g, dw, k, stride=1, pad=0, dil=1, in_shift=0, accumulate=False, precision=None, cin=None, cout=None, dbias=None, dbias_accumulate=False):
+    d = _lib.get().hv_wgrad_desc()
     kh, kw = (k, k) if isinstance(k, int) else k
     d.x = ptr(x.t).value
     d.B, d.H, d.W, d.in_shift = x.B, x.H << in_shift, x.W << in_shift, in_shift
@@ -287,14 +301,24 @@
     d.dbias_accumulate = int(dbias_accumulate)
     d.x_f16, d.g_f16 = x.f16, g.f16
     d.workspace, d.workspace_bytes = None, 0
+    return d
+
+
+def conv2d_wgrad(x, g, dw, k, stride=1, pad=0, dil=1, in_shift=0, accumulate=False, precision=None, cin=None, cout=None, dbias=None,
+                 dbias_accumulate=False, chain=None, chunks=0):
+    L = _lib.get()
+    d = _wgrad_desc(x, g, dw, k, stride, pad, dil, in_shift, accumulate, precision, cin, cout, dbias, dbias_accumulate)
+    d.chunks = int(chunks)
+    kh, kw = d.KH, d.KW
     if chain is not None and not FOLD_CHAIN:
         chain = None
     need = L.size('hv_conv2d_wgrad_workspace_bytes', ctypes.byref(d))
     fold = None
     if chain is not None:
         assert torch.cuda.current_stream(x.t.device).cuda_stream == chain.stream, 'a FoldChain belongs to one stream'
-        if chain.pending is not None:
-            d.carry = ctypes.pointer(chain.pending)
+        carried = chain.take(1)
+        if carried:
+            d.carry = ctypes.pointer(carried[0])
         if need:
             b, _ = _ws(need, x.t.device, slot=('fold-chain', chain.slot))
             chain.slot ^= 1
@@ -314,6 +338,62 @@
     if chain is not None:
         chain.pending = fold if (fold is not None and fold.nslabs > 0) else None
     return dw
+
+
+def wgrad_group_ok(chunks, *args, **kw):
+    d = _wgrad_desc(*args, **kw)
+    key = ('hv_wgrad_tr_group_workspace_bytes', int(chunks), bytes(d))
+    r = _PROBES.get(key)
+    if r is None:
+        r = _PROBES[key] = _lib.get().size('hv_wgrad_tr_group_workspace_bytes', ctypes.byref(d), int(chunks)) > 0
+    return r
+
+
+def conv2d_wgrad_group(members, chunks, chain=None):
+    L = _lib.get()
+    n = len(members)
+    descs = (L.hv_wgrad_desc * n)()
+    if chain is not None and not FOLD_CHAIN:
+        chain = None
+    dev = members[0]['x'].t.device
+    folds, keep = [], []
+    if chain is not None:
+        assert torch.cuda.current_stream(dev).cuda_stream == chain.stream, 'a FoldChain belongs to one stream'
+        carried = chain.take(None)
+        if len(carried) > n:
+            fold_now(carried[n:])
+            carried = carried[:n]
+        par = chain.gslot
+        chain.gslot ^= 1
+    else:
+        carried, par = [], None
+    names = [m.get('name', 'layer %d' % i) for i, m in enumerate(members)]
+    for i, m in enumerate(members):
+        d = _wgrad_desc(**{k: v for k, v in m.items() if k != 'name'})
+        need = L.size('hv_wgrad_tr_group_workspace_bytes', ctypes.byref(d), int(chunks))
+        if not need:
+            raise RuntimeError('conv2d_wgrad_group: member %d does not qualify (ask wgrad_group_ok first)' % i)
+        b, _ = _ws(need, dev, slot=('wgrad-group', par, i))
+        keep.append(b)
+        d.workspace, d.workspace_bytes = ptr(b).value, b.numel()
+        if i < len(carried):
+            d.carry = ctypes.pointer(carried[i])
+        if chain is not None:
+            f = L.hv_wgrad_fold()
+            folds.append(f)
+            d.pending = ctypes.pointer(f)
+        descs[i] = d
+    nslabs = (ctypes.c_int * n)()
+    run = lambda: L.call('hv_wgrad_tr_group', descs, n, int(chunks), nslabs, stream())
+    if _TIMER is not None:
+        d = descs[0]
+        flops = 2.0 * n * d.B * d.Ho * d.Wo * d.Cout * d.KH * d.KW * d.Cin
+        nbytes = n * (2 * d.B * d.H * d.W * (d.Cin + d.Cout) + 4 * d.Cout * d.KH * d.KW * d.Cin)
+        _TIMER.wrap(('wgrad', d.B, d.H, d.W, d.Cin, d.Cout, d.KH, 1, tuple('%s d%d' % (nm, m.get('dil', 1)) for nm, m in zip(names, members)), 0), flops, run, nbytes)
+    else:
+        run()
+    if chain is not None:
+        chain.group = [f for f in folds if f.nslabs > 0]
 
 
 class LayerTable:
diff --git a/healthivert-gan_amd/profiler.py b/healthivert-gan_amd/profiler.py
--- a/healthivert-gan_amd/profiler.py
+++ b/healthivert-gan_amd/profiler.py
@@ -127,4 +127,6 @@
     if name.startswith('void '):
         name = name[5:]
     name = name.split('(')[0]
+    if isinstance(d, tuple):
+        return '%s forward B%d %dx%d Cin%d->Cout%d k%d s%d group of %d: %s' % (name, B, H, W, cin, cout, k, s, len(d), ', '.join(d))
     return '%s %s B%d %dx%d Cin%d->Cout%d k%d s%d d%d' % (name, 'transposed' if tr else 'forward', B, H, W, cin, cout, k, s, d)
diff --git a/include/hvgan.h b/include/hvgan.h
--- a/include/hvgan.h
+++ b/include/hvgan.h
@@ -73,10 +73,14 @@
     float* dbias; int dbias_accumulate;
     hv_wgrad_fold* pending;
     const hv_wgrad_fold* carry;
+    int chunks;
 } hv_wgrad_desc;
 int hv_wgrad_fold_now(const hv_wgrad_fold* fold , void* stream);
 size_t hv_conv2d_wgrad_workspace_bytes(const hv_wgrad_desc* d);
 int hv_conv2d_wgrad(const hv_wgrad_desc* d, void* stream);
+int hv_wgrad_fold_group(const hv_wgrad_fold* folds , int n, void* stream);
+size_t hv_wgrad_tr_group_workspace_bytes(const hv_wgrad_desc* d, int chunks_per_layer);
+int hv_wgrad_tr_group(const hv_wgrad_desc* descs, int n, int chunks_per_layer, int* nslabs, void* stream);
 
 typedef struct {
     const float* w_orig;
```

Result: no change. 2576 slices/s, median of 3 (+0.1%).
